# andrewendlinger/xmris

Hardware: AMD Instinct MI355X
Metric: spectra/sec (zero_fill->apodize->FFT->autophase), n_time=4096; HBM-roofline % (higher is better)
Workload: dtype f32

## Files before the change

include/xmris_hip.h:

```cpp
#ifndef XMRIS_HIP_H
#define XMRIS_HIP_H

#include <stdint.h>

#ifdef __cplusplus
extern "C" {
#endif

typedef enum { XM_C64 = 0, XM_C128 = 1 } xm_dtype;

typedef enum {
  XM_OK = 0,
  XM_ERR_INVALID_ARG = -1,
  XM_ERR_UNSUPPORTED_N = -2,
  XM_ERR_HIP = -3,
  XM_ERR_NO_DEVICE = -4
} xm_status;

#define XM_FFT_INVERSE 1u
#define XM_FFT_ORTHO 2u
#define XM_FFT_SHIFT_IN 4u
#define XM_FFT_SHIFT_OUT 8u
#define XM_AMAX_VALUE_ONLY 16u

#define XM_AMAX_GLOBAL_KEY 32u
#define XM_KEY_BYTES 131072
typedef struct {
  float max2;
  float pad_;
  int64_t flat;
} xm_argmax_result;

int xm_version(void);
const char* xm_last_error_string(void);
int xm_clear_cache(void);
const char* xm_last_kernel_string(void);
int xm_fft_supported(int n, int dtype);
int xm_plan_prepare(int n, int dtype);

int xm_zero_fill(const void* in, void* out, int64_t n_batch, int n_in, int n_out, int pad_left,
                 int dtype, void* stream);

int xm_apodize(const void* in, void* out, const void* window, int64_t n_batch, int n, int dtype,
               void* stream);

int xm_zf_apod(const void* in, int64_t in_row_stride, void* out, const void* window, int64_t n_batch, int n_in, int n_out,
               int pad_left, int in_dtype, int out_dtype, void* stream);

int xm_pipeline_key_native(const void* in, int64_t in_row_stride, int n_in, int n_out, int pad_left, unsigned flags,
                           int dtype);

int xm_fft1d_batched(const void* in, void* out, int64_t n_batch, int n, unsigned flags, int dtype,
                     void* stream);

int xm_roll(const void* in, void* out, int64_t n_batch, int n, int shift, int dtype, void* stream);

int xm_phase_apply(const void* in, void* out, const void* phase_table, int64_t n_batch, int n,
                   int dtype, void* stream);

int xm_absmax_rows(const void* in, int64_t n_batch, int n, void* absmax2, int32_t* argidx, int dtype,
                   void* stream);

int xm_row_l1(const void* in, int64_t in_row_stride, const void* window, int64_t n_batch, int n_in, int pad_left,
              int sub_step, void* norm, uint64_t* key, int dtype, void* stream);

int xm_argmax_key_take(uint64_t* key, int n_per_row, void* out_max2, int64_t* out_flat, const void* in,
                       int64_t in_row_stride, int n_in, void* out_row, int dtype, void* stream);

int xm_guess_supported(const void* in, int64_t in_row_stride, int n_in, int n_out, int pad_left, unsigned flags, int dtype);
int xm_guess_rows(const void* in, int64_t in_row_stride, const void* window, int64_t n_batch, int n_in, int n_out,
                  int n_guess, unsigned flags, float* est, uint64_t* key, int dtype, void* stream);
int xm_guess_refine(const void* in, int64_t in_row_stride, const void* window, int64_t n_batch, int n_in, int n_out,
                    unsigned flags, const float* est, uint64_t* guess_key, float band, uint64_t* work_key,
                    float* out_max2, int64_t* out_flat, void* out_row, int dtype, void* stream);

int xm_argmax_reduce(const void* absmax2, const int32_t* argidx, int64_t n_batch, int n, void* out_max2,
                     int64_t* out_flat, int dtype, void* stream);

int xm_gather_row_c128(const void* in, int64_t in_row_stride, int n_in, const int64_t* flat_index, int n_per_row,
                       void* out, int dtype, void* stream);

int xm_pipeline_fused(const void* in, int64_t in_row_stride, void* out, const void* window,
                      const void* phase_table, int64_t n_batch, int n_in, int n_out, int pad_left,
                      unsigned flags, void* absmax2, int32_t* argidx, int dtype, void* stream);

int xm_pipeline_fused_ramp(const void* in, int64_t in_row_stride, void* out, const void* window, double phase0,
                           double dphase, int64_t n_batch, int n_in, int n_out, int pad_left, unsigned flags,
                           void* absmax2, int32_t* argidx, int dtype, void* stream);
int xm_pipeline_ramp_native(const void* in, int64_t in_row_stride, int n_in, int n_out, int pad_left, unsigned flags,
                            int dtype);

int64_t xm_baseline_als_workspace_bytes(int64_t n_batch, int n);
int xm_baseline_als(const void* in, int is_complex, int64_t n_batch, int n, double lam, double p, int n_iter, void* out,
                    void* workspace, int64_t workspace_bytes, int dtype, void* stream);

int xm_amares_model(const double* params, int64_t n_batch, int n_peaks, int n, double dt, double t0, void* out,
                    void* stream);
int64_t xm_amares_workspace_bytes(int64_t n_batch, int n, int n_peaks);
int xm_amares_fit(const void* in, int64_t in_row_stride, int64_t n_batch, int n, double dt, double t0, int n_peaks,
                  const double* init, const double* lower, const double* upper, const int32_t* fixed, int max_iter,
                  double ftol, double xtol, double* params, double* amp_sd, double* rss, int32_t* status,
                  int32_t* iters, void* fit_data, void* workspace, int64_t workspace_bytes, int dtype, void* stream);
int xm_amares_fit_linked(const void* in, int64_t in_row_stride, int64_t n_batch, int n, double dt, double t0,
                         int n_peaks, const double* init, const double* lower, const double* upper,
                         const int32_t* fixed, const int32_t* link_to, const double* link_scale,
                         const double* link_offset, int max_iter, double ftol, double xtol, double* params,
                         double* amp_sd, double* rss, int32_t* status, int32_t* iters, void* fit_data, void* workspace,
                         int64_t workspace_bytes, int dtype, void* stream);

int xm_basis_model(const double* params, int64_t n_batch, const void* basis, int n_metab, const int32_t* group,
                   int n_groups, int n, double dt, void* out, void* stream);
int64_t xm_basis_workspace_bytes(int64_t n_batch, int n, int n_metab);
int xm_basis_fit(const void* in, int64_t in_row_stride, int64_t n_batch, int n, double dt, int skip, const void* basis,
                 int n_metab, const int32_t* group, int n_groups, const double* init, const double* lower,
                 const double* upper, const int32_t* fixed, int max_iter, double ftol, double xtol, double* params,
                 double* amp_sd, double* rss, int32_t* status, int32_t* iters, void* fit_data, void* workspace,
                 int64_t workspace_bytes, int dtype, void* stream);

#define XM_COIL_SVD 0
#define XM_COIL_FIRST_POINT 1
#define XM_COIL_SVD_FMA 2
#define XM_COIL_WORKSPACE_BYTES 256
int xm_coil_combine(const void* x, const void* ref_or_null, void* y, void* w, double* quality, int32_t* status,
                    int64_t n_outer, int C, int64_t n_inner, int N, int N_R, const void* linv_or_null, int method,
                    int n_points, int is_complex128, void* workspace, void* stream);

#define XM_ALIGN_WORKSPACE_BYTES 256
#define XM_ALIGN_SKIP_COARSE 0x100
#define XM_ALIGN_SKIP_REFINE 0x200
#define XM_ALIGN_SKIP_APPLY 0x400
int64_t xm_align_workspace_bytes(int64_t n_outer, int A, int64_t n_inner, int N);
int xm_align_rows(const void* x, const void* r, int64_t r_voxel_stride, void* y, void* mean_or_null, double* shift,
                  double* phase, double* quality, int32_t* status, int32_t* n_averaged_or_null, int64_t n_outer, int A,
                  int64_t n_inner, int N, int N_r, int L, double dt, double t0, double max_shift, double min_quality,
                  int dtype, void* workspace, void* stream);

#define XM_HSVD_WORKSPACE_BYTES 256
#define XM_HSVD_GRAM_FMA 0x100
#define XM_HSVD_STOP_GRAM 0x200
#define XM_HSVD_STOP_EIG 0x400
#define XM_HSVD_STOP_POLES 0x600
#define XM_HSVD_STOP_AMPL 0x800
int xm_hsvd_rows(const void* x, int64_t row_stride, void* y_or_null, double* freq, double* damp, double* amp,
                 double* phase, int32_t* removed, int32_t* n_removed, int32_t* status, int64_t n_batch, int N, int M,
                 int K, double dt, double f_lo, double f_hi, int dtype, void* workspace, void* stream);

#define XM_DENOISE_WORKSPACE_BYTES 256
#define XM_DENOISE_GRAM_FMA 0x100
#define XM_DENOISE_STOP_GRAM 0x200
#define XM_DENOISE_STOP_EIG 0x400
int xm_denoise_patches(const void* x, void* y, int32_t* rank_out, double* sigma, int32_t* status, int64_t n_outer, int s1,
                       int s2, int s3, int p1, int p2, int p3, int N, int rank, int dtype, void* workspace, void* stream);

int xm_axis_dft(const void* x, void* y, const void* table, int64_t n_outer, int n, int m, int64_t n_inner, int dtype,
                void* stream);

#define XM_SENSE_WORKSPACE_BYTES 256
int xm_sense_unfold(const void* a, void* y, const void* sens, const void* linv_or_null, double* g_or_null,
                    int32_t* status_or_null, int64_t n_outer, int C, const int32_t n[3], const int32_t accel[3], int N_t,
                    const int64_t a_strides[5], const int64_t y_strides[4], double regularization, int dtype,
                    void* workspace, void* stream);

int xm_grappa_fill(const void* a, void* y, const void* weights, int64_t n_outer, int C, const int32_t n[3],
                   const int32_t accel[3], const int32_t kernel[3], int N_t, const int64_t a_strides[5],
                   const int64_t y_strides[5], int dtype, void* stream);

int xm_axis_sparse(const void* x, void* y, const int32_t* rowptr, const int32_t* col, const double* val, int64_t n_outer,
                   int64_t n, int64_t n_rows, int64_t n_inner, int dtype, void* stream);

#define XM_CGS_VOXELS 16
int xm_cgs_expand(const void* r, void* p, const void* s, void* u, const double* rho_new, const double* rho_old,
                  const int32_t* status, int64_t n_coils, int64_t n_vox, int64_t n_cols, int first, int dtype,
                  void* stream);
int xm_cgs_reduce(const void* u, const void* s, const void* p, void* q, double* part, int64_t n_coils, int64_t n_vox,
                  int64_t n_cols, double lambda, int initial, int dtype, void* stream);
int xm_cgs_step(void* x, void* r, const void* p, const void* q, const double* rho, const double* rho0,
                const double* delta, double* rho_out, const int32_t* status_in, int32_t* status_out, int32_t* n_iter,
                double* residual, int64_t n_vox, int64_t n_cols, double tol, int iteration, int final_test, void* stream);

int xm_l1_start(const void* b, double* bpart, double* bmax, int32_t* status, double* change, void* x, int64_t n_vox,
                int64_t n_cols, int finish, void* stream);
int xm_l1_prox(void* x, void* v, const void* q, const void* b, const uint8_t* mask, const double* bmax,
               const double* d2_in, const double* n2_in, double* d2_out, double* n2_out, const int32_t* status_in,
               int32_t* status_out, int32_t* n_iter, double* change, int n_dims, int64_t m0, int64_t m1, int64_t m2, int l0,
               int l1, int l2, int s0, int s1, int s2, int64_t n_cols, double tau, double theta_scale, double beta, double tol,
               int iteration, int mode, void* stream);

int xm_espirit_eig(const void* h, void* maps, double* values, int32_t* status, int64_t n_vox, int n_coils, int n_maps,
                   int phase_ref, double crop, void* stream);

int xm_shift_time_fused(int L, int dtype);
int xm_shift_time(const void* in, int64_t in_row_stride, void* out, int64_t n_rows, int n, int L, const double* frac,
                  int64_t n_delay, int64_t delay_div, int dtype, void* stream);

int xm_kinetics_fit(const double* substrate, const double* products, const double* weights, int64_t n_batch,
                    int n_products, int n_times, const double* times, const double* flip_s, const double* flip_p,
                    const double* init, const double* lower, const double* upper, const int32_t* fixed, int max_iter,
                    double ftol, double xtol, double* params, double* param_sd, double* rss, int32_t* status,
                    int32_t* iters, double* fit, double* auc_ratio, void* stream);

#define XM_SPECIES_SKIP_GRAM 0x100
#define XM_SPECIES_SKIP_COARSE 0x200
#define XM_SPECIES_SKIP_REFINE 0x400
#define XM_SPECIES_SKIP_APPLY 0x800
int xm_species_separate(const void* x, void* y, const int64_t* dims, const int64_t* x_strides, const int64_t* y_strides,
                        int n_echoes, int n_species, const double* tables, const double* tau, int64_t tau_s0,
                        int64_t tau_s1, const double* psi, int64_t psi_s0, int64_t psi_s1, double* field,
                        double* residual, int32_t* status, int fit, double max_field, double span, int dtype,
                        void* stream);

#define XM_LIPID_FMA 0x100
#define XM_LIPID_SKIP_COEF 0x200
#define XM_LIPID_SKIP_APPLY 0x400
int xm_lipid_project(const void* x, void* y, int64_t n_rows, int64_t x_row_stride, int64_t y_row_stride, int T, int rank,
                     const double* tables, const uint8_t* apply, int32_t* status, int dtype, void* stream);

#define XM_SUB_MAX_RANK 32
int xm_sub_project(const void* y, void* b, const void* basis, const uint8_t* sampling, int64_t n_coils, int64_t n_samples,
                   int64_t n_frames, int64_t n_time, int rank, int64_t coil_stride, int64_t sample_stride,
                   int64_t frame_stride, int dtype, void* stream);
int xm_sub_mix(const void* a, void* z, const void* kernel, int64_t n_coils, int64_t n_samples, int64_t n_frames, int rank,
               int dtype, void* stream);
int xm_sub_expand(const void* u, const void* basis, void* x, int64_t n_vox, int64_t n_frames, int64_t n_time, int rank,
                  void* stream);

void* xm_solver_create(const double* slice_re_im, const double* coords, int n, double pivot, int method,
                       int target_idx, int index_width);
void xm_solver_destroy(void* solver);
double xm_solver_score(void* solver, const double* x, int nx);
void xm_solver_score_batch(void* solver, const double* xs, int nx, int count, double* out);
long xm_solver_nfev(void* solver);
int xm_solver_set_threads(void* solver, int threads);
int xm_solver_fg(void* solver, const double* x, int n, const double* lb, const double* ub, double* f_out, double* g_out);
long xm_solver_pool_backups(void);
int xm_solver_de(void* solver, int p0_only, unsigned seed, double tol, int maxiter, double* x_out ,
                 double* fun_out, int* nfev_out, int* nit_out);

int xm_phase_table(const double* coords, int n, double p0_deg, double p1_deg, double pivot, void* out, int as_float);

int xm_phase_apply_rows(const void* in, void* out, const double* coords, int64_t n_rows, int n, const double* p0,
                        const double* p1, const double* pivot, const int32_t* skip, int dtype, void* stream);

typedef struct {
  double x[2];
  double fun;
  double pg_norm;
  int32_t nfev, nit;
  int32_t status;
  int32_t needs_polish;
  int32_t target_idx;
  int32_t pad_;
  uint64_t seq;
  double t_us[8];
} xm_search_result;
int xm_search_supported(int n, int method, double x_range);
int xm_search_launch(const void* slice, int n, double c0, double cstep, double x_range, int method, int p0_only,
                     unsigned seed, double tol, int maxiter, uint64_t seq, xm_search_result* out, void* stream);
int xm_search_eval(const void* slice, int n, double c0, double cstep, double x_range, int target_idx, int p0_only,
                   const double* xs, int count, double* fs, void* stream);

enum { XM_SEARCH_CONVERGED = 0, XM_SEARCH_MAXITER = 1, XM_SEARCH_ALL_ZERO = 2, XM_SEARCH_NOT_FINITE = 3 };
typedef struct {
  double x[2];
  double fun;
  double pg_norm;
  int32_t nfev, nit;
  int32_t target_idx;
  int32_t status;
  int32_t needs_polish;
  int32_t pad_;
} xm_search_row;
int xm_search_rows_supported(int n, int method, double x_range, int dtype);
int xm_search_rows(const void* in, int64_t n_rows, int n, int dtype, double c0, double cstep, double x_range, int p0_only,
                   unsigned seed, double tol, int maxiter, double pivot, int target_idx, xm_search_row* records,
                   void* stream);

int xm_hostsearch_submit(const void* slice, int n, const double* coords, int method, int target_idx, int index_width,
                         int p0_only, unsigned seed, double tol, int maxiter, int threads, uint64_t seq,
                         xm_search_result* out);

int xm_hostsearch_set_workers(int n);

int xm_stream_create(void** stream, int reserved_cus, int partition);
int xm_stream_destroy(void* stream);
int xm_stream_cus(void* stream);

int64_t xm_atomic_load_acquire_i64(const int64_t* p);
void xm_atomic_store_release_i64(int64_t* p, int64_t value);
int xm_atomic_wait_all_ge_i64(const int64_t* p, int stride_words, int count, int64_t value, int spin_us);

#ifdef __cplusplus
}
#endif
#endif
```

xmris_amd/_lib.py:

```python
from __future__ import annotations

import ctypes
import os
import threading

XM_C64 = 0
XM_C128 = 1

XM_FFT_INVERSE = 1
XM_FFT_ORTHO = 2
XM_FFT_SHIFT_IN = 4
XM_FFT_SHIFT_OUT = 8
XM_AMAX_VALUE_ONLY = 16
XM_AMAX_GLOBAL_KEY = 32

XM_COIL_SVD = 0
XM_COIL_FIRST_POINT = 1
XM_COIL_SVD_FMA = 2
XM_COIL_WORKSPACE_BYTES = 256

XM_ALIGN_WORKSPACE_BYTES = 256
XM_ALIGN_SKIP_COARSE = 0x100
XM_ALIGN_SKIP_REFINE = 0x200
XM_ALIGN_SKIP_APPLY = 0x400

XM_HSVD_WORKSPACE_BYTES = 256
XM_HSVD_GRAM_FMA = 0x100
XM_HSVD_STOP_GRAM = 0x200
XM_HSVD_STOP_EIG = 0x400
XM_HSVD_STOP_POLES = 0x600
XM_HSVD_STOP_AMPL = 0x800

XM_DENOISE_WORKSPACE_BYTES = 256
XM_DENOISE_GRAM_FMA = 0x100
XM_DENOISE_STOP_GRAM = 0x200
XM_DENOISE_STOP_EIG = 0x400

XM_SPECIES_SKIP_GRAM = 0x100
XM_SPECIES_SKIP_COARSE = 0x200
XM_SPECIES_SKIP_REFINE = 0x400
XM_SPECIES_SKIP_APPLY = 0x800

XM_LIPID_FMA = 0x100
XM_LIPID_SKIP_COEF = 0x200
XM_LIPID_SKIP_APPLY = 0x400

XM_SENSE_WORKSPACE_BYTES = 256
XM_CGS_VOXELS = 16
XM_L1_MAX_BLOCK = 16
XM_SUB_MAX_RANK = 32

XM_ERR_INVALID_ARG = -1
XM_ERR_UNSUPPORTED_N = -2
XM_ERR_HIP = -3
XM_ERR_NO_DEVICE = -4

LIB_NAME = "libxmris_hip.so"
LIB_PATH = os.environ.get("XMRIS_AMD_LIB") or os.path.join(os.path.dirname(os.path.abspath(__file__)), LIB_NAME)

_p = ctypes.c_void_p
_i = ctypes.c_int
_u = ctypes.c_uint
_l = ctypes.c_int64

SIGNATURES = {
    "xm_version": (_i, []),
    "xm_last_error_string": (ctypes.c_char_p, []),
    "xm_clear_cache": (_i, []),
    "xm_last_kernel_string": (ctypes.c_char_p, []),
    "xm_fft_supported": (_i, [_i, _i]),
    "xm_plan_prepare": (_i, [_i, _i]),
    "xm_zero_fill": (_i, [_p, _p, _l, _i, _i, _i, _i, _p]),
    "xm_apodize": (_i, [_p, _p, _p, _l, _i, _i, _p]),
    "xm_fft1d_batched": (_i, [_p, _p, _l, _i, _u, _i, _p]),
    "xm_zf_apod": (_i, [_p, _l, _p, _p, _l, _i, _i, _i, _i, _i, _p]),
    "xm_roll": (_i, [_p, _p, _l, _i, _i, _i, _p]),
    "xm_phase_apply": (_i, [_p, _p, _p, _l, _i, _i, _p]),
    "xm_absmax_rows": (_i, [_p, _l, _i, _p, _p, _i, _p]),
    "xm_argmax_reduce": (_i, [_p, _p, _l, _i, _p, _p, _i, _p]),
    "xm_baseline_als_workspace_bytes": (_l, [_l, _i]),
    "xm_baseline_als": (_i, [_p, _i, _l, _i, ctypes.c_double, ctypes.c_double, _i, _p, _p, _l, _i, _p]),
    "xm_amares_model": (_i, [_p, _l, _i, _i, ctypes.c_double, ctypes.c_double, _p, _p]),
    "xm_amares_workspace_bytes": (_l, [_l, _i, _i]),
    "xm_amares_fit": (_i, [_p, _l, _l, _i, ctypes.c_double, ctypes.c_double, _i, _p, _p, _p, _p, _i, ctypes.c_double,
                           ctypes.c_double, _p, _p, _p, _p, _p, _p, _p, _l, _i, _p]),
    "xm_amares_fit_linked": (_i, [_p, _l, _l, _i, ctypes.c_double, ctypes.c_double, _i, _p, _p, _p, _p, _p, _p, _p, _i,
                                  ctypes.c_double, ctypes.c_double, _p, _p, _p, _p, _p, _p, _p, _l, _i, _p]),
    "xm_basis_model": (_i, [_p, _l, _p, _i, _p, _i, _i, ctypes.c_double, _p, _p]),
    "xm_basis_workspace_bytes": (_l, [_l, _i, _i]),
    "xm_basis_fit": (_i, [_p, _l, _l, _i, ctypes.c_double, _i, _p, _i, _p, _i, _p, _p, _p, _p, _i, ctypes.c_double,
                          ctypes.c_double, _p, _p, _p, _p, _p, _p, _p, _l, _i, _p]),
    "xm_coil_combine": (_i, [_p, _p, _p, _p, _p, _p, _l, _i, _l, _i, _i, _p, _i, _i, _i, _p, _p]),
    "xm_align_workspace_bytes": (_l, [_l, _i, _l, _i]),
    "xm_align_rows": (_i, [_p, _p, _l, _p, _p, _p, _p, _p, _p, _p, _l, _i, _l, _i, _i, _i, ctypes.c_double, ctypes.c_double,
                           ctypes.c_double, ctypes.c_double, _i, _p, _p]),
    "xm_hsvd_rows": (_i, [_p, _l, _p, _p, _p, _p, _p, _p, _p, _p, _l, _i, _i, _i, ctypes.c_double, ctypes.c_double,
                          ctypes.c_double, _i, _p, _p]),
    "xm_denoise_patches": (_i, [_p, _p, _p, _p, _p, _l, _i, _i, _i, _i, _i, _i, _i, _i, _i, _p, _p]),
    "xm_axis_dft": (_i, [_p, _p, _p, _l, _i, _i, _l, _i, _p]),
    "xm_sense_unfold": (_i, [_p, _p, _p, _p, _p, _p, _l, _i, _p, _p, _i, _p, _p, ctypes.c_double, _i, _p, _p]),
    "xm_grappa_fill": (_i, [_p, _p, _p, _l, _i, _p, _p, _p, _i, _p, _p, _i, _p]),
    "xm_axis_sparse": (_i, [_p, _p, _p, _p, _p, _l, _l, _l, _l, _i, _p]),
    "xm_cgs_expand": (_i, [_p, _p, _p, _p, _p, _p, _p, _l, _l, _l, _i, _i, _p]),
    "xm_cgs_reduce": (_i, [_p, _p, _p, _p, _p, _l, _l, _l, ctypes.c_double, _i, _i, _p]),
    "xm_cgs_step": (_i, [_p, _p, _p, _p, _p, _p, _p, _p, _p, _p, _p, _p, _l, _l, ctypes.c_double, _i, _i, _p]),
    "xm_l1_start": (_i, [_p, _p, _p, _p, _p, _p, _l, _l, _i, _p]),
    "xm_l1_prox": (_i, [_p] * 14 + [_i, _l, _l, _l, _i, _i, _i, _i, _i, _i, _l, ctypes.c_double, ctypes.c_double,
                                    ctypes.c_double, ctypes.c_double, _i, _i, _p]),
    "xm_espirit_eig": (_i, [_p, _p, _p, _p, _l, _i, _i, _i, ctypes.c_double, _p]),
    "xm_shift_time_fused": (_i, [_i, _i]),
    "xm_shift_time": (_i, [_p, _l, _p, _l, _i, _i, _p, _l, _l, _i, _p]),
    "xm_kinetics_fit": (_i, [_p, _p, _p, _l, _i, _i, _p, _p, _p, _p, _p, _p, _p, _i, ctypes.c_double, ctypes.c_double, _p, _p,
                             _p, _p, _p, _p, _p, _p]),
    "xm_species_separate": (_i, [_p, _p, _p, _p, _p, _i, _i, _p, _p, _l, _l, _p, _l, _l, _p, _p, _p, _i, ctypes.c_double,
                                 ctypes.c_double, _i, _p]),
    "xm_lipid_project": (_i, [_p, _p, _l, _l, _l, _i, _i, _p, _p, _p, _i, _p]),
    "xm_sub_project": (_i, [_p, _p, _p, _p, _l, _l, _l, _l, _i, _l, _l, _l, _i, _p]),
    "xm_sub_mix": (_i, [_p, _p, _p, _l, _l, _l, _i, _i, _p]),
    "xm_sub_expand": (_i, [_p, _p, _p, _l, _l, _l, _i, _p]),
    "xm_gather_row_c128":(_i, [_p, _l, _i, _p, _i, _p, _i, _p]),
    "xm_pipeline_fused": (_i, [_p, _l, _p, _p, _p, _l, _i, _i, _i, _u, _p, _p, _i, _p]),
    "xm_pipeline_fused_ramp": (_i, [_p, _l, _p, _p, ctypes.c_double, ctypes.c_double, _l, _i, _i, _i, _u, _p, _p, _i, _p]),
    "xm_pipeline_ramp_native": (_i, [_p, _l, _i, _i, _i, _u, _i]),
    "xm_pipeline_key_native": (_i, [_p, _l, _i, _i, _i, _u, _i]),
    "xm_row_l1": (_i, [_p, _l, _p, _l, _i, _i, _i, _p, _p, _i, _p]),
    "xm_argmax_key_take": (_i, [_p, _i, _p, _p, _p, _l, _i, _p, _i, _p]),
    "xm_guess_supported": (_i, [_p, _l, _i, _i, _i, _u, _i]),
    "xm_guess_rows": (_i, [_p, _l, _p, _l, _i, _i, _i, _u, _p, _p, _i, _p]),
    "xm_guess_refine": (_i, [_p, _l, _p, _l, _i, _i, _u, _p, _p, ctypes.c_float, _p, _p, _p, _p, _i, _p]),
    "xm_phase_table": (_i, [_p, _i, ctypes.c_double, ctypes.c_double, ctypes.c_double, _p, _i]),
    "xm_solver_create": (_p, [_p, _p, _i, ctypes.c_double, _i, _i, _i]),
    "xm_solver_destroy": (None, [_p]),
    "xm_solver_score": (ctypes.c_double, [_p, _p, _i]),
    "xm_solver_score_batch": (None, [_p, _p, _i, _i, _p]),
    "xm_solver_fg": (_i, [_p, _p, _i, _p, _p, _p, _p]),
    "xm_solver_pool_backups": (ctypes.c_long, []),
    "xm_solver_nfev": (ctypes.c_long, [_p]),
    "xm_solver_set_threads": (_i, [_p, _i]),
    "xm_solver_de": (_i, [_p, _i, _u, ctypes.c_double, _i, _p, _p, _p, _p]),
    "xm_search_supported": (_i, [_i, _i, ctypes.c_double]),
    "xm_search_launch": (_i, [_p, _i, ctypes.c_double, ctypes.c_double, ctypes.c_double, _i, _i, _u, ctypes.c_double, _i,
                              ctypes.c_uint64, _p, _p]),
    "xm_search_eval": (_i, [_p, _i, ctypes.c_double, ctypes.c_double, ctypes.c_double, _i, _i, _p, _i, _p, _p]),
    "xm_search_rows_supported": (_i, [_i, _i, ctypes.c_double, _i]),
    "xm_search_rows": (_i, [_p, _l, _i, _i, ctypes.c_double, ctypes.c_double, ctypes.c_double, _i, _u, ctypes.c_double, _i,
                            ctypes.c_double, _i, _p, _p]),
    "xm_phase_apply_rows": (_i, [_p, _p, _p, _l, _i, _p, _p, _p, _p, _i, _p]),
    "xm_hostsearch_submit": (_i, [_p, _i, _p, _i, _i, _i, _i, _u, ctypes.c_double, _i, _i, ctypes.c_uint64, _p]),
    "xm_hostsearch_set_workers": (_i, [_i]),
    "xm_stream_create": (_i, [_p, _i, _i]),
    "xm_stream_destroy": (_i, [_p]),
    "xm_stream_cus": (_i, [_p]),
    "xm_atomic_load_acquire_i64": (_l, [_p]),
    "xm_atomic_store_release_i64": (None, [_p, _l]),
    "xm_atomic_wait_all_ge_i64": (_i, [_p, _i, _i, _l, _i]),
}


class XmrisHipError(RuntimeError):

    def __init__(self, func: str, code: int, detail: str):
        self.func, self.code, self.detail = func, code, detail
        super().__init__(f"{func} failed with status {code}: {detail}")


class UnsupportedLengthError(XmrisHipError, ValueError):
    """The transform length has no in-LDS plan on the device (status XM_ERR_UNSUPPORTED_N)."""


_lock = threading.Lock()
_lib = None


def load() -> ctypes.CDLL:
    global _lib
    if _lib is not None:
        return _lib
    with _lock:
        if _lib is not None:
            return _lib
        if not os.path.exists(LIB_PATH):
            raise RuntimeError(
                f"{LIB_PATH} is missing. The xmris_amd hot path has no CPU fallback: build the HIP "
                f"library first (`python -c \"import __graft_entry__ as g; g.build()\"` or "
                f"`make -C xmris_amd/csrc`)."
            )
        lib = ctypes.CDLL(LIB_PATH)
        for name, (res, args) in SIGNATURES.items():
            fn = getattr(lib, name)
            fn.restype = res
            fn.argtypes = args
        _lib = lib
    return _lib


def check(func: str, status: int) -> None:
    if status == 0:
        return
    detail = load().xm_last_error_string()
    detail = detail.decode("utf-8", "replace") if detail else ""
    if status == XM_ERR_UNSUPPORTED_N:
        raise UnsupportedLengthError(func, status, detail)
    raise XmrisHipError(func, status, detail)


def call(func: str, *args) -> None:
    check(func, getattr(load(), func)(*args))
```

xmris_amd/csrc/xm_api.hip:

```cpp
#include "xm_host.h"
#include "xm_als.h"
#include "xm_kernels.h"
#include "xm_plans.h"
#include "xm_zfapod.h"

#include <cmath>
#include <cstdio>
#include <cstdlib>
#include <cstring>
#include <map>
#include <mutex>
#include <tuple>

#define XM_VERSION_NUM 500

static thread_local std::string g_err;
static thread_local std::string g_last_kernel;

#include <cxxabi.h>
void xm_note_kernel(const char* base, const std::type_info* plan, const char* scalar, int mode, int opt) {
  std::string name = base;
  name += "<";
  if (scalar) name += std::string(scalar) + ", ";
  if (plan) {
// ... 260 lines not shown
  HIP_TRY(hipGetDevice(&dev));
  HIP_TRY(hipDeviceGetAttribute(&total, hipDeviceAttributeMultiprocessorCount, dev));
  if (reserved_cus >= total || (partition == 1 && reserved_cus == 0)) return fail(XM_ERR_INVALID_ARG, "xm_stream_create: bad partition");
  const int words = (total + 31) / 32;
  std::vector<uint32_t> mask((size_t)words, 0u);
  for (int i = 0; i < total; ++i) {
    const bool reserved = i < reserved_cus;
    if (reserved == (partition == 1)) mask[i / 32] |= 1u << (i % 32);
  }
  hipStream_t st = nullptr;
  HIP_TRY(hipExtStreamCreateWithCUMask(&st, (uint32_t)words, mask.data()));
  {
    std::lock_guard<std::mutex> lk(g_stream_mu);
    g_stream_cus[st] = partition == 1 ? reserved_cus : total - reserved_cus;
  }
  *stream = (void*)st;
  return XM_OK;
}

extern "C" int xm_stream_destroy(void* stream) {
  if (!stream) return XM_OK;
  {
    std::lock_guard<std::mutex> lk(g_stream_mu);
    g_stream_cus.erase((hipStream_t)stream);
  }
  HIP_TRY(hipStreamDestroy((hipStream_t)stream));
  return XM_OK;
}

extern "C" int xm_stream_cus(void* stream) {
  int cus = 0;
  const int rc = xm_stream_cu_count((hipStream_t)stream, &cus);
  return rc ? rc : cus;
}

const char* xm_last_kernel_string(void) { return g_last_kernel.c_str(); }

int xm_clear_cache(void) {
  {
    std::lock_guard<std::mutex> lk(g_stream_mu);
    g_stream_cus.clear();
  }
  std::lock_guard<std::mutex> lk(g_mu);
  for (auto& kv : g_tables) (void)hipFree(kv.second);
  g_tables.clear();
  for (int d = 0; d < 16; ++d) {
    if (g_queue_base[d]) (void)hipFree(g_queue_base[d]);
    g_queue_base[d] = nullptr;
  }
  return XM_OK;
}

int xm_fft_supported(int n, int dtype) { return xm_supported(n, dtype) ? 1 : 0; }

int xm_plan_prepare(int n, int dtype) {
  if (!xm_supported(n, dtype)) return fail(XM_ERR_UNSUPPORTED_N, "unsupported length " + std::to_string(n));
  int rc = XM_OK;
  const int n_ins[2] = {n, n / 2};
  for (int i = 0; i < (n % 2 == 0 && n >= 4 ? 2 : 1) && rc == XM_OK; ++i) {
    const unsigned fl = XM_FFT_ORTHO | XM_FFT_SHIFT_OUT;
    rc = dtype == XM_C64
             ? xm_pipeline_f32(nullptr, n_ins[i], nullptr, nullptr, nullptr, nullptr, 0, n_ins[i], n, 0, fl, nullptr, nullptr, nullptr)
             : xm_pipeline_f64(nullptr, n_ins[i], nullptr, nullptr, nullptr, nullptr, 0, n_ins[i], n, 0, fl, nullptr, nullptr, nullptr);
  }
  return rc;
}

int xm_zero_fill(const void* in, void* out, int64_t n_batch, int n_in, int n_out, int pad_left, int dtype,
                 void* stream) {
  int rc = check_common(in, n_batch, n_in, dtype);
  if (rc) return rc;
  if (!out || n_out < n_in || pad_left < 0 || pad_left + n_in > n_out)
    return fail(XM_ERR_INVALID_ARG, "zero_fill: bad output pointer or geometry");
  if (n_batch == 0) return XM_OK;
  const long long total = (long long)n_batch * n_out;
  hipStream_t st = (hipStream_t)stream;
  DeviceGuard guard(in);
  if (dtype == XM_C64)
    hipLaunchKernelGGL(k_zero_fill<float>, dim3(grid_for(total, 256)), dim3(256), 0, st, (const Cx<float>*)in,
                       (Cx<float>*)out, (long long)n_batch, n_in, n_out, pad_left);
  else
    hipLaunchKernelGGL(k_zero_fill<double>, dim3(grid_for(total, 256)), dim3(256), 0, st, (const Cx<double>*)in,
                       (Cx<double>*)out, (long long)n_batch, n_in, n_out, pad_left);
  HIP_TRY(hipGetLastError());
  return XM_OK;
}

int xm_apodize(const void* in, void* out, const void* window, int64_t n_batch, int n, int dtype, void* stream) {
  int rc = check_common(in, n_batch, n, dtype);
  if (rc) return rc;
  if (!out || !window) return fail(XM_ERR_INVALID_ARG, "apodize: null output or window");
  if (n_batch == 0) return XM_OK;
  const long long total = (long long)n_batch * n;
  hipStream_t st = (hipStream_t)stream;
  DeviceGuard guard(in);
  if (dtype == XM_C64)
    hipLaunchKernelGGL(k_apodize<float>, dim3(grid_for(total, 256)), dim3(256), 0, st, (const Cx<float>*)in,
                       (Cx<float>*)out, (const float*)window, (long long)n_batch, n);
  else
    hipLaunchKernelGGL(k_apodize<double>, dim3(grid_for(total, 256)), dim3(256), 0, st, (const Cx<double>*)in,
                       (Cx<double>*)out, (const double*)window, (long long)n_batch, n);
  HIP_TRY(hipGetLastError());
  return XM_OK;
}

int xm_zf_apod(const void* in, int64_t in_row_stride, void* out, const void* window, int64_t n_batch, int n_in, int n_out,
               int pad_left, int in_dtype, int out_dtype, void* stream) {
  int rc = check_common(in, n_batch, n_in, in_dtype);
  if (rc) return rc;
  if (!out || !window || n_out < n_in || pad_left < 0 || pad_left + n_in > n_out || in_row_stride < n_in || in == out)
    return fail(XM_ERR_INVALID_ARG, "zf_apod: bad pointer or geometry");
  if ((out_dtype != XM_C64 && out_dtype != XM_C128) || (in_dtype == XM_C128 && out_dtype == XM_C64))
    return fail(XM_ERR_INVALID_ARG, "zf_apod: the output precision is the input's or complex128");
  if ((size_t)n_out * (out_dtype == XM_C64 ? 4 : 8) > 96 * 1024)
    return fail(XM_ERR_UNSUPPORTED_N, "zf_apod: the window does not fit the LDS (use xm_zero_fill + xm_apodize)");
  if (n_batch == 0) return XM_OK;
  hipStream_t st = (hipStream_t)stream;
  DeviceGuard guard(in);
  if (in_dtype == XM_C64 && out_dtype == XM_C64)
    return launch_zf_apod<float, float>(in, in_row_stride, out, window, n_batch, n_in, n_out, pad_left, st);
  if (in_dtype == XM_C64)
    return launch_zf_apod<float, double>(in, in_row_stride, out, window, n_batch, n_in, n_out, pad_left, st);
  return launch_zf_apod<double, double>(in, in_row_stride, out, window, n_batch, n_in, n_out, pad_left, st);
}

int xm_phase_apply(const void* in, void* out, const void* phase_table, int64_t n_batch, int n, int dtype,
                   void* stream) {
  int rc = check_common(in, n_batch, n, dtype);
  if (rc) return rc;
  if (!out || !phase_table) return fail(XM_ERR_INVALID_ARG, "phase_apply: null output or table");
  if (n_batch == 0) return XM_OK;
  const long long total = (long long)n_batch * n;
  hipStream_t st = (hipStream_t)stream;
  DeviceGuard guard(in);
  if (dtype == XM_C64)
    hipLaunchKernelGGL(k_phase<float>, dim3(grid_for(total, 256)), dim3(256), 0, st, (const Cx<float>*)in,
                       (Cx<float>*)out, (const Cx<float>*)phase_table, (long long)n_batch, n);
  else
    hipLaunchKernelGGL(k_phase<double>, dim3(grid_for(total, 256)), dim3(256), 0, st, (const Cx<double>*)in,
                       (Cx<double>*)out, (const Cx<double>*)phase_table, (long long)n_batch, n);
  HIP_TRY(hipGetLastError());
  return XM_OK;
}

int xm_phase_apply_rows(const void* in, void* out, const double* coords, int64_t n_rows, int n, const double* p0,
                        const double* p1, const double* pivot, const int32_t* skip, int dtype, void* stream) {
  int rc = check_common(in, n_rows, n, dtype);
  if (rc) return rc;
  if (n_rows == 0) return XM_OK;
  if (!out || !coords || !p0 || !p1 || !pivot) return fail(XM_ERR_INVALID_ARG, "phase_apply_rows: null pointer");
  const long long tiles = ((long long)n + kPhaseRowsBins * kPhaseRowsThreads - 1) / (kPhaseRowsBins * kPhaseRowsThreads);
  long long grid = (long long)n_rows * tiles;
  if (grid > 256LL * 8) grid = 256LL * 8;
  hipStream_t st = (hipStream_t)stream;
  DeviceGuard guard(in);
  if (dtype == XM_C64)
    hipLaunchKernelGGL(k_phase_rows<float>, dim3((unsigned)grid), dim3(kPhaseRowsThreads), 0, st, (const Cx<float>*)in,
                       (Cx<float>*)out, coords, (long long)n_rows, n, p0, p1, pivot, (const int*)skip);
  else
    hipLaunchKernelGGL(k_phase_rows<double>, dim3((unsigned)grid), dim3(kPhaseRowsThreads), 0, st, (const Cx<double>*)in,
                       (Cx<double>*)out, coords, (long long)n_rows, n, p0, p1, pivot, (const int*)skip);
  HIP_TRY(hipGetLastError());
  return XM_OK;
}

int xm_roll(const void* in, void* out, int64_t n_batch, int n, int shift, int dtype, void* stream) {
  int rc = check_common(in, n_batch, n, dtype);
  if (rc) return rc;
  if (!out || in == out) return fail(XM_ERR_INVALID_ARG, "roll: output must be a distinct buffer");
  if (n_batch == 0) return XM_OK;
  shift %= n;
  if (shift < 0) shift += n;
  const long long total = (long long)n_batch * n;
  hipStream_t st = (hipStream_t)stream;
  DeviceGuard guard(in);
  if (dtype == XM_C64)
    hipLaunchKernelGGL(k_roll<float>, dim3(grid_for(total, 256)), dim3(256), 0, st, (const Cx<float>*)in,
                       (Cx<float>*)out, (long long)n_batch, n, shift);
  else
    hipLaunchKernelGGL(k_roll<double>, dim3(grid_for(total, 256)), dim3(256), 0, st, (const Cx<double>*)in,
                       (Cx<double>*)out, (long long)n_batch, n, shift);
  HIP_TRY(hipGetLastError());
  return XM_OK;
}

int xm_absmax_rows(const void* in, int64_t n_batch, int n, void* absmax2, int32_t* argidx, int dtype,
                   void* stream) {
  int rc = check_common(in, n_batch, n, dtype);
  if (rc) return rc;
  if (!absmax2 || !argidx) return fail(XM_ERR_INVALID_ARG, "absmax_rows: null outputs");
  if (n_batch == 0) return XM_OK;
  hipStream_t st = (hipStream_t)stream;
  DeviceGuard guard(in);
  const int grid = (int)(n_batch < 65536 * 4 ? n_batch : 65536 * 4);
  if (dtype == XM_C64)
    hipLaunchKernelGGL(k_absmax_rows<float>, dim3(grid), dim3(256), 0, st, (const Cx<float>*)in,
                       (long long)n_batch, n, (float*)absmax2, argidx);
  else
    hipLaunchKernelGGL(k_absmax_rows<double>, dim3(grid), dim3(256), 0, st, (const Cx<double>*)in,
                       (long long)n_batch, n, (double*)absmax2, argidx);
  HIP_TRY(hipGetLastError());
  return XM_OK;
}

int xm_row_l1(const void* in, int64_t in_row_stride, const void* window, int64_t n_batch, int n_in, int pad_left,
              int sub_step, void* norm, uint64_t* key, int dtype, void* stream) {
  int rc = check_common(in, n_batch, n_in, dtype);
  if (rc) return rc;
  if ((!norm && !key) || pad_left < 0 || in_row_stride < n_in || sub_step < 1)
    return fail(XM_ERR_INVALID_ARG, "row_l1: bad arguments");
  if (key && (dtype != XM_C64 || n_batch > 0xffffffffLL))
    return fail(XM_ERR_INVALID_ARG, "row_l1: the arg-max key needs complex64 and fewer than 2^32 rows");
  if (n_batch == 0) return XM_OK;
  hipStream_t st = (hipStream_t)stream;
  DeviceGuard guard(in);
  const int64_t want = (n_batch + 3) / 4;
  const int grid = (int)(want < 256 * 8 ? want : 256 * 8);
  if (dtype == XM_C64)
    hipLaunchKernelGGL(k_row_l1<float>, dim3(grid), dim3(256), 0, st, (const Cx<float>*)in, (long long)in_row_stride,
                       (const float*)window, (long long)n_batch, n_in, pad_left, sub_step, (float*)norm,
                       (unsigned long long*)key);
  else
    hipLaunchKernelGGL(k_row_l1<double>, dim3(grid), dim3(256), 0, st, (const Cx<double>*)in,
                       (long long)in_row_stride, (const double*)window, (long long)n_batch, n_in, pad_left, sub_step,
                       (double*)norm, (unsigned long long*)nullptr);
  HIP_TRY(hipGetLastError());
  return XM_OK;
}

int xm_argmax_reduce(const void* absmax2, const int32_t* argidx, int64_t n_batch, int n, void* out_max2,
                     int64_t* out_flat, int dtype, void* stream) {
  if (!absmax2 || !argidx || !out_max2 || !out_flat || n_batch < 1 || n < 1)
    return fail(XM_ERR_INVALID_ARG, "argmax_reduce: null pointer or empty batch");
  if (dtype != XM_C64 && dtype != XM_C128) return fail(XM_ERR_INVALID_ARG, "bad dtype");
  hipStream_t st = (hipStream_t)stream;
  DeviceGuard guard(absmax2);
  if (dtype == XM_C64)
    hipLaunchKernelGGL(k_argmax_final<float>, dim3(1), dim3(1024), 0, st, (const float*)absmax2, argidx,
                       (long long)n_batch, n, (float*)out_max2, (long long*)out_flat);
  else
    hipLaunchKernelGGL(k_argmax_final<double>, dim3(1), dim3(1024), 0, st, (const double*)absmax2, argidx,
                       (long long)n_batch, n, (double*)out_max2, (long long*)out_flat);
  HIP_TRY(hipGetLastError());
  return XM_OK;
}

int xm_argmax_key_take(uint64_t* key, int n_per_row, void* out_max2, int64_t* out_flat, const void* in,
                       int64_t in_row_stride, int n_in, void* out_row, int dtype, void* stream) {
  if (!key || !out_max2 || !out_flat || n_per_row < 1) return fail(XM_ERR_INVALID_ARG, "argmax_key_take: null pointer");
  if (in && (!out_row || n_in < 1 || in_row_stride < n_in)) return fail(XM_ERR_INVALID_ARG, "argmax_key_take: bad row geometry");
  if (dtype != XM_C64 && dtype != XM_C128) return fail(XM_ERR_INVALID_ARG, "bad dtype");
  hipStream_t st = (hipStream_t)stream;
  DeviceGuard guard(key);
  if (dtype == XM_C64)
    hipLaunchKernelGGL(k_key_take<float>, dim3(1), dim3(1024), 0, st, (unsigned long long*)key, n_per_row, (float*)out_max2,
                       (long long*)out_flat, (const Cx<float>*)in, (long long)in_row_stride, n_in, (Cx<double>*)out_row);
  else
    hipLaunchKernelGGL(k_key_take<double>, dim3(1), dim3(1024), 0, st, (unsigned long long*)key, n_per_row, (float*)out_max2,
                       (long long*)out_flat, (const Cx<double>*)in, (long long)in_row_stride, n_in, (Cx<double>*)out_row);
  HIP_TRY(hipGetLastError());
  return XM_OK;
}

int xm_guess_supported(const void* in, int64_t in_row_stride, int n_in, int n_out, int pad_left, unsigned flags, int dtype) {
  if (!in || (dtype != XM_C64 && dtype != XM_C128) || in_row_stride < n_in) return 0;
  return xm_zf2p_guess_supported(in, in_row_stride, n_in, n_out, pad_left, flags, dtype);
}

static float guess_scale(int n_out, unsigned flags) {
  return (flags & XM_FFT_ORTHO) ? (float)(1.0 / std::sqrt((double)n_out)) : 1.0f;
}

int xm_guess_rows(const void* in, int64_t in_row_stride, const void* window, int64_t n_batch, int n_in, int n_out,
                  int n_guess, unsigned flags, float* est, uint64_t* key, int dtype, void* stream) {
  int rc = check_common(in, n_batch, n_out, dtype);
  if (rc) return rc;
  if (!est || !key || n_guess < 0 || n_batch > 0xffffffffLL)
    return fail(XM_ERR_INVALID_ARG, "guess_rows: null output or bad sizes");
  if (!xm_guess_supported(in, in_row_stride, n_in, n_out, 0, flags, dtype))
    return fail(XM_ERR_INVALID_ARG, "guess_rows: geometry outside xm_guess_supported");
  if (n_batch == 0) return XM_OK;
  DeviceGuard guard(in);
  return xm_zf2p_guess_rows(in, in_row_stride, (const float*)window, n_batch, n_in, n_out, n_guess,
                            guess_scale(n_out, flags), est, (unsigned long long*)key, dtype, (hipStream_t)stream);
}

int xm_guess_refine(const void* in, int64_t in_row_stride, const void* window, int64_t n_batch, int n_in, int n_out,
                    unsigned flags, const float* est, uint64_t* guess_key, float band, uint64_t* work_key,
                    float* out_max2, int64_t* out_flat, void* out_row, int dtype, void* stream) {
  int rc = check_common(in, n_batch, n_out, dtype);
  if (rc) return rc;
  if (!est || !guess_key || !work_key || work_key == guess_key || !out_flat || n_batch < 1 || n_batch > 0xffffffffLL ||
      !(band > 0.0f && band <= 1.0f))
    return fail(XM_ERR_INVALID_ARG, "guess_refine: null pointer, empty batch or band outside (0, 1]");
  if (!xm_guess_supported(in, in_row_stride, n_in, n_out, 0, flags, dtype))
    return fail(XM_ERR_INVALID_ARG, "guess_refine: geometry outside xm_guess_supported");
  DeviceGuard guard(in);
  return xm_zf2p_guess_refine(in, in_row_stride, (const float*)window, n_batch, n_in, n_out, flags,
                              guess_scale(n_out, flags), est, (unsigned long long*)guess_key, band,
                              (unsigned long long*)work_key, out_max2, (long long*)out_flat, out_row, dtype,
                              (hipStream_t)stream);
}

int64_t xm_baseline_als_workspace_bytes(int64_t n_batch, int n) {
  if (n_batch < 0 || n < 0) return 0;
  return 5 * n_batch * (int64_t)n * (int64_t)sizeof(double);
}

int xm_baseline_als(const void* in, int is_complex, int64_t n_batch, int n, double lam, double p, int n_iter, void* out,
                    void* workspace, int64_t workspace_bytes, int dtype, void* stream) {
  if ((!in || !out || !workspace) && n_batch > 0) return fail(XM_ERR_INVALID_ARG, "baseline_als: null pointer");
  if (n_batch < 0 || n < 4 || n_iter < 1) return fail(XM_ERR_INVALID_ARG, "baseline_als: needs n >= 4, n_iter >= 1");
  if (dtype != XM_C64 && dtype != XM_C128) return fail(XM_ERR_INVALID_ARG, "bad dtype");
  if (workspace_bytes < xm_baseline_als_workspace_bytes(n_batch, n))
    return fail(XM_ERR_INVALID_ARG, "baseline_als: workspace too small (see xm_baseline_als_workspace_bytes)");
  if (n_batch == 0) return XM_OK;
  hipStream_t st = (hipStream_t)stream;
  DeviceGuard guard(in);
  const long long plane = (long long)n_batch * n;
  double* yt = (double*)workspace;
  double *zt = yt + plane, *l1t = yt + 2 * plane, *l2t = yt + 3 * plane, *vt = yt + 4 * plane;
  const long long by = (n_batch + 31) / 32;
  if (by > 65535) return fail(XM_ERR_INVALID_ARG, "baseline_als: n_batch too large for one launch (> 2M spectra)");
  dim3 tgrid((n + 31) / 32, (unsigned)by), tblock(32, 8);
  if (dtype == XM_C64) {
    if (is_complex)
      hipLaunchKernelGGL((k_als_transpose_in<float, true>), tgrid, tblock, 0, st, (const float*)in, (long long)n_batch, n, yt);
    else
      hipLaunchKernelGGL((k_als_transpose_in<float, false>), tgrid, tblock, 0, st, (const float*)in, (long long)n_batch, n, yt);
  } else {
    if (is_complex)
      hipLaunchKernelGGL((k_als_transpose_in<double, true>), tgrid, tblock, 0, st, (const double*)in, (long long)n_batch, n, yt);
    else
      hipLaunchKernelGGL((k_als_transpose_in<double, false>), tgrid, tblock, 0, st, (const double*)in, (long long)n_batch, n, yt);
  }
  hipLaunchKernelGGL(k_als_solve, dim3((unsigned)((n_batch + 63) / 64)), dim3(64), 0, st, yt, zt, l1t, l2t, vt,
                     (long long)n_batch, n, lam, p, n_iter);
  hipLaunchKernelGGL(k_als_transpose_out, tgrid, tblock, 0, st, yt, zt, (long long)n_batch, n, (double*)out);
  HIP_TRY(hipGetLastError());
  return XM_OK;
}

int xm_gather_row_c128(const void* in, int64_t in_row_stride, int n_in, const int64_t* flat_index, int n_per_row,
                       void* out, int dtype, void* stream) {
  if (!in || !flat_index || !out || n_in < 1 || n_per_row < 1 || in_row_stride < n_in)
    return fail(XM_ERR_INVALID_ARG, "gather_row: null pointer or bad geometry");
  if (dtype != XM_C64 && dtype != XM_C128) return fail(XM_ERR_INVALID_ARG, "bad dtype");
  hipStream_t st = (hipStream_t)stream;
  DeviceGuard guard(in);
  const int grid = (n_in + 255) / 256;
  if (dtype == XM_C64)
    hipLaunchKernelGGL(k_gather_row<float>, dim3(grid), dim3(256), 0, st, (const Cx<float>*)in,
                       (long long)in_row_stride, n_in, (const long long*)flat_index, n_per_row, (Cx<double>*)out);
  else
    hipLaunchKernelGGL(k_gather_row<double>, dim3(grid), dim3(256), 0, st, (const Cx<double>*)in,
                       (long long)in_row_stride, n_in, (const long long*)flat_index, n_per_row, (Cx<double>*)out);
  HIP_TRY(hipGetLastError());
  return XM_OK;
}

static int pipeline_common(const void* in, int64_t in_row_stride, void* out, const void* window,
                           const void* phase_table, const double* ramp, int64_t n_batch, int n_in, int n_out,
                           int pad_left, unsigned flags, void* absmax2, int32_t* argidx, int dtype, void* stream) {
  int rc = check_common(in, n_batch, n_out, dtype);
  if (rc) return rc;
  if (n_in < 1 || pad_left < 0 || pad_left + n_in > n_out || in_row_stride < n_in)
    return fail(XM_ERR_INVALID_ARG, "pipeline: bad zero-fill geometry or row stride");
  if (flags & XM_AMAX_GLOBAL_KEY) {
    if (!absmax2 || n_batch > 0xffffffffLL ||
        !xm_pipeline_key_native(in, in_row_stride, n_in, n_out, pad_left, flags & ~(XM_AMAX_GLOBAL_KEY | XM_AMAX_VALUE_ONLY), dtype))
      return fail(XM_ERR_INVALID_ARG, "pipeline: XM_AMAX_GLOBAL_KEY needs a key and a geometry of xm_pipeline_key_native");
    if (dtype == XM_C128 && !argidx)
      return fail(XM_ERR_INVALID_ARG, "pipeline: complex128 arg-max keys are decoded by the launch itself (result record needed)");
  } else if ((absmax2 == nullptr) != (argidx == nullptr))
    return fail(XM_ERR_INVALID_ARG, "pipeline: absmax2 and argidx must be given together");
  if (!out && !absmax2) return fail(XM_ERR_INVALID_ARG, "pipeline: nothing to produce");
  if (out == in) return fail(XM_ERR_INVALID_ARG, "pipeline: in-place operation is not supported");
  if (ramp && !out) return fail(XM_ERR_INVALID_ARG, "pipeline: a phase ramp needs an output");
  if (flags & ~(XM_FFT_INVERSE | XM_FFT_ORTHO | XM_FFT_SHIFT_IN | XM_FFT_SHIFT_OUT | XM_AMAX_VALUE_ONLY | XM_AMAX_GLOBAL_KEY))
    return fail(XM_ERR_INVALID_ARG, "pipeline: unknown flag bits");
  if (!xm_supported(n_out, dtype))
    return fail(XM_ERR_UNSUPPORTED_N, "no plan for length " + std::to_string(n_out));
  hipStream_t st = (hipStream_t)stream;
  DeviceGuard guard(in);
  if (dtype == XM_C64)
    return xm_pipeline_f32(in, in_row_stride, out, window, phase_table, ramp, n_batch, n_in, n_out, pad_left, flags,
                           absmax2, argidx, st);
  return xm_pipeline_f64(in, in_row_stride, out, window, phase_table, ramp, n_batch, n_in, n_out, pad_left, flags,
                         absmax2, argidx, st);
}

int xm_pipeline_fused(const void* in, int64_t in_row_stride, void* out, const void* window,
                      const void* phase_table, int64_t n_batch, int n_in, int n_out, int pad_left, unsigned flags,
                      void* absmax2, int32_t* argidx, int dtype, void* stream) {
  return pipeline_common(in, in_row_stride, out, window, phase_table, nullptr, n_batch, n_in, n_out, pad_left, flags,
                         absmax2, argidx, dtype, stream);
}

int xm_pipeline_fused_ramp(const void* in, int64_t in_row_stride, void* out, const void* window, double phase0,
                           double dphase, int64_t n_batch, int n_in, int n_out, int pad_left, unsigned flags,
                           void* absmax2, int32_t* argidx, int dtype, void* stream) {
  const double ramp[2] = {phase0, dphase};
  return pipeline_common(in, in_row_stride, out, window, nullptr, ramp, n_batch, n_in, n_out, pad_left, flags, absmax2,
                         argidx, dtype, stream);
}

int xm_pipeline_ramp_native(const void* in, int64_t in_row_stride, int n_in, int n_out, int pad_left, unsigned flags,
                            int dtype) {
  if ((dtype != XM_C64 && dtype != XM_C128) || n_in < 1 || pad_left < 0 || pad_left + n_in > n_out) return 0;
  return dtype == XM_C64 ? xm_ramp_native_f32(in, in_row_stride, n_in, n_out, pad_left, flags)
                         : xm_ramp_native_f64(in, in_row_stride, n_in, n_out, pad_left, flags);
}

int xm_pipeline_key_native(const void* in, int64_t in_row_stride, int n_in, int n_out, int pad_left, unsigned flags,
                           int dtype) {
  if ((dtype != XM_C64 && dtype != XM_C128) || n_in < 1 || pad_left < 0 || pad_left + n_in > n_out) return 0;
  return dtype == XM_C64 ? xm_key_native_f32(in, in_row_stride, n_in, n_out, pad_left, flags)
                         : xm_key_native_f64(in, in_row_stride, n_in, n_out, pad_left, flags);
}

int xm_fft1d_batched(const void* in, void* out, int64_t n_batch, int n, unsigned flags, int dtype, void* stream) {
  if (!out) return fail(XM_ERR_INVALID_ARG, "fft: null output");
  return xm_pipeline_fused(in, n, out, nullptr, nullptr, n_batch, n, n, 0, flags, nullptr, nullptr, dtype, stream);
}

}
```

xmris_amd/csrc/xm_coarse.h:

```cpp
#pragma once
#include "xm_kernels.h"

typedef _Float16 xm_h8 __attribute__((ext_vector_type(8)));
typedef _Float16 xm_h2 __attribute__((ext_vector_type(2)));
typedef float xm_f16v __attribute__((ext_vector_type(16)));

struct CoarseArgs {
  const void* in;
  const float* window;
  const Cx<float>* w1024;
  float* est;
  unsigned long long* gkey;
  long long in_stride;
  long long n_batch;
  float scale2;
};

constexpr int kCoarseWaves = 4;

XM_DEV Cx<float> coarse_w1024(const Cx<float>* __restrict__ t, unsigned k) {
  k &= 1023u;
  const Cx<float> w = t[k & 511u];
  return (k & 512u) ? mk<float>(-w.re, -w.im) : w;
}

XM_DEV xm_h8 coarse_pack(const float* v) {
  union {
    xm_h8 v8;
    xm_h2 v2[4];
  } u;
#pragma unroll
  for (int j = 0; j < 4; ++j) {
    const xm_f2 p = {v[2 * j], v[2 * j + 1]};
    u.v2[j] = __builtin_convertvector(p, xm_h2);
  }
  return u.v8;
}

template <bool IN64>
__global__ __launch_bounds__(64 * kCoarseWaves, 2) void k_coarse_mfma(CoarseArgs A) {
  const unsigned lane = threadIdx.x & 63u, r = lane & 31u, h = lane >> 5;
  const long long wave = (long long)blockIdx.x * kCoarseWaves + (threadIdx.x >> 6);
  const long long n_waves = (long long)gridDim.x * kCoarseWaves;

  xm_h8 b1r, b1i, b1n, a2r[2], a2i[2], a2n[2];
  {
    float cr[8], ci[8], cn[8];
#pragma unroll
    for (int j = 0; j < 8; ++j) {
      const Cx<float> w = coarse_w1024(A.w1024, 32u * ((8u * h + (unsigned)j) * r));
      cr[j] = w.re;
      ci[j] = w.im;
      cn[j] = -w.im;
    }
    b1r = coarse_pack(cr);
    b1i = coarse_pack(ci);
    b1n = coarse_pack(cn);
#pragma unroll
    for (int s = 0; s < 2; ++s) {
#pragma unroll
      for (int j = 0; j < 8; ++j) {
        const unsigned n2 = 16u * s + 8u * ((unsigned)j >> 2) + 4u * h + ((unsigned)j & 3u);
        const Cx<float> w = coarse_w1024(A.w1024, 32u * (n2 * r));
        cr[j] = w.re;
        ci[j] = w.im;
        cn[j] = -w.im;
      }
      a2r[s] = coarse_pack(cr);
      a2i[s] = coarse_pack(ci);
      a2n[s] = coarse_pack(cn);
    }
  }
  float twr[16], twi[16];
#pragma unroll
  for (int q = 0; q < 16; ++q) {
    const unsigned n2 = ((unsigned)q & 3u) + 8u * ((unsigned)q >> 2) + 4u * h;
    const Cx<float> w = coarse_w1024(A.w1024, n2 * r);
    twr[q] = w.re;
    twi[q] = w.im;
  }
  float wnd[8];
#pragma unroll
  for (int j = 0; j < 8; ++j) wnd[j] = A.window[32u * (8u * h + (unsigned)j) + r];

  auto fetch = [&](long long s, Cx<float>* x) {
    if constexpr (IN64) {
      const xm_d2* __restrict__ row = reinterpret_cast<const xm_d2*>(A.in) + s * A.in_stride;
#pragma unroll
      for (int j = 0; j < 8; ++j) {
        const xm_d2 v = __builtin_nontemporal_load(row + 32u * (8u * h + (unsigned)j) + r);
        x[j] = mk<float>((float)v.x, (float)v.y);
      }
      return;
    }
    const xm_f2* __restrict__ row = reinterpret_cast<const xm_f2*>(A.in) + s * A.in_stride;
#pragma unroll
    for (int j = 0; j < 8; ++j) {
      const xm_f2 v = __builtin_nontemporal_load(row + 32u * (8u * h + (unsigned)j) + r);
      x[j] = mk<float>(v.x, v.y);
    }
  };

  unsigned best_key = 0u, best_row = 0u;
  bool have = false;
  constexpr int DEPTH = 1;
  Cx<float> nx[DEPTH][8];
  long long s = wave;
#pragma unroll
  for (int d = 0; d < DEPTH; ++d)
    if (s + d * n_waves < A.n_batch) fetch(s + d * n_waves, nx[d]);
  auto one_row = [&](Cx<float>* cur, long long s) {
    float re[8], im[8];
    float m = 0.f;
#pragma unroll
    for (int j = 0; j < 8; ++j) {
      re[j] = cur[j].re * wnd[j];
      im[j] = cur[j].im * wnd[j];
      m = fmaxf(m, fmaxf(fabsf(re[j]), fabsf(im[j])));
    }
    if (s + DEPTH * n_waves < A.n_batch) fetch(s + DEPTH * n_waves, cur);
    unsigned e = (wave_reduce_u32<true>(__float_as_uint(m)) >> 23) & 0xffu;
    e = e > 253u ? 253u : (e < 1u ? 1u : e);
    const float up = __uint_as_float((254u - e) << 23);
    const float down = __uint_as_float(e << 23);
#pragma unroll
    for (int j = 0; j < 8; ++j) {
      re[j] *= up;
      im[j] *= up;
    }
    const xm_h8 ar = coarse_pack(re), ai = coarse_pack(im);
    xm_f16v d1r = {0.f}, d1i = {0.f};
    d1r = __builtin_amdgcn_mfma_f32_32x32x16_f16(ar, b1r, d1r, 0, 0, 0);
    d1r = __builtin_amdgcn_mfma_f32_32x32x16_f16(ai, b1n, d1r, 0, 0, 0);
    d1i = __builtin_amdgcn_mfma_f32_32x32x16_f16(ar, b1i, d1i, 0, 0, 0);
    d1i = __builtin_amdgcn_mfma_f32_32x32x16_f16(ai, b1r, d1i, 0, 0, 0);
    float zr[16], zi[16];
#pragma unroll
    for (int q = 0; q < 16; ++q) {
      zr[q] = d1r[q] * twr[q] - d1i[q] * twi[q];
      zi[q] = d1r[q] * twi[q] + d1i[q] * twr[q];
    }
    xm_f16v d2r = {0.f}, d2i = {0.f};
#pragma unroll
    for (int k = 0; k < 2; ++k) {
      const xm_h8 br = coarse_pack(zr + 8 * k), bi = coarse_pack(zi + 8 * k);
      d2r = __builtin_amdgcn_mfma_f32_32x32x16_f16(a2r[k], br, d2r, 0, 0, 0);
      d2r = __builtin_amdgcn_mfma_f32_32x32x16_f16(a2n[k], bi, d2r, 0, 0, 0);
      d2i = __builtin_amdgcn_mfma_f32_32x32x16_f16(a2r[k], bi, d2i, 0, 0, 0);
      d2i = __builtin_amdgcn_mfma_f32_32x32x16_f16(a2i[k], br, d2i, 0, 0, 0);
    }
    float bv = -1.f;
#pragma unroll
    for (int q = 0; q < 16; ++q) bv = fmaxf(bv, d2r[q] * d2r[q] + d2i[q] * d2i[q]);
    bv = amax_nan_if_unset(bv);
    bv = bv * (down * down) * A.scale2;
    const unsigned key = wave_reduce_u32<true>(bv != bv ? 0x7fc00000u : __float_as_uint(bv));
    const unsigned row = (unsigned)s;
    const bool take = !have || key > best_key;
    best_key = take ? key : best_key;
    best_row = take ? row : best_row;
    have = true;
    if (lane == 0u) A.est[s] = __uint_as_float(key);
  };
  for (; s < A.n_batch; s += DEPTH * n_waves) {
#pragma unroll
    for (int d = 0; d < DEPTH; ++d)
      if (s + d * n_waves < A.n_batch) one_row(nx[d], s + d * n_waves);
  }
  if (A.gkey && have && lane == 0u)
    atomicMax(A.gkey + (blockIdx.x % XM_KEY_SLOTS) * XM_KEY_STRIDE,
              ((unsigned long long)best_key << 32) | (unsigned long long)(0xffffffffu - best_row));
}
```

xmris_amd/csrc/xm_host.h:

```cpp
#pragma once
#include <cstdlib>
#include "../../include/xmris_hip.h"
#include "xm_common.h"

#include <cmath>
#include <map>
#include <mutex>
#include <string>
#include <type_traits>
#include <utility>
#include <typeinfo>
#include <vector>

int xm_fail(int code, const std::string& msg);
#define HIP_TRY(expr)                                                                \
  do {                                                                               \
    hipError_t e_ = (expr);                                                          \
    if (e_ != hipSuccess) {                                                          \
      (void)hipGetLastError();  \
      return xm_fail(XM_ERR_HIP, std::string(#expr) + ": " + hipGetErrorString(e_)); \
    }                                                                                \
  } while (0)

struct DeviceGuard {
  int prev = -1;
  explicit DeviceGuard(const void* dev_ptr) {
    if (!dev_ptr) return;
    hipPointerAttribute_t at;
    if (hipPointerGetAttributes(&at, dev_ptr) != hipSuccess) {
      (void)hipGetLastError();
      return;
    }
    if (at.type != hipMemoryTypeDevice) return;
    int cur = 0;
    if (hipGetDevice(&cur) != hipSuccess) return;
    if (cur != at.device && hipSetDevice(at.device) == hipSuccess) prev = cur;
  }
  ~DeviceGuard() {
    if (prev >= 0) (void)hipSetDevice(prev);
  }
};

enum XmTableKind { TK_TWIDDLE = 0, TK_HALF = 1, TK_CHIRP = 2, TK_CHIRP_FFT = 3, TK_BIG_WN = 4 };

typedef void (*xm_table_gen)(int n, int m, const void* ctx, std::vector<double>& re, std::vector<double>& im);
int xm_table_get(int kind, int n, int m, int dtype, xm_table_gen gen, const void* ctx, const void** out);

void xm_unit(long long num, long long den, double sign, double& c, double& s);

bool xm_has_direct_plan(int n, int dtype);
bool xm_has_pow2_plan(int n, int dtype);
int xm_bluestein_m(int n);
bool xm_supported(int n, int dtype);

int xm_pipeline_f32(const void* in, int64_t in_stride, void* out, const void* window, const void* phase,
                    const double* ramp, int64_t n_batch, int n_in, int n_out, int pad_left, unsigned flags,
                    void* absmax2, int32_t* argidx, hipStream_t st);
int xm_pipeline_f64(const void* in, int64_t in_stride, void* out, const void* window, const void* phase,
                    const double* ramp, int64_t n_batch, int n_in, int n_out, int pad_left, unsigned flags,
                    void* absmax2, int32_t* argidx, hipStream_t st);
int xm_big_supported_f32(int n);
int xm_big_supported_f64(int n);
bool xm_supported_in_lds(int n, int dtype);
int xm_ramp_native_f32(const void* in, int64_t in_stride, int n_in, int n_out, int pad_left, unsigned flags);
int xm_ramp_native_f64(const void* in, int64_t in_stride, int n_in, int n_out, int pad_left, unsigned flags);
int xm_key_native_f32(const void* in, int64_t in_stride, int n_in, int n_out, int pad_left, unsigned flags);
int xm_key_native_f64(const void* in, int64_t in_stride, int n_in, int n_out, int pad_left, unsigned flags);

template <class T>
struct PipeArgs;
int xm_zf2p_launch(int h, int mode, const PipeArgs<float>& A, const double* ramp, hipStream_t st);
int xm_zf2d_launch(int h, int mode, const PipeArgs<double>& A, const double* ramp, hipStream_t st);
int xm_zf2p_guess_supported(const void* in, int64_t in_stride, int n_in, int n_out, int pad_left, unsigned flags, int dtype);
int xm_zf2p_guess_rows(const void* in, int64_t in_stride, const float* window, int64_t n_batch, int n_in, int n_out,
                       int n_guess, float scale, float* est, unsigned long long* key, int dtype, hipStream_t st);
int xm_zf2p_guess_refine(const void* in, int64_t in_stride, const float* window, int64_t n_batch, int n_in, int n_out,
                         unsigned flags, float scale, const float* est, unsigned long long* guess_key, float band,
                         unsigned long long* work_key, float* out_max2, long long* out_flat, void* out_row, int dtype,
                         hipStream_t st);

int xm_queue_slot(unsigned** out);

int xm_ramp_table_async(void* table, int n, double phase0, double dphase, int dtype, hipStream_t st);

extern "C" int xm_stream_cu_count(hipStream_t st, int* cus);

struct XmResidency {
  std::mutex mu;
  std::map<std::pair<int, size_t>, int> blocks;
  size_t opt_in[16] = {0};
};
template <class K>
int xm_resident_blocks(XmResidency& r, K kern, int nt, size_t lds, int* out, hipStream_t st = nullptr, int max_per_cu = 0) {
  int dev = 0;
  HIP_TRY(hipGetDevice(&dev));
  if (dev < 0 || dev >= 16) return xm_fail(XM_ERR_INVALID_ARG, "device ordinal out of range");
  int per_cu = 0;
  {
    std::lock_guard<std::mutex> lk(r.mu);
    if (lds > 48 * 1024 && lds > r.opt_in[dev]) {
      HIP_TRY(hipFuncSetAttribute((const void*)kern, hipFuncAttributeMaxDynamicSharedMemorySize, (int)lds));
      r.opt_in[dev] = lds;
    }
    auto it = r.blocks.find({dev, lds});
    if (it == r.blocks.end()) {
      int q = 0;
      HIP_TRY(hipOccupancyMaxActiveBlocksPerMultiprocessor(&q, kern, nt, lds));
      it = r.blocks.emplace(std::make_pair(dev, lds), q < 1 ? 1 : q).first;
    }
    per_cu = it->second;
  }
  if (max_per_cu > 0 && per_cu > max_per_cu) per_cu = max_per_cu;
  int cus = 0;
  const int rc = xm_stream_cu_count(st, &cus);
  if (rc) return rc;
  *out = per_cu * cus;
  return XM_OK;
}

template <int... Ms, class F>
int xm_with_mode(int mode, F&& f) {
  int rc = XM_OK;
  const bool hit = ((mode == Ms ? (rc = f(std::integral_constant<int, Ms>{}), true) : false) || ...);
  return hit ? rc : xm_fail(XM_ERR_INVALID_ARG, "no kernel built for mode " + std::to_string(mode));
}

template <class PL, bool PAIRED, class Args>
void xm_set_ramp(Args& A, const double* ramp) {
  using R = typename std::remove_reference<decltype(A.ramp_c[0])>::type;
  constexpr long long M = PAIRED ? 2 : 1;
  for (int q = 0; q < PL::P; ++q) {
    const long long base = (M * PL::NT * q + A.out_shift) % (M * PL::N);
    const double a = ramp[0] + ramp[1] * (double)base;
    A.ramp_c[2 * q] = (R)std::cos(a);
    A.ramp_c[2 * q + 1] = (R)std::sin(a);
  }
  if (PAIRED) {
    A.ramp_e[0] = (R)std::cos(ramp[1]);
    A.ramp_e[1] = (R)std::sin(ramp[1]);
  }
  A.ramp_db = ramp[1];
  A.phase = nullptr;
}

inline bool xm_pair_loads_ok(const void* in, int64_t in_stride, int n_in, int pad_left) {
  return (pad_left % 2 == 0) && (n_in % 2 == 0) && (in_stride % 2 == 0) && ((reinterpret_cast<size_t>(in) & 15u) == 0);
}

void xm_note_kernel(const char* base, const std::type_info* plan, const char* scalar, int mode, int opt);

template <class K, class Args>
int xm_launch_items(XmResidency& res, K kern, int nt, size_t lds, long long n_items, const Args& A, hipStream_t st,
                    const char* name, const char* form, int mode, int opt) {
  HIP_TRY(hipMemsetAsync(A.counter, 0, 2 * sizeof(unsigned), st));
  int resident = 0;
  if (const int rc = xm_resident_blocks(res, kern, nt, lds, &resident, st)) return rc;
  const long long blocks = n_items < resident ? n_items : resident;
  xm_note_kernel(name, nullptr, form, mode, opt);
  hipLaunchKernelGGL(kern, dim3((unsigned)blocks), dim3(nt), lds, st, A);
  HIP_TRY(hipGetLastError());
  return XM_OK;
}
```

xmris_amd/csrc/xm_zf2p.h:

```cpp
#pragma once
#include "xm_kernels.h"

enum { ZF2P_LOAD16 = 1, ZF2P_NT = 2, ZF2P_QUEUE = 8, ZF2P_EST = 16, ZF2P_CAND = 32, ZF2P_IN64 = 64 };
constexpr int ZF2P_CAND_CAP = 16;
constexpr int ZF2P_CAND_KMAX = 16384;
constexpr int ZF2P_CAND_ROWS = 1, ZF2P_CAND_EST = 1 + ZF2P_CAND_CAP, ZF2P_CAND_COUNT = 1 + 2 * ZF2P_CAND_CAP,
              ZF2P_CAND_TOP = ZF2P_CAND_COUNT + 1, ZF2P_CAND_BITMAP = ZF2P_CAND_TOP + 1;
constexpr size_t zf2p_cand_lds_bytes() { return (ZF2P_CAND_BITMAP + ZF2P_CAND_KMAX / 32) * sizeof(unsigned); }

constexpr int xm_ilog2(int v) {
  int s = 0;
  while ((1 << s) < v) ++s;
  return s;
}

template <class PL, bool L16>
constexpr int zf2p_pad_shift() {
  if (!L16) return -1;
  return PL::radix(0) == 8 ? 4 : xm_ilog2(2 * PL::radix(0));
}

template <class PL, int MODE, int OPT>
__global__ __launch_bounds__(PL::NT, (zf2_waves<float, PL>())) void k_zf2p(PipeArgs<float> A) {
  using T = float;
  using V = xm_f2;
  constexpr unsigned N = 2 * PL::N, NT = PL::NT;
  constexpr int P = PL::P;
  constexpr bool WRITE = (MODE & ZF2_WRITE) != 0, PHASE = (MODE & ZF2_PHASE) != 0, AMAX = (MODE & ZF2_AMAX) != 0;
  constexpr bool RAMP = (MODE & ZF2_RAMP) != 0;
  constexpr bool L16 = (OPT & ZF2P_LOAD16) != 0;
  constexpr int AUX = (OPT & ZF2P_NT) ? 2 : 0;
  constexpr bool EST = (OPT & ZF2P_EST) != 0, CAND = (OPT & ZF2P_CAND) != 0, IN64 = (OPT & ZF2P_IN64) != 0;
  static_assert(!EST || (NT == XM_WAVE && AMAX && !WRITE), "the per-row estimate is stored by the row's one wave");
  static_assert(!CAND || (AMAX && !WRITE && (OPT & ZF2P_QUEUE) == 0), "candidates: maxima only, static order");
  static_assert(!(IN64 && L16), "pair loads are complex64 loads");
  static_assert(!(PHASE && RAMP), "phase table and ramp are exclusive");
  static_assert(!RAMP || WRITE, "a ramp needs an output");
  static_assert(P % 2 == 0 && NT >= XM_WAVE, "pair loads need an even number of points per thread, whole waves");
  using FFT = BlockFFT<V, PL, zf2p_pad_shift<PL, L16>()>;
  using HT = HotTw<T, PL, RAMP>;
  extern __shared__ __attribute__((aligned(16))) char xm_smem[];
  Cx<V>* lds = reinterpret_cast<Cx<V>*>(xm_smem);
  Cx<T>* mid = reinterpret_cast<Cx<T>*>(lds + FFT::lds_elems());
  T* red_v = reinterpret_cast<T*>(mid + HT::mid_lds_size());
  int* red_i = reinterpret_cast<int*>(red_v + NT / XM_WAVE + 1);
  unsigned* lds_next = reinterpret_cast<unsigned*>(red_i + NT / XM_WAVE + 1);
  constexpr bool QUEUE = (OPT & ZF2P_QUEUE) != 0;
  const unsigned t = threadIdx.x;
  const unsigned lane = t & (XM_WAVE - 1), half = lane >> 5;
  const unsigned col = L16 ? (t & ~(XM_WAVE - 1u)) + 2u * (lane & 31u) + half : t;

  long long n_rows = A.n_batch;
  unsigned* cand = lds_next + ZF2P_CAND_ROWS;
  const unsigned n_in = (unsigned)A.n_in;
  if constexpr (CAND) {
    float* cand_e = reinterpret_cast<float*>(lds_next + ZF2P_CAND_EST);
    unsigned* cand_n = lds_next + ZF2P_CAND_COUNT;
    unsigned* top_bits = lds_next + ZF2P_CAND_TOP;
    unsigned* bitmap = lds_next + ZF2P_CAND_BITMAP;
    const unsigned G = gridDim.x, b = blockIdx.x;
    const unsigned kmax = (unsigned)((A.n_batch + G - 1) / G);
    for (unsigned i = t; i < (kmax + 31u) / 32u; i += NT) bitmap[i] = 0u;
    if (t < XM_WAVE) {
      const unsigned long long k = __hip_atomic_load(A.gkey_in + t * XM_KEY_STRIDE, __ATOMIC_RELAXED, __HIP_MEMORY_SCOPE_AGENT);
      const unsigned hi = wave_reduce_u32<true>((unsigned)(k >> 32));
      if (t == 0) *top_bits = hi;
    }
    __syncthreads();
    const float thr = A.band2 * __uint_as_float(*top_bits);
    for (unsigned k = t; k < kmax; k += NT) {
      const long long r = (long long)k * G + (b + 37u * k) % G;
      if (r < A.n_batch) {
        const float e = A.est[r];
        if (e >= thr || e != e) atomicOr(&bitmap[k >> 5], 1u << (k & 31u));
      }
    }
    __syncthreads();
    if (t == 0) {
      unsigned n = 0;
      for (unsigned w = 0; w < (kmax + 31u) / 32u; ++w) {
        unsigned bits = bitmap[w];
        while (bits) {
          const unsigned k = w * 32u + (unsigned)__builtin_ctz(bits);
          bits &= bits - 1u;
          const unsigned r = (unsigned)((long long)k * G + (b + 37u * k) % G);
          float e = A.est[r];
          e = e != e ? __builtin_inff() : e;
          unsigned pos = n;
          while (pos > 0 && cand_e[pos - 1] < e) --pos;
          if (pos >= (unsigned)ZF2P_CAND_CAP) continue;
          const unsigned top = n < (unsigned)ZF2P_CAND_CAP ? n : (unsigned)ZF2P_CAND_CAP - 1u;
          for (unsigned i = top; i > pos; --i) {
            cand[i] = cand[i - 1];
            cand_e[i] = cand_e[i - 1];
          }
          cand[pos] = r;
          cand_e[pos] = e;
          n = n < (unsigned)ZF2P_CAND_CAP ? n + 1u : n;
        }
      }
      *cand_n = n;
    }
    __syncthreads();
    n_rows = (long long)(unsigned)__builtin_amdgcn_readfirstlane((int)*cand_n);
  }
  const bool live = !CAND || n_rows > 0;

  HT tw;
  tw.mid = HT::mid_in_lds() ? mid : A.tw;
  if (live) {
    tw.load(A.tw, (int)t);
    for (unsigned i = t; i < (unsigned)HT::mid_lds_size(); i += NT) mid[i] = A.tw[i];
  }
  if constexpr (RAMP) {
    double sn, cs;
    sincos(A.ramp_db * (double)(2u * t), &sn, &cs);
    tw.fold(mk<T>((T)cs, (T)sn));
  }
  Cx<T> rot = live ? A.aux[col] : mk<T>(T(0), T(0));
  if constexpr (RAMP) rot = rot * mk<T>(A.ramp_e[0], A.ramp_e[1]);
  const unsigned coff = col - (unsigned)A.pad_left;
  T w[P];
#pragma unroll
  for (int q = 0; q < P; ++q) {
    const bool ok = live && (coff + NT * q) < n_in;
    w[q] = ok ? (A.window ? A.window[col + NT * q] * A.scale : A.scale) : T(0);
  }
  __syncthreads();

  constexpr int NRAW = L16 ? P / 2 : P;
  typedef unsigned raw_t __attribute__((ext_vector_type((L16 || IN64) ? 4 : 2)));
  raw_t raw[NRAW];
  const unsigned e0 = (t & ~(XM_WAVE - 1u)) + 2u * (lane & 31u) + NT * half - (unsigned)A.pad_left;
  auto fetch = [&](long long s2, unsigned ee0, unsigned cc, unsigned nin) {
    constexpr size_t EB = IN64 ? 16u : 8u;
    const char* __restrict__ row = reinterpret_cast<const char*>(A.in) + (size_t)(s2 * A.in_stride) * EB;
    if constexpr (L16) {
#pragma unroll
      for (int j = 0; j < P / 2; ++j) {
        const unsigned e = min(ee0 + 2u * NT * j, nin - 2u);
        raw[j] = __builtin_nontemporal_load(reinterpret_cast<const raw_t*>(row + (size_t)e * 8u));
      }
    } else {
#pragma unroll
      for (int q = 0; q < P; ++q) {
        const unsigned e = min(cc + NT * q, nin - 1u);
        raw[q] = *reinterpret_cast<const raw_t*>(row + (size_t)e * EB);
      }
    }
  };
  unsigned best_key = 0, best_row = 0;
  bool have = false;
  auto rowid = [&](long long v) -> long long {
    if constexpr (CAND) return (long long)(unsigned)__builtin_amdgcn_readfirstlane((int)cand[v]);
    else return v;
  };
  unsigned gb_seen = 0;
  auto next_live = [&](long long v) -> long long {
    if constexpr (CAND) {
      const float* cand_e = reinterpret_cast<const float*>(lds_next + ZF2P_CAND_EST);
      const unsigned gb = wave_reduce_u32<true>(__hip_atomic_load(A.gbest + lane * (2u * XM_KEY_STRIDE), __ATOMIC_RELAXED,
                                                                  __HIP_MEMORY_SCOPE_AGENT));
      gb_seen = gb;
      const float lim = A.band2 * __uint_as_float(gb);
      while (v < n_rows && __uint_as_float((unsigned)__builtin_amdgcn_readfirstlane((int)__float_as_uint(cand_e[v]))) < lim) ++v;
    }
    return v;
  };
  const long long ch = (!CAND && A.queue_chunk > 0) ? A.queue_chunk : 1;
  const long long c_first = CAND ? 0 : blockIdx.x, c_step = CAND ? 1 : gridDim.x;
  long long c_cur = c_first, c_nxt = c_cur + c_step, c_nn = c_nxt + c_step;
  long long s = c_cur * ch;
  unsigned off = 0;
  if constexpr (CAND) {
    if (n_rows > 0) {
      const float* cand_e = reinterpret_cast<const float*>(lds_next + ZF2P_CAND_EST);
      const float top = __uint_as_float((unsigned)__builtin_amdgcn_readfirstlane((int)__float_as_uint(cand_e[0])));
      const float emax2 = __uint_as_float((unsigned)__builtin_amdgcn_readfirstlane((int)lds_next[ZF2P_CAND_TOP]));
      if (top < 0.81f * emax2) {
#pragma unroll 1
        for (int i = 0; i < 3; ++i) __builtin_amdgcn_s_sleep(127);
        if (t < XM_WAVE) {
          const long long nx = next_live(0);
          if (t == 0u) *lds_next = (unsigned)nx;
        }
        __syncthreads();
        s = (long long)(unsigned)__builtin_amdgcn_readfirstlane((int)*lds_next);
        __syncthreads();
      }
    }
  }
  if (s < n_rows) fetch(rowid(s), e0, coff, n_in);
  if constexpr (QUEUE) {
    if (t == 0) *lds_next = atomicAdd(A.queue, 1u) + gridDim.x;
    __syncthreads();
    c_nxt = (long long)(unsigned)__builtin_amdgcn_readfirstlane((int)*lds_next);
    __syncthreads();
  }

  while (s < n_rows) {
    const bool chunk_end = (off + 1 == (unsigned)ch) || (s + 1 >= n_rows);
    long long s_nxt = chunk_end ? c_nxt * ch : s + 1;
    unsigned tt = t, cc = col, sh = (unsigned)A.out_shift, nin = n_in, pl = (unsigned)A.pad_left, ee0 = e0;
    asm volatile("" : "+v"(tt));
    asm volatile("" : "+v"(cc));
    asm volatile("" : "+v"(ee0));
    asm volatile("" : "+s"(sh));
    asm volatile("" : "+s"(nin));
    asm volatile("" : "+s"(pl));

    Cx<T> xr[P];
    if constexpr (L16) {
#pragma unroll
      for (int j = 0; j < P / 2; ++j) {
        const auto re = __builtin_amdgcn_permlane32_swap(raw[j].x, raw[j].z, false, false);
        const auto im = __builtin_amdgcn_permlane32_swap(raw[j].y, raw[j].w, false, false);
        xr[2 * j] = mk<T>(__uint_as_float(re[0]), __uint_as_float(im[0]));
        xr[2 * j + 1] = mk<T>(__uint_as_float(re[1]), __uint_as_float(im[1]));
      }
    } else if constexpr (IN64) {
#pragma unroll
      for (int q = 0; q < P; ++q) {
        Cx<double> d;
        __builtin_memcpy(&d, &raw[q], 16);
        xr[q] = mk<T>((T)d.re, (T)d.im);
      }
    } else {
#pragma unroll
      for (int q = 0; q < P; ++q) xr[q] = mk<T>(__uint_as_float(raw[q].x), __uint_as_float(raw[q].y));
    }
    Cx<V> v[P];
    static_for<0, P>([&](auto qc) {
      constexpr int q = decltype(qc)::value;
      const Cx<T> e = xr[q] * w[q];
      const Cx<T> o = mul_w<q, 2 * P, T>(e * rot);
      v[q].re = V{e.re, o.re};
      v[q].im = V{e.im, o.im};
    });
    if constexpr (!CAND) {
      if (s_nxt < n_rows) fetch(rowid(s_nxt), ee0, cc - pl, nin);
    }
    if constexpr (CAND) {
      FFT::run_cols(v, lds, tw, (int)tt, (int)cc, [&]() {
        if (tt < XM_WAVE) {
          const long long nx = next_live(s + 1);
          if (tt == 0u) *lds_next = (unsigned)nx;
        }
      });
      s_nxt = (long long)(unsigned)__builtin_amdgcn_readfirstlane((int)*lds_next);
      if (s_nxt < n_rows) fetch(rowid(s_nxt), ee0, cc - pl, nin);
    } else if constexpr (QUEUE) {
      const bool claim = off == 0u;
      unsigned ticket = 0;
      if (claim && tt == 0u) ticket = atomicAdd(A.queue, 1u) + gridDim.x;
      FFT::run_cols(v, lds, tw, (int)tt, (int)cc, [&]() {
        if (claim && tt == 0u) *lds_next = ticket;
      });
      if (claim) c_nn = (long long)(unsigned)__builtin_amdgcn_readfirstlane((int)*lds_next);
    } else {
      FFT::run_cols(v, lds, tw, (int)tt, (int)cc);
    }

    const unsigned t2 = 2u * tt;
    if constexpr (AMAX) {
      T bv = T(-1);
#pragma unroll
      for (int q = 0; q < P; ++q) {
        const V m2 = v[q].re * v[q].re + v[q].im * v[q].im;
        bv = fmax(bv, fmax(m2.x, m2.y));
      }
      bv = amax_nan_if_unset(bv);
      if (A.amax_value_only) {
        const unsigned key = wave_reduce_u32<true>(__float_as_uint(bv));
        if (A.gkey) {
          const unsigned r = (unsigned)rowid(s);
          const bool take = !have || key > best_key || (CAND && key == best_key && r < best_row);
          if constexpr (CAND) {
            if (lane == 0u && key > gb_seen) atomicMax(A.gbest + (blockIdx.x % XM_KEY_SLOTS) * (2u * XM_KEY_STRIDE), key);
          }
          best_key = take ? key : best_key;
          best_row = take ? r : best_row;
          have = true;
          if constexpr (EST) {
            if (lane == 0u) A.est[r] = __uint_as_float(key);
          }
        } else {
          if ((tt & (XM_WAVE - 1)) == 0u) atomicMax(reinterpret_cast<unsigned*>(A.absmax2 + s), key);
          if (tt == 0u) A.argidx[s] = 0;
        }
      } else {
        int bi = 0;
        if (!A.amax_value_only) {
          bi = 0x7fffffff;
          const bool all_nan = bv != bv;
#pragma unroll
          for (int q = 0; q < P; ++q) {
            const int k0 = (int)(((2u * NT * q + sh) & (N - 1u)) + t2);
            const V m2 = v[q].re * v[q].re + v[q].im * v[q].im;
            bi = min(bi, ((m2.x == bv) | all_nan) ? k0 : 0x7fffffff);
            bi = min(bi, ((m2.y == bv) | all_nan) ? k0 + 1 : 0x7fffffff);
          }
        }
        amax_reduce_store<T, (int)NT>(bv, bi, (int)tt, true, s, A.absmax2, A.argidx, red_v, red_i);
      }
    }
    if constexpr (WRITE) {
      Cx<T>* __restrict__ orow = A.out + s * (long long)N;
      const __amdgpu_buffer_rsrc_t rph = xm_rsrc(A.phase, PHASE ? N * 8u : 0u);
      typedef const T __attribute__((address_space(4))) * kptr_t;
      kptr_t rc = (kptr_t)((const char __attribute__((address_space(4)))*)__builtin_amdgcn_kernarg_segment_ptr() +
                           __builtin_offsetof(PipeArgs<T>, ramp_c));
      asm volatile("" : "+s"(rc));
      static_for<0, P>([&](auto qc) {
        constexpr int q = decltype(qc)::value;
        const unsigned base = (2u * NT * q + sh) & (N - 1u);
        const __amdgpu_buffer_rsrc_t rout = xm_rsrc(orow + base, 2u * NT * 8u);
        Cx<V> y = v[q];
        if constexpr (RAMP) {
          const V cr = V{rc[2 * q], rc[2 * q]}, ci = V{rc[2 * q + 1], rc[2 * q + 1]};
          y.re = __builtin_elementwise_fma(v[q].re, cr, -(v[q].im * ci));
          y.im = __builtin_elementwise_fma(v[q].re, ci, v[q].im * cr);
        } else if constexpr (PHASE) {
          const CxPair<T> ph = buf_load(rph, t2 * 8u, base * 8u, (CxPair<T>*)nullptr);
          const V cr = V{ph.a.re, ph.b.re}, ci = V{ph.a.im, ph.b.im};
          y.re = __builtin_elementwise_fma(v[q].re, cr, -(v[q].im * ci));
          y.im = __builtin_elementwise_fma(v[q].re, ci, v[q].im * cr);
        }
        xm_u4 u;
        u.x = __float_as_uint(y.re.x);
        u.y = __float_as_uint(y.im.x);
        u.z = __float_as_uint(y.re.y);
        u.w = __float_as_uint(y.im.y);
        __builtin_amdgcn_raw_buffer_store_b128(u, rout, t2 * 8u, 0, AUX);
      });
    }
    if (chunk_end) {
      c_cur = c_nxt;
      c_nxt = c_nn;
      if constexpr (!QUEUE) c_nn = c_nxt + c_step;
      off = 0;
    } else {
      ++off;
    }
    s = s_nxt;
  }
  if constexpr (AMAX) {
    if (A.gkey && have && lane == 0u)
      atomicMax(A.gkey + (blockIdx.x % XM_KEY_SLOTS) * XM_KEY_STRIDE,
                ((unsigned long long)best_key << 32) | (unsigned long long)(0xffffffffu - best_row));
  }
  if constexpr (QUEUE || CAND || (AMAX && WRITE)) {
    bool decode = false;
    if constexpr (AMAX) decode = A.gkey && (A.key_result || (CAND && A.take_flat));
    if (decode) {
      asm volatile("s_waitcnt vmcnt(0)" ::: "memory");
      __syncthreads();
    }
    unsigned last = 0;
    if (t == 0) {
      const unsigned d = atomicAdd(A.queue + 1, 1u);
      last = d == gridDim.x - 1u;
      if (last) {
        __hip_atomic_store(A.queue, 0u, __ATOMIC_RELAXED, __HIP_MEMORY_SCOPE_AGENT);
        __hip_atomic_store(A.queue + 1, 0u, __ATOMIC_RELAXED, __HIP_MEMORY_SCOPE_AGENT);
      }
      if constexpr (CAND) *lds_next = last;
    }
    if constexpr (AMAX) {
      if (decode && t < XM_WAVE) {
        last = (unsigned)__builtin_amdgcn_readfirstlane((int)last);
        if (last) {
          unsigned long long k = __hip_atomic_load(A.gkey + t * XM_KEY_STRIDE, __ATOMIC_RELAXED, __HIP_MEMORY_SCOPE_AGENT);
          __hip_atomic_store(A.gkey + t * XM_KEY_STRIDE, 0ull, __ATOMIC_RELAXED, __HIP_MEMORY_SCOPE_AGENT);
          if constexpr (CAND) {
            __hip_atomic_store(A.gkey_in + t * XM_KEY_STRIDE, 0ull, __ATOMIC_RELAXED, __HIP_MEMORY_SCOPE_AGENT);
            __hip_atomic_store(A.gbest + t * (2u * XM_KEY_STRIDE), 0u, __ATOMIC_RELAXED, __HIP_MEMORY_SCOPE_AGENT);
          }
#pragma unroll
          for (int m = XM_WAVE / 2; m >= 1; m >>= 1) {
            const unsigned hi = (unsigned)__shfl_xor((int)(k >> 32), m, XM_WAVE), lo = (unsigned)__shfl_xor((int)(unsigned)k, m, XM_WAVE);
            const unsigned long long o = ((unsigned long long)hi << 32) | lo;
            k = o > k ? o : k;
          }
          if (t == 0) {
            const unsigned row = k ? 0xffffffffu - (unsigned)(k & 0xffffffffu) : 0u;
            if (A.key_result) {
              A.key_result->max2 = __uint_as_float((unsigned)(k >> 32));
              A.key_result->flat = (long long)row * (long long)N;
            }
            if constexpr (CAND) {
              if (A.take_max2) A.take_max2[0] = __uint_as_float((unsigned)(k >> 32));
              A.take_flat[0] = (long long)row * (long long)N;
              cand[0] = row;
            }
          }
        }
      }
      if constexpr (CAND) {
        if (decode) {
          __syncthreads();
          if (*lds_next != 0u && A.take_row) {
            const size_t r = (size_t)cand[0] * (size_t)A.in_stride;
            for (unsigned j = t; j < n_in; j += NT) {
              if constexpr (IN64) {
                A.take_row[j] = reinterpret_cast<const Cx<double>*>(A.in)[r + j];
              } else {
                const Cx<T> x = A.in[r + j];
                A.take_row[j] = mk<double>((double)x.re, (double)x.im);
              }
            }
          }
        }
      }
    }
  }
}
```

xmris_amd/device.py:

```python
from __future__ import annotations

import ctypes
import math

import numpy as np

from . import _lib


def _torch():
    import torch

    return torch


def _dtype_code(x) -> int:
    torch = _torch()
    if x.dtype == torch.complex64:
        return _lib.XM_C64
    if x.dtype == torch.complex128:
        return _lib.XM_C128
    raise TypeError(f"xmris_amd kernels need complex64/complex128 data, got {x.dtype}")


# ... 1498 lines not shown

    def row_level(t_):
        if t_.shape[-1] > 1 and t_.stride(-1) != 1:
            return None
        lv = _collapse(lead, [[t_.stride(a)] for a in range(len(lead))])
        if len(lv) > 1 or (lv and lv[0][1][0] < T):
            return None
        return lv[0][1][0] if lv else T

    in_place = out is x
    if out is not None and (tuple(out.shape) != tuple(x.shape) or out.dtype != x.dtype or out.device != x.device):
        raise ValueError("out must have x's shape, dtype and device")
    xs, copied = x, False
    sx = row_level(xs)
    if sx is None:
        xs, copied, in_place = x.contiguous(), True, False
        sx = T
    if in_place:
        ys = xs
    elif out is not None and not copied and row_level(out) is not None:
        ys = out
    else:
        ys = torch.empty(xs.shape, dtype=x.dtype, device=x.device)
    sy = row_level(ys)
    status = torch.empty(lead, dtype=torch.int32, device=x.device)
    ap = None
    if apply is not None:
        ap = apply if isinstance(apply, torch.Tensor) else torch.from_numpy(np.ascontiguousarray(apply))
        if tuple(ap.shape) != lead:
            raise ValueError(f"apply must have the data's leading shape {lead}, got {tuple(ap.shape)}")
        ap = (ap != 0).to(device=x.device, dtype=torch.uint8).contiguous()
    if form == "fma":
        code |= LIPID_FLAGS["fma"]
    for s in _skip:
        code |= LIPID_FLAGS[s]
    _lib.call("xm_lipid_project", xs.data_ptr(), ys.data_ptr(), n_rows, int(sx), int(sy), T, r, tables.data_ptr(),
              ap.data_ptr() if ap is not None else None, status.data_ptr(), code, _stream(x))
    if out is not None and ys is not out:
        out.copy_(ys)
        ys = out
    return LipidResult(out=ys, status=status, copied=copied)


SUB_MAX_RANK = _lib.XM_SUB_MAX_RANK


def _sub_basis(basis, what: str = "basis"):
    torch = _torch()
    _require_device(basis)
    if basis.dtype != torch.complex128 or basis.dim() != 2 or not basis.is_contiguous():
        raise ValueError(f"{what} must be a contiguous complex128 tensor [R, T], got {tuple(basis.shape)} of {basis.dtype}")
    r, t = (int(n) for n in basis.shape)
    if not 1 <= r <= SUB_MAX_RANK or r > t:
        raise ValueError(f"{what}: rank {r} must be in 1 ... {SUB_MAX_RANK} and at most T = {t}")
    return r, t


def sub_project(y, basis, sampling=None):
    torch = _torch()
    _require_device(y)
    code = _dtype_code(y)
    if y.dim() != 4:
        raise ValueError(f"y must be [C, S, F, T], got {tuple(y.shape)}")
    c, s, f, t = (int(n) for n in y.shape)
    r, tb = _sub_basis(basis)
    if tb != t:
        raise ValueError(f"sub_project: the data has {t} points along time, the basis {tb}")
    if t > 1 and y.stride(3) != 1:
        y = y.contiguous()
    m = None
    if sampling is not None:
        _require_device(sampling)
        if sampling.dtype not in (torch.uint8, torch.bool) or tuple(sampling.shape) != (s, t) or not sampling.is_contiguous():
            raise ValueError(f"sampling must be a contiguous uint8 / bool tensor of shape {(s, t)}")
        m = sampling
    b = torch.empty((c, s, r, f), dtype=y.dtype, device=y.device)
    if b.numel():
        _lib.call("xm_sub_project", y.data_ptr(), b.data_ptr(), basis.data_ptr(), None if m is None else m.data_ptr(), c, s, f, t,
                  r, int(y.stride(0)), int(y.stride(1)), int(y.stride(2)), code, _stream(y))
    return b


def sub_mix(a, kernel, out=None):
    torch = _torch()
    _require_device(a)
    code = _dtype_code(a)
    if a.dim() != 4 or not a.is_contiguous():
        raise ValueError(f"a must be a contiguous tensor [C, S, R, F], got {tuple(a.shape)}")
    c, s, r, f = (int(n) for n in a.shape)
    _cgs_c128(kernel, (s, r, r), "kernel")
    z = torch.empty_like(a) if out is None else out
    if z is not a and (tuple(z.shape) != tuple(a.shape) or z.dtype != a.dtype or not z.is_contiguous() or z.device != a.device):
        raise ValueError("out must be contiguous with a's shape, dtype and device")
    if a.numel():
        _lib.call("xm_sub_mix", a.data_ptr(), z.data_ptr(), kernel.data_ptr(), c, s, f, r, code, _stream(a))
    return z


def sub_expand(u, basis):
    torch = _torch()
    r, t = _sub_basis(basis)
    if u.dim() != 3 or int(u.shape[1]) != r:
        raise ValueError(f"u must be [V, {r}, F], got {tuple(u.shape)}")
    v, _, f = (int(n) for n in u.shape)
    _cgs_c128(u, (v, r, f), "u")
    x = torch.empty((v, f, t), dtype=torch.complex128, device=u.device)
    if x.numel():
        _lib.call("xm_sub_expand", u.data_ptr(), basis.data_ptr(), x.data_ptr(), v, f, t, r, _stream(u))
    return x


class SubspaceSetup:

    __slots__ = ("basis", "sampling", "kernel", "kappa", "fraction")

    def __init__(self, **kw):
        for k, v in kw.items():
            setattr(self, k, v)


def subspace_setup(basis, sampling, weights, n_samples: int, device) -> SubspaceSetup:
    torch = _torch()
    V = basis if hasattr(basis, "detach") else torch.from_numpy(np.ascontiguousarray(basis, dtype=np.complex128))
    V = V.to(device=device, dtype=torch.complex128).contiguous()
    r, t = (int(n) for n in V.shape)
    if not 1 <= r <= SUB_MAX_RANK or r > t:
        raise ValueError(f"basis: rank {r} must be in 1 ... {SUB_MAX_RANK} and at most T = {t}")
    pairs = (V.conj()[:, None, :] * V[None, :, :]).reshape(r * r, t)
    if sampling is None:
        m, fraction = None, 1.0
        K = pairs.sum(dim=1).reshape(1, r, r).expand(int(n_samples), r, r).contiguous()
    else:
        m = torch.from_numpy(np.ascontiguousarray(sampling, dtype=np.uint8)).to(device)
        K = (m.to(torch.complex128) @ pairs.transpose(0, 1)).reshape(int(n_samples), r, r).contiguous()
        fraction = float(m.to(torch.float64).mean().item())
    w = torch.from_numpy(np.ascontiguousarray(weights, dtype=np.float64)).to(device)
    trace = torch.diagonal(K, dim1=1, dim2=2).real.sum(dim=1)
    kappa = float(((w * trace).sum() / (r * w.sum())).item())
    return SubspaceSetup(basis=V, sampling=m, kernel=K, kappa=kappa, fraction=fraction)


class SubspaceSense:

    __slots__ = ("x", "coefficients", "residual", "iterations", "status")

    def __init__(self, **kw):
        for k, v in kw.items():
            setattr(self, k, v)


def subspace_sense(y, s, adjoint, forward, setup: SubspaceSetup, lam: float, iterations: int, tol: float) -> SubspaceSense:
    c, n_s, f, _ = (int(n) for n in y.shape)
    v = int(s.shape[1])
    V, K = setup.basis, setup.kernel
    r = int(V.shape[0])
    b = sub_project(y, V, setup.sampling)
    s_rep = s.repeat_interleave(r, dim=1) if hasattr(s, "repeat_interleave") else np.repeat(s, r, axis=1)

    def adj(a):
        n = int(a.shape[2])
        return adjoint(a.reshape(c, n_s, r * n)).reshape(c, v * r, n)

    def fwd(u):
        n = int(u.shape[2])
        z = forward(u.reshape(c, v, r * n)).reshape(c, n_s, r, n)
        z = z.contiguous() if hasattr(z, "contiguous") else np.ascontiguousarray(z)
        return sub_mix(z, K, out=z).reshape(c, n_s * r, n)

    res = cg_sense(b.reshape(c, n_s * r, f), s_rep, adj, fwd, lam, iterations, tol)
    coef = res.x.reshape(v, r, f)
    return SubspaceSense(x=sub_expand(coef, V), coefficients=coef, residual=res.residual, iterations=res.iterations,
                         status=res.status)


def absmax_argmax(x):
    _require_device(x)
    torch = _torch()
    xc = x if x.is_contiguous() else x.contiguous()
    n = xc.shape[-1] if xc.dim() else 1
    x2 = xc.reshape(-1, n)
    nb = x2.shape[0]
    rd = _real_dtype(x)
    amax = torch.empty(nb, dtype=rd, device=x.device)
    aidx = torch.empty(nb, dtype=torch.int32, device=x.device)
    gmax = torch.empty(1, dtype=rd, device=x.device)
    gflat = torch.empty(1, dtype=torch.int64, device=x.device)
    code, st = _dtype_code(x), _stream(x)
    _lib.call("xm_absmax_rows", x2.data_ptr(), nb, n, amax.data_ptr(), aidx.data_ptr(), code, st)
    _lib.call("xm_argmax_reduce", amax.data_ptr(), aidx.data_ptr(), nb, n, gmax.data_ptr(), gflat.data_ptr(),
              code, st)
    return float(gmax.item()) ** 0.5, int(gflat.item())


class FusedResult:

    __slots__ = ("out", "absmax2", "argidx")

    def __init__(self, out, absmax2, argidx):
        self.out, self.absmax2, self.argidx = out, absmax2, argidx


def ramp_native(x2, n_out: int, pad_left: int = 0, shift_out: bool = True, ortho: bool = True) -> bool:
    _require_device(x2)
    flags = (_lib.XM_FFT_ORTHO if ortho else 0) | (_lib.XM_FFT_SHIFT_OUT if shift_out else 0)
    return bool(_lib.load().xm_pipeline_ramp_native(x2.data_ptr(), x2.shape[1], x2.shape[1], int(n_out), int(pad_left),
                                                    flags, _dtype_code(x2)))


def key_native(x2, n_out: int, pad_left: int = 0, shift_out: bool = True, ortho: bool = True) -> bool:
    _require_device(x2)
    flags = (_lib.XM_FFT_ORTHO if ortho else 0) | (_lib.XM_FFT_SHIFT_OUT if shift_out else 0)
    return x2.shape[0] >= 2 and bool(_lib.load().xm_pipeline_key_native(x2.data_ptr(), x2.shape[1], x2.shape[1], int(n_out),
                                                                       int(pad_left), flags, _dtype_code(x2)))


def pipeline_fused(x2, n_out: int, pad_left: int = 0, window=None, phase_table=None, shift_out: bool = True,
                   ortho: bool = True, want_out: bool = True, want_argmax: bool = False, out=None,
                   absmax2=None, argidx=None, argmax_value_only: bool = False, phase_ramp=None, global_key=None,
                   key_result=None):
    _require_device(x2)
    torch = _torch()
    if x2.dim() != 2 or not x2.is_contiguous():
        raise ValueError("pipeline_fused expects a contiguous [n_batch, n_in] tensor")
    nb, n_in = x2.shape
    rd = _real_dtype(x2)
    if want_out and out is None:
        out = torch.empty((nb, n_out), dtype=x2.dtype, device=x2.device)
    if global_key is not None:
        want_argmax, absmax2 = True, global_key
        argidx = key_result
    if want_argmax:
        if absmax2 is None:
            absmax2 = torch.empty(nb, dtype=rd, device=x2.device)
        if argidx is None and global_key is None:
            argidx = torch.empty(nb, dtype=torch.int32, device=x2.device)
    flags = (_lib.XM_FFT_ORTHO if ortho else 0) | (_lib.XM_FFT_SHIFT_OUT if shift_out else 0)
    if global_key is not None:
        flags |= _lib.XM_AMAX_GLOBAL_KEY | _lib.XM_AMAX_VALUE_ONLY
    if argmax_value_only:
        flags |= _lib.XM_AMAX_VALUE_ONLY
    if phase_ramp is not None:
        if phase_table is not None or not want_out:
            raise ValueError("phase_ramp excludes phase_table and needs an output")
        _lib.call(
            "xm_pipeline_fused_ramp", x2.data_ptr(), n_in, out.data_ptr(),
            window.data_ptr() if window is not None else None, float(phase_ramp[0]), float(phase_ramp[1]), nb, n_in,
            n_out, pad_left, flags, absmax2.data_ptr() if want_argmax else None,
            argidx.data_ptr() if (want_argmax and argidx is not None) else None, _dtype_code(x2), _stream(x2))
        return FusedResult(out, absmax2 if want_argmax else None, argidx if want_argmax else None)
    _lib.call(
        "xm_pipeline_fused", x2.data_ptr(), n_in, out.data_ptr() if want_out else None,
        window.data_ptr() if window is not None else None,
        phase_table.data_ptr() if phase_table is not None else None, nb, n_in, n_out, pad_left, flags,
        absmax2.data_ptr() if want_argmax else None,
        argidx.data_ptr() if (want_argmax and argidx is not None) else None, _dtype_code(x2), _stream(x2))
    return FusedResult(out if want_out else None, absmax2 if want_argmax else None,
                       argidx if want_argmax else None)


def row_l1(x2, window=None, pad_left: int = 0, out=None, n_used: int | None = None, sub_step: int = 1, key=None):
    _require_device(x2)
    torch = _torch()
    if x2.dim() != 2 or not x2.is_contiguous():
        raise ValueError("row_l1 expects a contiguous [n_batch, n_in] tensor")
    nb, n_in = x2.shape
    if out is None and key is None:
        out = torch.empty(nb, dtype=_real_dtype(x2), device=x2.device)
    n_sum = n_in if n_used is None else max(1, min(int(n_used), n_in))
    _lib.call("xm_row_l1", x2.data_ptr(), n_in, window.data_ptr() if window is not None else None, nb, n_sum,
              int(pad_left), max(1, int(sub_step)), out.data_ptr() if out is not None else None,
              key.data_ptr() if key is not None else None, _dtype_code(x2), _stream(x2))
    return out


def guess_supported(x2, n_out: int, pad_left: int = 0, shift_out: bool = True, ortho: bool = True) -> bool:
    _require_device(x2)
    if x2.dim() != 2 or not x2.is_contiguous():
        return False
    flags = (_lib.XM_FFT_ORTHO if ortho else 0) | (_lib.XM_FFT_SHIFT_OUT if shift_out else 0)
    return bool(_lib.load().xm_guess_supported(x2.data_ptr(), x2.shape[1], x2.shape[1], int(n_out), int(pad_left), flags,
                                               _dtype_code(x2)))


def guess_rows(x2, n_out: int, window32, est, key, n_guess: int = 0, shift_out: bool = True, ortho: bool = True):
    _require_device(x2)
    flags = (_lib.XM_FFT_ORTHO if ortho else 0) | (_lib.XM_FFT_SHIFT_OUT if shift_out else 0)
    nb, n_in = x2.shape
    _lib.call("xm_guess_rows", x2.data_ptr(), n_in, window32.data_ptr() if window32 is not None else None, nb, n_in,
              int(n_out), int(n_guess), flags, est.data_ptr(), key.data_ptr(), _dtype_code(x2), _stream(x2))
    return est


def guess_refine(x2, n_out: int, window32, est, guess_key, work_key, gmax, gflat, out_row, band: float = 0.75,
                 shift_out: bool = True, ortho: bool = True):
    _require_device(x2)
    flags = (_lib.XM_FFT_ORTHO if ortho else 0) | (_lib.XM_FFT_SHIFT_OUT if shift_out else 0)
    nb, n_in = x2.shape
    _lib.call("xm_guess_refine", x2.data_ptr(), n_in, window32.data_ptr() if window32 is not None else None, nb, n_in,
              int(n_out), flags, est.data_ptr(), guess_key.data_ptr(), float(band), work_key.data_ptr(),
              gmax.data_ptr(), gflat.data_ptr(), out_row.data_ptr(), _dtype_code(x2), _stream(x2))
    return out_row


def new_argmax_key(device):
    return _torch().zeros(131072 // 8, dtype=_torch().int64, device=device)


def new_key_result():
    return _torch().zeros(2, dtype=_torch().int64, pin_memory=True)


def read_key_result(rec, complex128: bool = False):
    m2 = rec.view(_torch().float64)[0] if complex128 else rec.view(_torch().float32)[0]
    return float(m2.item()), int(rec[1].item())


def argmax_key_take(key, n_per_row: int, gmax, gflat, x2=None, out_row=None):
    torch = _torch()
    if x2 is not None:
        _require_device(x2)
        if out_row is None:
            out_row = torch.empty((1, x2.shape[1]), dtype=torch.complex128, device=x2.device)
    st = torch.cuda.current_stream(key.device).cuda_stream
    _lib.call("xm_argmax_key_take", key.data_ptr(), int(n_per_row), gmax.data_ptr(), gflat.data_ptr(),
              x2.data_ptr() if x2 is not None else None, x2.shape[1] if x2 is not None else 0,
              x2.shape[1] if x2 is not None else 0, out_row.data_ptr() if x2 is not None else None,
              _dtype_code(x2) if x2 is not None else _lib.XM_C64, st)
    return out_row


def argmax_reduce(absmax2, argidx, n: int):
    torch = _torch()
    nb = absmax2.numel()
    gmax = torch.empty(1, dtype=absmax2.dtype, device=absmax2.device)
    gflat = torch.empty(1, dtype=torch.int64, device=absmax2.device)
    code = _lib.XM_C64 if absmax2.dtype == torch.float32 else _lib.XM_C128
    _lib.call("xm_argmax_reduce", absmax2.data_ptr(), argidx.data_ptr(), nb, n, gmax.data_ptr(),
              gflat.data_ptr(), code, torch.cuda.current_stream(absmax2.device).cuda_stream)
    return float(gmax.item()) ** 0.5, int(gflat.item())


def argmax_reduce_async(absmax2, argidx, n: int, gmax=None, gflat=None):
    torch = _torch()
    nb = absmax2.numel()
    if gmax is None:
        gmax = torch.empty(1, dtype=absmax2.dtype, device=absmax2.device)
    if gflat is None:
        gflat = torch.empty(1, dtype=torch.int64, device=absmax2.device)
    code = _lib.XM_C64 if absmax2.dtype == torch.float32 else _lib.XM_C128
    _lib.call("xm_argmax_reduce", absmax2.data_ptr(), argidx.data_ptr(), nb, n, gmax.data_ptr(),
              gflat.data_ptr(), code, torch.cuda.current_stream(absmax2.device).cuda_stream)
    return gmax, gflat


def gather_row_c128(x2, gflat, n_per_row: int, out=None):
    _require_device(x2)
    torch = _torch()
    nb, n_in = x2.shape
    if out is None:
        out = torch.empty((1, n_in), dtype=torch.complex128, device=x2.device)
    _lib.call("xm_gather_row_c128", x2.data_ptr(), n_in, n_in, gflat.data_ptr(), int(n_per_row), out.data_ptr(),
              _dtype_code(x2), _stream(x2))
    return out


def last_kernel() -> str:
    v = _lib.load().xm_last_kernel_string()
    return v.decode("utf-8", "replace") if v else ""


def fft_supported(n: int, complex128: bool = False) -> bool:
    if n == 1:
        return True
    return bool(_lib.load().xm_fft_supported(int(n), _lib.XM_C128 if complex128 else _lib.XM_C64))


SEARCH_RECORD_WORDS = 16


def search_supported(n: int, method: str = "acme", x_range: float = 1.0) -> bool:
    from .autophase_solver import METHODS

    return method in METHODS and bool(_lib.load().xm_search_supported(int(n), METHODS.index(method), float(x_range)))


def new_search_record():
    return _torch().zeros(SEARCH_RECORD_WORDS, dtype=_torch().int64, pin_memory=True)


def uniform_axis(coords):
    c = np.asarray(coords, dtype=np.float64)
    if c.size < 2:
        return None
    step = (c[-1] - c[0]) / (c.size - 1)
    rng = float(c.max() - c.min())
    if step == 0 or rng <= 0 or not np.all(np.abs(c - (c[0] + step * np.arange(c.size))) <= 4e-15 * rng):
        return None
    return float(c[0]), float(step), rng


def search_launch(slice_c128, axis, record, seq: int, p0_only: bool = False, seed: int = 42, tol: float = 0.01,
                  maxiter: int = 1000, stream=None):
    torch = _torch()
    n = slice_c128.numel()
    st = (stream if stream is not None else torch.cuda.current_stream()).cuda_stream
    _lib.call("xm_search_launch", slice_c128.data_ptr(), int(n), float(axis[0]), float(axis[1]), float(axis[2]), 0,
              int(bool(p0_only)), int(seed), float(tol), int(maxiter), int(seq), record.data_ptr(), st)


def search_done(record, seq: int) -> bool:
    return int(_lib.load().xm_atomic_load_acquire_i64(record.data_ptr() + 56)) == int(seq)


def read_search_record(record) -> dict:
    f = record.view(_torch().float64)
    i = record.view(_torch().int32)
    return dict(x=(float(f[0]), float(f[1])), fun=float(f[2]), pg_norm=float(f[3]), nfev=int(i[8]), nit=int(i[9]),
                status=int(i[10]), needs_polish=bool(int(i[11])), target_idx=int(i[12]),
                t_us=[float(v) for v in f[8:14]])


def search_eval(slice_c128, axis, xs, target_idx: int = -1, p0_only: bool = False):
    torch = _torch()
    xs_t = torch.as_tensor(np.ascontiguousarray(xs, dtype=np.float64)).reshape(-1, 2).to(slice_c128.device if slice_c128.is_cuda else "cuda")
    fs = torch.empty(xs_t.shape[0], dtype=torch.float64, device=xs_t.device)
    _lib.call("xm_search_eval", slice_c128.data_ptr(), int(slice_c128.numel()), float(axis[0]), float(axis[1]),
              float(axis[2]), int(target_idx), int(bool(p0_only)), xs_t.data_ptr(), int(xs_t.shape[0]), fs.data_ptr(),
              torch.cuda.current_stream().cuda_stream)
    return fs.cpu().numpy()


SEARCH_ALL_ZERO, SEARCH_NOT_FINITE = 2, 3
SEARCH_ROW_DTYPE = np.dtype([("x", "<f8", (2,)), ("fun", "<f8"), ("pg_norm", "<f8"), ("nfev", "<i4"), ("nit", "<i4"),
                             ("target_idx", "<i4"), ("status", "<i4"), ("needs_polish", "<i4"), ("pad_", "<i4")])


def search_rows_supported(n: int, method: str = "acme", x_range: float = 1.0, complex128: bool = False) -> bool:
    from .autophase_solver import METHODS

    return method in METHODS and bool(_lib.load().xm_search_rows_supported(
        int(n), METHODS.index(method), float(x_range), _lib.XM_C128 if complex128 else _lib.XM_C64))


def search_rows(x2d, axis, p0_only: bool = False, seed: int = 42, tol: float = 0.01, maxiter: int = 1000, pivot=None,
                target_idx: int = -1):
    _require_device(x2d)
    torch = _torch()
    if x2d.dim() != 2 or not x2d.is_contiguous():
        raise ValueError("search_rows expects a contiguous [n_rows, n] tensor")
    nb, n = x2d.shape
    rec = torch.empty((nb, SEARCH_ROW_DTYPE.itemsize), dtype=torch.uint8, device=x2d.device)
    _lib.call("xm_search_rows", x2d.data_ptr(), nb, n, _dtype_code(x2d), float(axis[0]), float(axis[1]), float(axis[2]),
              int(bool(p0_only)), int(seed), float(tol), int(maxiter), float("nan") if pivot is None else float(pivot),
              -1 if pivot is None else int(target_idx), rec.data_ptr(), _stream(x2d))
    return rec.cpu().numpy().view(SEARCH_ROW_DTYPE).reshape(nb)


def phase_apply_rows(x, axis: int, coords, p0, p1, pivot, skip=None, out=None):
    _require_device(x)
    torch = _torch()
    x2, restore = _rows(x, axis)
    nb, n = x2.shape
    lead = tuple(x.shape[:axis % x.dim()]) + tuple(x.shape[axis % x.dim() + 1:])
    c = np.array(coords, dtype=np.float64)
    if c.size != n:
        raise ValueError(f"coordinate axis has {c.size} points, data axis has {n}")

    def per_row(v, dtype):
        v = np.array(np.broadcast_to(np.asarray(v, dtype=dtype), lead))
        return torch.from_numpy(v.reshape(nb)).to(x.device)

    cd = torch.from_numpy(c).to(x.device)
    p0d, p1d, pvd = (per_row(v, np.float64) for v in (p0, p1, pivot))
    skd = per_row(np.asarray(skip) != 0, np.int32) if skip is not None else None
    if out is not None:
        if out is not x or x2.data_ptr() != x.data_ptr():
            raise ValueError("phase_apply_rows: `out` must be `x` itself, contiguous with `axis` last")
        y2 = x2
    else:
        y2 = torch.empty_like(x2)
    _lib.call("xm_phase_apply_rows", x2.data_ptr(), y2.data_ptr(), cd.data_ptr(), nb, n, p0d.data_ptr(), p1d.data_ptr(),
              pvd.data_ptr(), skd.data_ptr() if skd is not None else None, _dtype_code(x), _stream(x))
    return x if out is not None else restore(y2)


class ChipPartition:

    def __init__(self, device, reserved: int, n_search: int):
        import ctypes

        torch = _torch()
        self.device, self.reserved = device, int(reserved)
        self._handles = []

        def make(partition):
            h = ctypes.c_void_p()
            with torch.cuda.device(device):
                _lib.call("xm_stream_create", ctypes.byref(h), int(reserved), partition)
            self._handles.append(h.value)
            return torch.cuda.ExternalStream(h.value, device=device)

        self.compute = make(0)
        self.search = [make(1) for _ in range(int(n_search))]

    def another_search_stream(self):
        import ctypes

        h = ctypes.c_void_p()
        with _torch().cuda.device(self.device):
            _lib.call("xm_stream_create", ctypes.byref(h), self.reserved, 1)
        self._handles.append(h.value)
        st = _torch().cuda.ExternalStream(h.value, device=self.device)
        self.search.append(st)
        return st


_PARTITIONS = {}


def chip_partition(device, reserved: int, n_search: int) -> ChipPartition:
    torch = _torch()
    device = torch.device(device)
    key = (device.index if device.index is not None else torch.cuda.current_device(), int(reserved))
    part = _PARTITIONS.get(key)
    if part is None:
        part = _PARTITIONS[key] = ChipPartition(device, reserved, n_search)
    while len(part.search) < n_search:
        part.another_search_stream()
    return part


def replacement_search_stream(device, partition_streams):
    torch = _torch()
    if partition_streams is None:
        return torch.cuda.Stream(device=device)
    for part in _PARTITIONS.values():
        if partition_streams and partition_streams[0] in part.search:
            return part.another_search_stream()
    return torch.cuda.Stream(device=device)
```

xmris_amd/pipeline.py:

```python
from __future__ import annotations

from dataclasses import dataclass, field

import numpy as np

from . import autophase_solver as aps
from . import device as dev
from .cpu_budget import search_team as _search_team, search_workers as _search_workers
from .dims import MSG_POSITION


@dataclass
class PipelinePlan:

    n_in: int
    n_out: int
    pad_left: int
    time: np.ndarray
    freq: np.ndarray
    window_host: np.ndarray
    window: object = None
    window64: object = None
    extra: dict = field(default_factory=dict)


def zero_fill_coords(t: np.ndarray, target_points: int, pad_left: int) -> np.ndarray:
    delta = t[1] - t[0]
    if pad_left == 0:
        return t[0] + np.arange(target_points) * delta
    return (t[0] - (pad_left * delta)) + np.arange(target_points) * delta


def make_plan(x2, t: np.ndarray, target_points: int, lb, position: str = "end", window_host=None) -> PipelinePlan:
    import torch

    n_in = x2.shape[-1]
    t = np.asarray(t, dtype=np.float64)
    if target_points <= n_in:
        n_out, pad_left, tt = n_in, 0, t
    else:
        n_out = int(target_points)
        if position == "end":
            pad_left = 0
        elif position == "symmetric":
            pad_left = (n_out - n_in) // 2
        else:
            raise ValueError(MSG_POSITION)
        tt = zero_fill_coords(t, n_out, pad_left) if len(t) > 1 else t
    win = np.exp(-np.pi * lb * tt) if lb is not None else np.ones(n_out)
    if window_host is not None:
        win = np.asarray(window_host, dtype=np.float64)
        if win.shape != (n_out,):
            raise ValueError("window_host must cover the zero-filled axis")
    delta = (tt[1] - tt[0]) if len(tt) > 1 else 1.0
    freq = np.roll(np.fft.fftfreq(n_out, d=delta), n_out // 2)
    rd = torch.float32 if x2.dtype == torch.complex64 else torch.float64
    wdev = torch.from_numpy(np.ascontiguousarray(win)).to(device=x2.device, dtype=rd)
    return PipelinePlan(n_in, n_out, pad_left, tt, freq, win, wdev)


@dataclass
class AutophaseResult:
    p0: float
    p1: float
    pivot: float
    flat_index: int
    target_idx: int
    max_abs: float
    nfev: int = 0
    fun: float = float("nan")
    timing: dict = field(default_factory=dict)
    owner: int = 0
    mine: bool = True
    speculation: str = ""
    hedged: bool = False


def slice_on_host() -> bool:
    import os

    return os.environ.get("XMRIS_AMD_SLICE", "host") != "device"


def winner_spectrum(plan: "PipelinePlan", row) -> np.ndarray:
    n_out, n_in, pl = plan.n_out, plan.n_in, plan.pad_left
    row = np.asarray(row).reshape(-1)[:n_in]
    buf = np.zeros(n_out, dtype=np.complex128)
    buf[pl:pl + n_in] = row
    if plan.window_host is not None:
        buf = buf * np.asarray(plan.window_host, dtype=np.float64)
    return np.roll(np.fft.fft(buf, norm="ortho"), n_out // 2)


class Selection:

    @staticmethod
    def new_slot(x2, plan: "PipelinePlan", real_dtype):
        import torch

        return (torch.empty(1, dtype=real_dtype, pin_memory=True), torch.empty(1, dtype=torch.int64, pin_memory=True),
                torch.empty((1, plan.n_out), dtype=torch.complex128, pin_memory=True),
                torch.empty((1, x2.shape[1]), dtype=torch.complex128, device=x2.device),
                torch.empty((1, x2.shape[1]), dtype=torch.complex128, pin_memory=True))

    def __init__(self, x2, plan: "PipelinePlan", absmax2, argidx, index_from_slice: bool = False, key=None, slot=None,
                 refine=None, blocking=None):
        import torch

        n = plan.n_out
        self.index_from_slice = index_from_slice
        if plan.window64 is None:
            plan.window64 = torch.from_numpy(np.ascontiguousarray(plan.window_host)).to(x2.device, torch.float64)
        self.n = n
        rdt = absmax2.dtype if (key is None and refine is None) else torch.float32
        if slot is None:
            pool = plan.extra.setdefault("pinned", [])
            turn = plan.extra["turn"] = (plan.extra.get("turn", -1) + 1) % 2
            if len(pool) <= turn:
                pool.append(Selection.new_slot(x2, plan, rdt))
            slot = pool[turn]
        self.h_max, self.h_flat, self.h_slice, x1 = slot[:4]
        self.plan = plan
        self.h_row = slot[4] if (len(slot) > 4 and slice_on_host()) else None
        if self.h_row is not None:
            x1 = self.h_row
        if refine is not None:
            window32, est, gkey, wkey, band = refine
            dev.guess_refine(x2, n, window32, est, gkey, wkey, self.h_max, self.h_flat, x1, band=band)
        elif key is not None:
            dev.argmax_key_take(key, n, self.h_max, self.h_flat, x2, out_row=x1)
        else:
            dev.argmax_reduce_async(absmax2, argidx, n, gmax=self.h_max, gflat=self.h_flat)
            dev.gather_row_c128(x2, self.h_flat, n, out=x1)
        if self.h_row is None:
            dev.pipeline_fused(x1, n, plan.pad_left, window=plan.window64, out=self.h_slice)
        self.event = torch.cuda.Event(blocking=aps.scarce_cpus() if blocking is None else blocking)
        self.event.record()
        self._done = False

    def wait(self):
        self.event.synchronize()
        if self.h_row is not None and not self._done:
            self.h_slice[0].numpy()[:] = winner_spectrum(self.plan, self.h_row[0].numpy())
            self._done = True
        sl = self.h_slice[0].numpy().copy()
        flat = int(self.h_flat.item())
        if self.index_from_slice:
            flat = (flat // self.n) * self.n + int(np.argmax(np.abs(sl)))
        return float(self.h_max.item()) ** 0.5, flat, sl


def select_and_solve(x2, plan: PipelinePlan, absmax2, argidx, method="acme", peak_width=100, target_coord=None,
                     p0_only=False, exchange=None, rank_offset_rows=0, disp=False, on_host_phase=None,
                     selection: "Selection | None" = None, threads=None, polish="exact"):
    n = plan.n_out
    sl_ready = None
    if selection is not None:
        amax, flat, sl_ready = selection.wait()
    else:
        amax, flat = dev.argmax_reduce(absmax2, argidx, n)
    gflat = rank_offset_rows * n + flat
    mine = True
    if exchange is not None:
        mine, gflat = exchange(amax, gflat)
    k = gflat % n
    if target_coord is not None:
        target_idx = int(np.argmin(np.abs(plan.freq - target_coord)))
        pivot = float(target_coord)
    else:
        target_idx = int(k)
        pivot = float(plan.freq[k])
    res = AutophaseResult(0.0, 0.0, pivot, int(gflat), target_idx, amax)
    if mine:
        import torch

        if sl_ready is not None:
            sl = sl_ready
        else:
            row = gflat // n - rank_offset_rows
            x1 = x2[row:row + 1].to(torch.complex128)
            if plan.window64 is None:
                plan.window64 = torch.from_numpy(np.ascontiguousarray(plan.window_host)).to(x2.device, torch.float64)
            w64 = plan.window64
            sl = dev.pipeline_fused(x1, n, plan.pad_left, window=w64).out[0].cpu().numpy()
        if on_host_phase is not None:
            on_host_phase()
        iw = aps.index_width_of(plan.freq, peak_width)
        p0, p1, opt = aps.solve(sl, plan.freq, pivot, target_idx, iw, method=method, p0_only=p0_only, disp=disp,
                                threads=threads, polish=polish)
        res.p0, res.p1, res.nfev, res.fun = p0, p1, int(opt.nfev), float(opt.fun)
        res.timing = {"generations_ms": 1e3 * opt.get("t_generations", 0.0), "polish_ms": 1e3 * opt.get("t_polish", 0.0)}
    elif on_host_phase is not None:
        on_host_phase()
    return res, mine


def run(x2, t, target_points: int, lb: float, method: str = "acme", peak_width=100, target_coord=None,
        p0_only: bool = False, out=None, plan: PipelinePlan | None = None, params=None, polish: str | None = None):
    import os

    import torch

    if polish is None:
        polish = aps.default_polish()

    if plan is None:
        plan = make_plan(x2, t, target_points, lb)
    n = plan.n_out
    if (params is None and target_coord is None and os.environ.get("XMRIS_AMD_RUN_CLASSIC") is None
            and x2.dim() == 2 and x2.is_contiguous() and plan.window is not None
            and dev.guess_supported(x2, n, plan.pad_left) and dev.key_native(x2, n, plan.pad_left)):
        if out is None:
            out = torch.empty((x2.shape[0], n), dtype=x2.dtype, device=x2.device)
        res = run_stream([x2], [out], plan, method=method, peak_width=peak_width, p0_only=p0_only, speculate=True,
                         polish=polish)[0]
        return out, res, plan
    pre = dev.pipeline_fused(x2, n, plan.pad_left, window=plan.window, want_out=False, want_argmax=True,
                             argmax_value_only=params is None)
    if params is None:
        sel = Selection(x2, plan, pre.absmax2, pre.argidx, index_from_slice=True)
        res, _ = select_and_solve(x2, plan, pre.absmax2, pre.argidx, method, peak_width, target_coord, p0_only,
                                  selection=sel, threads=aps.burst_threads(), polish=polish)
    else:
        res = _selection_only(pre, plan, target_coord)
    if params is not None:
        res.p0, res.p1 = float(params[0]), float(params[1])
    main = main_pass(plan, x2, out, res.p0, res.p1, res.pivot)
    return main.out, res, plan


def run_stream(inputs, outputs, plan: PipelinePlan, *, exchange=None, broadcast=None, rank_offset_rows: int = 0,
               overlap: bool = True, method: str = "acme", peak_width=100, target_coord=None, p0_only: bool = False,
               trace: list | None = None, speculate: bool = False, polish: str | None = None):
    import time

    import torch

    n_sets = len(inputs)
    if polish is None:
        polish = aps.default_polish()
    if n_sets != len(outputs):
        raise ValueError("inputs and outputs must have the same length")
    if n_sets == 0:
        return []
    import gc

    gc_was_enabled = gc.isenabled()
    gc.disable()
    try:
        return _run_stream(inputs, outputs, plan, exchange, broadcast, rank_offset_rows, overlap, method, peak_width,
                           target_coord, p0_only, trace, speculate, polish)
    finally:
        if gc_was_enabled:
            gc.enable()


def _run_stream(inputs, outputs, plan, exchange, broadcast, rank_offset_rows, overlap, method, peak_width,
                target_coord, p0_only, trace, speculate, polish="exact"):
    import time

    import torch

    n_sets = len(inputs)
    if speculate:
        if target_coord is not None:
            raise ValueError("speculate=True needs the arg-max pivot (target_coord=None)")
        from . import stream

        return stream.run_speculative(inputs, outputs, plan, exchange, broadcast, rank_offset_rows, overlap, method,
                                      peak_width, p0_only, trace, polish)
    n = plan.n_out
    x0 = inputs[0]
    rd = torch.float32 if x0.dtype == torch.complex64 else torch.float64
    bufs = plan.extra.get(("stream_bufs", x0.shape[0], str(rd)))
    if bufs is None:
        bufs = plan.extra[("stream_bufs", x0.shape[0], str(rd))] = (
            [torch.empty(x0.shape[0], dtype=rd, device=x0.device) for _ in range(2)],
            [torch.empty(x0.shape[0], dtype=torch.int32, device=x0.device) for _ in range(2)])
    absmax2, argidx = bufs
    sel = [None, None]
    events = [dict() for _ in range(n_sets)]

    def prepass(i):
        b = i & 1
        ev = events[i]
        if trace is not None:
            ev["pre0"], ev["pre1"] = torch.cuda.Event(enable_timing=True), torch.cuda.Event(enable_timing=True)
            ev["pre0"].record()
        dev.pipeline_fused(inputs[i], n, plan.pad_left, window=plan.window, want_out=False, want_argmax=True,
                           absmax2=absmax2[b], argidx=argidx[b], argmax_value_only=True)
        if trace is not None:
            ev["pre1"].record()
        sel[b] = Selection(inputs[i], plan, absmax2[b], argidx[b], index_from_slice=True)

    results = []
    prepass(0)
    for i in range(n_sets):
        b = i & 1
        ev = events[i]
        ev["t_start"] = time.perf_counter()
        owner_box = [0]

        def merged(amax, gflat):
            if exchange is None:
                ev["t_exchanged"] = time.perf_counter()
                return True, gflat
            mine, gwin, owner = exchange(amax, gflat)
            owner_box[0] = owner
            ev["t_exchanged"] = time.perf_counter()
            return mine, gwin

        def queue_next():
            if overlap and i + 1 < n_sets:
                prepass(i + 1)

        res, mine = select_and_solve(inputs[i], plan, absmax2[b], argidx[b], method, peak_width, target_coord,
                                     p0_only, exchange=merged, rank_offset_rows=rank_offset_rows,
                                     on_host_phase=queue_next, selection=sel[b], polish=polish)
        if broadcast is not None:
            res.p0, res.p1 = broadcast([res.p0, res.p1], owner_box[0])
        res.owner, res.mine = owner_box[0], mine
        ev["t_solved"] = ev["t_table"] = time.perf_counter()
        if trace is not None:
            ev["main0"], ev["main1"] = torch.cuda.Event(enable_timing=True), torch.cuda.Event(enable_timing=True)
            ev["main0"].record()
        main_pass(plan, inputs[i], outputs[i], res.p0, res.p1, res.pivot)
        if trace is not None:
            ev["main1"].record()
        if not overlap and i + 1 < n_sets:
            prepass(i + 1)
        results.append(res)
        if trace is not None:
            trace.append(ev)
    return results


def phase_ramp_of(plan: PipelinePlan, p0: float, p1: float, pivot: float):
    lin = plan.extra.get("freq_linear")
    if lin is None:
        f = np.asarray(plan.freq, dtype=np.float64)
        ok = f.size >= 2
        if ok:
            step = (f[-1] - f[0]) / (f.size - 1)
            ok = step != 0 and bool(np.all(np.abs(f - (f[0] + step * np.arange(f.size))) <= 1e-12 * np.abs(f).max()))
        lin = plan.extra["freq_linear"] = (float(f[0]), float(step), float(f.max() - f.min())) if ok else False
    if lin is False:
        return None
    c0, step, rng = lin
    if rng == 0:
        return float(np.deg2rad(p0)), 0.0
    return (float(np.deg2rad(p0) + np.deg2rad(p1) * (c0 - pivot) / rng), float(np.deg2rad(p1) * step / rng))


def main_pass(plan: PipelinePlan, x2, out, p0: float, p1: float, pivot: float, **kw):
    native = plan.extra.get(("ramp_native", x2.data_ptr() & 15, x2.shape[1], str(x2.dtype)))
    if native is None:
        native = plan.extra[("ramp_native", x2.data_ptr() & 15, x2.shape[1], str(x2.dtype))] = dev.ramp_native(
            x2, plan.n_out, plan.pad_left)
    ramp = phase_ramp_of(plan, p0, p1, pivot) if native else None
    if ramp is not None:
        return dev.pipeline_fused(x2, plan.n_out, plan.pad_left, window=plan.window, phase_ramp=ramp, out=out, **kw)
    ph = upload_phase_table(plan, x2, p0, p1, pivot)
    return dev.pipeline_fused(x2, plan.n_out, plan.pad_left, window=plan.window, phase_table=ph, out=out, **kw)


def upload_phase_table(plan: PipelinePlan, like, p0: float, p1: float, pivot: float):
    import torch

    n = plan.n_out
    key = ("phase_stage", str(like.dtype))
    stage = plan.extra.get(key)
    if stage is None:
        stage = plan.extra[key] = [torch.empty(n, dtype=like.dtype, pin_memory=True) for _ in range(2)] + [0]
    stage[2] ^= 1
    host = stage[stage[2]]
    from . import _lib

    freq = plan.extra.get("freq_c")
    if freq is None:
        freq = plan.extra["freq_c"] = np.ascontiguousarray(plan.freq, dtype=np.float64)
    rc = _lib.load().xm_phase_table(freq.ctypes.data, n, float(p0), float(p1), float(pivot), host.data_ptr(),
                                    1 if like.dtype == torch.complex64 else 0)
    if rc:
        raise ValueError("xm_phase_table rejected its arguments")
    dev_t = plan.extra.setdefault(("phase_dev", str(like.dtype)),
                                  [torch.empty(n, dtype=like.dtype, device=like.device) for _ in range(2)])
    out = dev_t[stage[2]]
    out.copy_(host, non_blocking=True)
    return out


def _selection_only(pre, plan, target_coord):
    amax, flat = dev.argmax_reduce(pre.absmax2, pre.argidx, plan.n_out)
    k = flat % plan.n_out
    if target_coord is not None:
        return AutophaseResult(0.0, 0.0, float(target_coord), flat,
                               int(np.argmin(np.abs(plan.freq - target_coord))), amax)
    return AutophaseResult(0.0, 0.0, float(plan.freq[k]), flat, int(k), amax)
```

xmris_amd/stream.py:

```python
from __future__ import annotations

import os
import threading
import time
from concurrent.futures import FIRST_COMPLETED, ThreadPoolExecutor
from concurrent.futures import TimeoutError as FutureTimeout
from concurrent.futures import wait as wait_first
from dataclasses import dataclass
from typing import NamedTuple

import numpy as np
import torch

from . import _lib
from . import autophase_solver as aps
from . import cpu_budget
from . import device as dev
from .pipeline import AutophaseResult, Selection, main_pass, slice_on_host, winner_spectrum

_SUB_STEP = 8


def _look_ahead(workers: int, n_sets: int, overlap: bool, polish: str) -> int:
    if not overlap:
        return 0
    if n_sets <= 2:
        return 1
    extra = 3 if polish == "exact" else 0
    return min(workers + extra, n_sets - 1)


_ABANDONED_RECORDS = []


def _abandon(rec):
    _ABANDONED_RECORDS.append(rec)
    del _ABANDONED_RECORDS[:-256]



@dataclass(frozen=True)
class Schedule:

    workers: int
    team: int
    fill_team: int
    n_workers: int
    s_ahead: int
    s_look: int
    g_ahead: int
    ring: int
    cpu_fill: int
    use_dev: bool
    dev_ahead: int
    est_ms: float
    fast_fill: bool
    ramped: bool
    use_service: bool
    use_keys: bool
    use_guess: bool
    l1_keys: bool
    band: float
    n_used: int
    sub_step: int
    blocking: bool


def _uniform_axis(plan):
    axis = plan.extra.get("uniform_axis")
    if axis is None:
        axis = plan.extra["uniform_axis"] = dev.uniform_axis(plan.freq) or False
    return axis


def _device_engine_wanted(plan, method, polish, overlap) -> bool:
    want = os.environ.get("XMRIS_AMD_SEARCH", "auto")
    if want == "auto":
        local_world = cpu_budget.local_world()
        own_gpu = torch.cuda.device_count() >= local_world
        want = "device" if (cpu_budget.cpu_share() < 2 * local_world and own_gpu) else "host"
    axis = _uniform_axis(plan)
    return (want == "device" and polish == "exact" and method == "acme" and overlap and axis is not False
            and dev.search_supported(plan.n_out, method, axis[2]))


def _geometry(plan, x):
    k = ("geometry", x.data_ptr() & 15, tuple(x.shape), str(x.dtype), x.is_contiguous())
    g = plan.extra.get(k)
    if g is None:
        g = plan.extra[k] = (dev.key_native(x, plan.n_out, plan.pad_left), dev.guess_supported(x, plan.n_out, plan.pad_left))
    return g


def _window_weights(plan):
    return np.abs(np.asarray(plan.window_host, dtype=np.float64)[plan.pad_left:plan.pad_left + plan.n_in])


def _guess_band(plan) -> float:
    band = plan.extra.get("guess_band")
    if band is None:
        wabs = _window_weights(plan)
        inside = float(wabs[:512].sum()) / max(float(wabs.sum()), 1e-300)
        band = plan.extra["guess_band"] = float(min(0.95, max(0.4, 0.9 * inside)))
    return band


def _guess_n_used(plan) -> int:
    n_used = plan.extra.get("guess_n_used")
    if n_used is None:
        wabs = _window_weights(plan)
        total = float(wabs.sum())
        n_used = plan.n_in
        if total > 0:
            n_used = int(np.searchsorted(np.cumsum(wabs), (1.0 - 1e-3) * total)) + 1
            n_used = min(plan.n_in, max(256, -(-n_used // 256) * 256))
        plan.extra["guess_n_used"] = n_used
    return n_used


def make_schedule(inputs, plan, exchange, broadcast, overlap, method, polish) -> Schedule:
    n_sets, n, x0 = len(inputs), plan.n_out, inputs[0]
    workers, _ = cpu_budget.search_workers(plan, x0.shape[0], x0.element_size())
    use_dev = _device_engine_wanted(plan, method, polish, overlap)
    est_ms = 600 * (2.3 + 0.4 * n / 1000.0) * 1e-3
    dev_ahead = 0
    if use_dev:
        device_ms = x0.shape[0] * (plan.n_in + plan.n_out) * x0.element_size() / 5.5e9 + 0.12
        dev_ahead = int(min(24, max(3, -(-est_ms // device_ms) + 2)))
    if exchange is not None:
        if broadcast is not None:
            got = broadcast([float(workers), float(dev_ahead)], 0)
            workers, dev_ahead = int(round(got[0])), int(round(got[1]))
        else:
            workers, dev_ahead = 2, 0
        use_dev = dev_ahead > 0
    s_ahead = _look_ahead(workers, n_sets, overlap, polish)
    cpu_fill = min(n_sets, min(workers, s_ahead) + 1) if use_dev else n_sets
    use_dev = use_dev and cpu_fill < n_sets
    g_ahead = s_ahead + 1 if overlap else 0
    if use_dev:
        g_ahead = max(g_ahead, min(dev_ahead, n_sets - 1))
    s_look = s_ahead if not use_dev else (g_ahead if exchange is None else max(s_ahead, g_ahead - 1))
    n_workers = min(workers, s_ahead) if s_ahead >= 2 else 0
    fast_fill = exchange is None and not use_dev and overlap and n_sets > 2 and s_ahead >= 2
    c128 = x0.dtype == torch.complex128
    distinct = list({id(x): x for x in inputs}.values())
    use_keys = all(_geometry(plan, x)[0] for x in distinct)
    use_guess = (os.environ.get("XM_GUESS_L1") is None and plan.window is not None
                 and all(_geometry(plan, x)[1] for x in distinct))
    return Schedule(
        workers=workers, team=cpu_budget.search_team(n_workers) if n_workers else cpu_budget.stream_threads(),
        fill_team=cpu_budget.burst_threads(), n_workers=n_workers, s_ahead=s_ahead, s_look=s_look, g_ahead=g_ahead,
        ring=g_ahead + 2, cpu_fill=cpu_fill, use_dev=use_dev, dev_ahead=dev_ahead, est_ms=est_ms, fast_fill=fast_fill,
        ramped=overlap and not use_dev and not fast_fill,
        use_service=polish == "exact", use_keys=use_keys, use_guess=use_guess,
        l1_keys=use_keys and not c128 and not use_guess,
        band=_guess_band(plan), n_used=_guess_n_used(plan), sub_step=_SUB_STEP, blocking=cpu_budget.scarce_cpus())



@dataclass
class Ring:

    norm: list
    est: list
    wkey: object
    zero_idx: object
    tmax: list
    tidx: list
    vmax: list
    vflat: list
    gkey: list
    vkey: list
    vres: list
    sel_slots: list

    @staticmethod
    def of(plan, x0, s: Schedule) -> "Ring":
        rd = torch.float32 if x0.dtype == torch.complex64 else torch.float64
        nb, d = x0.shape[0], x0.device
        key = ("spec_bufs", nb, str(rd), s.ring, s.use_guess, s.use_keys, s.l1_keys)
        ring = plan.extra.get(key)
        if ring is None:
            slots = range(s.ring)
            sel_rd = torch.float32 if s.use_guess else rd
            ring = plan.extra[key] = Ring(
                norm=[None if (s.l1_keys or s.use_guess) else torch.empty(nb, dtype=rd, device=d) for _ in slots],
                est=[torch.empty(nb, dtype=torch.float32, device=d) if s.use_guess else None for _ in slots],
                wkey=dev.new_argmax_key(d) if s.use_guess else None,
                zero_idx=torch.zeros(nb, dtype=torch.int32, device=d),
                tmax=[None if s.use_keys else torch.empty(nb, dtype=rd, device=d) for _ in slots],
                tidx=[None if s.use_keys else torch.empty(nb, dtype=torch.int32, device=d) for _ in slots],
                vmax=[torch.empty(1, dtype=rd, pin_memory=True) for _ in slots],
                vflat=[torch.empty(1, dtype=torch.int64, pin_memory=True) for _ in slots],
                gkey=[dev.new_argmax_key(d) if (s.use_keys or s.use_guess) else None for _ in slots],
                vkey=[dev.new_argmax_key(d) if s.use_keys else None for _ in slots],
                vres=[dev.new_key_result() if s.use_keys else None for _ in slots],
                sel_slots=[Selection.new_slot(x0, plan, sel_rd) for _ in slots])
        return ring


class Records:

    def __init__(self, recs):
        self.recs, self.seq = recs, 0

    @staticmethod
    def of(plan, name, ring, new):
        r = plan.extra.get((name, ring))
        if r is None:
            r = plan.extra[(name, ring)] = Records([new() for _ in range(ring)])
        return r

    def next_seq(self) -> int:
        self.seq += 1
        return self.seq



@dataclass
class SearchOutcome:
    p0: float
    p1: float
    nfev: int
    fun: float
    timing: dict
    hedged: bool
    k: int


class Ticket(NamedTuple):

    handle: object
    sl: object
    k: int
    pivot: float


class Pending(NamedTuple):

    res: AutophaseResult | None
    engine: object
    ticket: Ticket | None


class Hedger:

    def __init__(self, plan, s: Schedule):
        self.enabled = os.environ.get("XMRIS_AMD_HEDGE", "1") != "0"
        self.gap = max(1, int(os.environ.get("XM_HEDGE_SPACING", "8")))
        self.run_hist = plan.extra.setdefault("search_run_hist", [])
        self.fill_hist = plan.extra.setdefault("fill_run_hist", [])
        self.last = -100
        self.n_out, self.team, self.fill_team = plan.n_out, s.team, s.fill_team

    def allowed(self, i: int) -> bool:
        return self.enabled and i - self.last >= self.gap

    def deadline(self, i: int, t_exchanged: float, scale: float, offset: float = 0.0) -> float:
        recent = (self.fill_hist if i == 0 else self.run_hist)[-9:]
        if len(recent) < 3:
            recent = [scale * cpu_budget.search_ms(self.n_out, self.fill_team if i == 0 else self.team) + offset]
        typical = sorted(recent)[len(recent) // 2]
        return t_exchanged + 2.0 * typical + 0.5e-3

    def record(self, i: int, seconds: float):
        hist = self.fill_hist if i == 0 else self.run_hist
        hist.append(seconds)
        del hist[:-16]


class PolishHandoff:

    def __init__(self, x: "Executor"):
        self.x, self.futs = x, {}
        pool = x.plan.extra.get("polish_pool")
        if pool is None:
            if os.environ.get("XM_POLISH_THREADS"):
                pool = ThreadPoolExecutor(max_workers=max(1, int(os.environ["XM_POLISH_THREADS"])),
                                          thread_name_prefix="xm-polish")
            elif x.n_sets > 4:
                pool = aps.polish_workers()
            if pool is not None:
                x.plan.extra["polish_pool"] = pool
        self.pool = pool

    def _args(self, j, k, x0):
        x = self.x
        sl = x.sel[j % x.s.ring].h_slice[0].numpy().copy()
        return (sl, x.plan.freq, float(x.plan.freq[k]), k, x.iw, x.method, x.p0_only, x0)

    def advance(self, pending):
        for j, p in pending.items():
            if j in self.futs or p.engine is None:
                continue
            rec = p.engine.record(j)
            if rec is None or not dev.search_done(rec, p.ticket.handle):
                continue
            r = dev.read_search_record(rec)
            if not r["needs_polish"] or self.pool is None:
                self.futs[j] = None
                continue
            args = self._args(j, r["target_idx"], r["x"])
            self.futs[j] = (self.pool.submit(aps.polish_reference, *args) if isinstance(self.pool, ThreadPoolExecutor)
                            else self.pool.submit(*args))

    def settle(self, i, r, k, out: SearchOutcome) -> SearchOutcome:
        if r["needs_polish"]:
            t0 = time.perf_counter()
            fut = self.futs.pop(i, None)
            x, fun, nfev_p, _ = fut.result() if fut is not None else aps.polish_reference(*self._args(i, k, r["x"]))
            out.p0, out.p1, out.fun, out.nfev = float(x[0]), (float(x[1]) if not self.x.p0_only else 0.0), fun, r["nfev"] + nfev_p
            out.timing["polish_ms"] = 1e3 * (time.perf_counter() - t0)
            out.timing["polish_route"] = "numpy"
        else:
            self.futs.pop(i, None)
        if self.x.p0_only:
            out.p1 = 0.0
        return out


def _record_outcome(r, p0_only, k, timing) -> SearchOutcome:
    p0, p1 = r["x"]
    return SearchOutcome(p0, p1, r["nfev"] + (1 if p0_only else 2) + 1, r["fun"], timing, False, k)


def _opt_outcome(p0, p1, opt, hedged, k) -> SearchOutcome:
    timing = {"generations_ms": 1e3 * opt.get("t_generations", 0.0), "polish_ms": 1e3 * opt.get("t_polish", 0.0)}
    return SearchOutcome(p0, p1, int(opt.nfev), float(opt.fun), timing, hedged, k)


class ServiceEngine:

    def __init__(self, x: "Executor"):
        self.x = x
        self.records = Records.of(x.plan, "host_search", x.s.ring, lambda: torch.zeros(dev.SEARCH_RECORD_WORDS, dtype=torch.int64))
        if x.plan.extra.get("freq_c") is None:
            x.plan.extra["freq_c"] = np.ascontiguousarray(x.plan.freq, dtype=np.float64)
        self.workers = max(1, x.s.n_workers)
        _lib.load().xm_hostsearch_set_workers(self.workers)

    def record(self, j):
        return self.records.recs[j % self.x.s.ring]

    def done(self, j, t: Ticket) -> bool:
        return dev.search_done(self.record(j), t.handle)

    def _submit(self, j, k, threads, rec, delay=0.0) -> int:
        x = self.x
        seq = self.records.next_seq()
        rec[7] = 0
        args = ("xm_hostsearch_submit", x.sel[j % x.s.ring].h_slice.data_ptr(), x.plan.n_out,
                x.plan.extra["freq_c"].ctypes.data, aps.METHODS.index(x.method), int(k), int(x.iw), int(bool(x.p0_only)),
                42, 0.01, 1000, int(threads), seq, rec.data_ptr())
        if delay:
            _abandon(rec)
            tm = threading.Timer(delay, _lib.call, args)
            tm.daemon = True
            tm.start()
        else:
            _lib.call(*args)
        return seq

    def submit(self, j, sl, k, pivot, threads) -> Ticket:
        return Ticket(self._submit(j, k, threads, self.record(j), self.x.slow_delay(j)), sl, k, pivot)

    def collect(self, i, t: Ticket, ev) -> SearchOutcome:
        x, h, b = self.x, self.x.hedger, i % self.x.s.ring
        rec = self.records.recs[b]
        deadline = h.deadline(i, ev["t_exchanged"], 3e-3, 1e-3)
        can_hedge, second, hedged, nap = h.allowed(i), None, False, 0.0
        give_up = time.perf_counter() + 120.0
        while not dev.search_done(rec, t.handle):
            if second is not None and dev.search_done(*second):
                _abandon(rec)
                self.records.recs[b] = torch.zeros(dev.SEARCH_RECORD_WORDS, dtype=torch.int64)
                rec = second[0]
                break
            now = time.perf_counter()
            if can_hedge and second is None and now > deadline:
                h.last, hedged = i, True
                spare = torch.zeros(dev.SEARCH_RECORD_WORDS, dtype=torch.int64)
                _abandon(spare)
                _lib.load().xm_hostsearch_set_workers(self.workers + 1)
                second = (spare, self._submit(i, t.k, x.s.fill_team, spare))
                _lib.load().xm_hostsearch_set_workers(self.workers)
            if now > give_up:
                raise RuntimeError("the search service did not answer within two minutes")
            nap = x.nap(nap)
        r = dev.read_search_record(rec)
        h.record(i, 1e-6 * r["t_us"][5])
        timing = {"generations_ms": 1e-3 * r["t_us"][0], "polish_ms": 1e-3 * (r["t_us"][5] - r["t_us"][0])}
        out = _record_outcome(r, x.p0_only, t.k, timing)
        out.hedged = hedged
        return x.polish.settle(i, r, t.k, out)


class ThreadEngine:

    def __init__(self, x: "Executor"):
        self.x, self.pool = x, None
        n_workers = x.s.n_workers
        if n_workers:
            self.pool = x.plan.extra.get(("search_pool", n_workers))
            if self.pool is None:
                self.pool = x.plan.extra[("search_pool", n_workers)] = ThreadPoolExecutor(
                    max_workers=n_workers + 1, thread_name_prefix="xm-search")

    def record(self, j):
        return None

    def done(self, j, t: Ticket) -> bool:
        return not hasattr(t.handle, "done") or t.handle.done()

    def submit(self, j, sl, k, pivot, threads) -> Ticket:
        x = self.x
        if self.pool is None:
            return Ticket(x.search(sl, k, pivot, threads, x.events[j]), sl, k, pivot)
        return Ticket(self.pool.submit(x.search, sl, k, pivot, threads, x.events[j], x.slow_delay(j)), sl, k, pivot)

    def collect(self, i, t: Ticket, ev) -> SearchOutcome:
        if self.pool is None:
            return _opt_outcome(*t.handle, False, t.k)
        (p0, p1, opt), hedged = self._wait(i, t, ev)
        if "t_search_end" in ev and "t_search_begin" in ev:
            self.x.hedger.record(i, ev["t_search_end"] - ev["t_search_begin"])
        return _opt_outcome(p0, p1, opt, hedged, t.k)

    def _wait(self, i, t: Ticket, ev):
        x, h, fut = self.x, self.x.hedger, t.handle
        if not h.allowed(i):
            return fut.result(), False
        try:
            return fut.result(timeout=max(h.deadline(i, ev["t_exchanged"], 1.5e-3) - time.perf_counter(), 0.0)), False
        except FutureTimeout:
            h.last = i
            hedge_pool = x.plan.extra.get("hedge_pool")
            if hedge_pool is None:
                hedge_pool = x.plan.extra["hedge_pool"] = ThreadPoolExecutor(max_workers=1, thread_name_prefix="xm-hedge")
            again = hedge_pool.submit(x.search, t.sl, t.k, t.pivot, x.s.fill_team, {})
            done, _ = wait_first([fut, again], return_when=FIRST_COMPLETED)
            return (fut.result() if fut in done else again.result()), True


class DeviceEngine:

    def __init__(self, x: "Executor", partition_streams):
        self.x, self.partition_streams = x, partition_streams
        self.records = Records.of(x.plan, "dev_search", x.s.ring, dev.new_search_record)
        self.streams = list(partition_streams)

    def record(self, j):
        return self.records.recs[j % self.x.s.ring]

    def done(self, j, t: Ticket) -> bool:
        return dev.search_done(self.record(j), t.handle)

    def submit(self, j, sl, k, pivot, threads, after=None) -> Ticket:
        x = self.x
        st = self.streams[j % len(self.streams)]
        if after is not None:
            st.wait_event(after)
        seq = self.records.next_seq()
        dev.search_launch(x.sel[j % x.s.ring].h_slice[0], _uniform_axis(x.plan), self.record(j), seq, p0_only=x.p0_only,
                          stream=st)
        x.events[j]["t_search_begin"] = time.perf_counter()
        return Ticket(seq, sl, k, pivot)

    def collect(self, i, t: Ticket, ev) -> SearchOutcome:
        x = self.x
        rec = self.record(i)
        deadline = time.perf_counter() + max(4.0 * x.s.est_ms * 1e-3, 8e-3)
        nap = 0.0
        while not dev.search_done(rec, t.handle):
            if time.perf_counter() > deadline:
                return self._overtake(i, rec)
            nap = x.nap(nap)
        ev["t_search_end"] = time.perf_counter()
        r = dev.read_search_record(rec)
        out = _record_outcome(r, x.p0_only, r["target_idx"], {"generations_ms": 1e-3 * r["t_us"][5], "polish_ms": 0.0,
                                                                "device": True})
        return x.polish.settle(i, r, out.k, out)

    def _overtake(self, i, rec) -> SearchOutcome:
        x = self.x
        sl = x.sel[i % x.s.ring].h_slice[0].numpy().copy()
        k = int(np.argmax(np.abs(sl)))
        p0, p1, opt = x.search(sl, k, float(x.plan.freq[k]), x.s.fill_team, {})
        s = i % len(self.streams)
        _abandon((rec, self.streams[s]))
        self.records.recs[i % x.s.ring] = dev.new_search_record()
        self.streams[s] = dev.replacement_search_stream(x.inputs[0].device, self.partition_streams)
        return _opt_outcome(p0, p1, opt, True, k)



class Executor:

    def __init__(self, inputs, outputs, plan, s: Schedule, exchange, broadcast, rank_offset_rows, method, peak_width,
                 p0_only, trace, polish, search_streams=None):
        self.t_call = time.perf_counter()
        self.inputs, self.outputs, self.plan, self.s = inputs, outputs, plan, s
        self.exchange, self.broadcast, self.rank_offset_rows = exchange, broadcast, rank_offset_rows
        self.method, self.p0_only, self.trace, self.polish_mode = method, p0_only, trace, polish
        self.n_sets, self.n = len(inputs), plan.n_out
        self.c128 = inputs[0].dtype == torch.complex128
        self.bufs = Ring.of(plan, inputs[0], s)
        if s.use_guess and plan.extra.get("window32") is None:
            plan.extra["window32"] = plan.window.to(torch.float32).contiguous()
        self.sel = [None] * s.ring
        self.events = [dict() for _ in range(self.n_sets)]
        self.results = [None] * self.n_sets
        self.iw = aps.index_width_of(plan.freq, peak_width)
        self.pending, self.dev_tickets, self.unverified = {}, {}, []
        self.guessed = self.started = -1
        slow = os.environ.get("XM_TEST_SLOW_SEARCH")
        self.slow_j, self.slow_s = (int(slow.split(",")[0]), 1e-3 * float(slow.split(",")[1])) if slow else (-1, 0.0)
        self.host = ServiceEngine(self) if s.use_service else ThreadEngine(self)
        self.polish = PolishHandoff(self)
        self.device = DeviceEngine(self, search_streams) if s.use_dev else None
        self.hedger = Hedger(plan, s)

    def slow_delay(self, j) -> float:
        return self.slow_s if j == self.slow_j and j >= 0 else 0.0

    def nap(self, nap: float) -> float:
        if self.s.blocking:
            nap = min(1e-4, nap + 1e-5)
            time.sleep(nap)
        return nap

    def search(self, sl, k, pivot, threads, ev, delay=0.0):
        ev["t_search_begin"] = time.perf_counter()
        if delay:
            time.sleep(delay)
        out = aps.solve(sl, self.plan.freq, pivot, k, self.iw, method=self.method, p0_only=self.p0_only, threads=threads,
                        polish=self.polish_mode)
        ev["t_search_end"] = time.perf_counter()
        return out

    def guess_next(self):
        self.guessed += 1
        j, s, bufs, plan = self.guessed, self.s, self.bufs, self.plan
        b, ev, x2 = j % s.ring, self.events[j], self.inputs[j]
        if self.trace is not None:
            ev["pre0"], ev["pre1"] = torch.cuda.Event(enable_timing=True), torch.cuda.Event(enable_timing=True)
            ev["pre0"].record()
        if s.use_guess:
            dev.guess_rows(x2, self.n, plan.extra["window32"], bufs.est[b], bufs.gkey[b])
        else:
            dev.row_l1(x2, plan.window, plan.pad_left, out=bufs.norm[b], n_used=s.n_used, sub_step=s.sub_step,
                       key=bufs.gkey[b] if s.l1_keys else None)
        if self.trace is not None:
            ev["pre1"].record()
            ev["guess_kernel"] = dev.last_kernel()
        self.sel[b] = Selection(x2, plan, bufs.norm[b], bufs.zero_idx, index_from_slice=True,
                                key=bufs.gkey[b] if s.l1_keys else None, slot=bufs.sel_slots[b],
                                refine=(plan.extra["window32"], bufs.est[b], bufs.gkey[b], bufs.wkey, s.band)
                                if s.use_guess else None, blocking=s.blocking)
        if self.trace is not None:
            ev["sel1"] = torch.cuda.Event(enable_timing=True)
            ev["sel1"].record()
        if s.use_dev and self.exchange is None and j >= s.cpu_fill and not slice_on_host():
            self.dev_tickets[j] = self.device.submit(j, None, -1, 0.0, 0, after=self.sel[b].event)

    def start_search(self, j):
        s, ev, n = self.s, self.events[j], self.n
        ev["t_start"] = time.perf_counter()
        on_dev = s.use_dev and j >= s.cpu_fill
        if on_dev and self.exchange is None and not slice_on_host():
            ev["t_exchanged"] = ev["t_start"]
            self.pending[j] = Pending(None, self.device, self.dev_tickets.pop(j))
            return
        amax, flat, sl = self.sel[j % s.ring].wait()
        ev["t_selected"] = time.perf_counter()
        gflat, mine, owner = self.rank_offset_rows * n + flat, True, 0
        if self.exchange is not None:
            mine, gflat, owner = self.exchange(amax, gflat)
        ev["t_exchanged"] = time.perf_counter()
        k = gflat % n
        res = AutophaseResult(0.0, 0.0, float(self.plan.freq[k]), int(gflat), int(k), amax)
        res.owner, res.mine = owner, mine
        if not mine:
            self.pending[j] = Pending(res, None, None)
            return
        engine = self.device if on_dev else self.host
        ticket = engine.submit(j, sl, int(k), res.pivot, s.fill_team if j == 0 else s.team)
        self.pending[j] = Pending(res, engine, ticket)

    def fill_one_rank(self):
        s, last = self.s, self.n_sets - 1
        while self.guessed < min(last, 1):
            self.guess_next()
        self.started = 0
        self.start_search(0)
        first = self.pending[0]
        while first.engine is not None and not first.engine.done(0, first.ticket):
            more_guesses = self.guessed < min(last, s.g_ahead)
            if more_guesses:
                self.guess_next()
            nxt = self.started + 1
            if nxt > min(last, s.s_look, 1):
                if more_guesses:
                    continue
                break
            if nxt <= self.guessed and self.sel[nxt % s.ring].event.query():
                self.started = nxt
                self.start_search(nxt)
            elif s.blocking and not more_guesses:
                time.sleep(2e-5)

    def look_ahead(self, i):
        s, last = self.s, self.n_sets - 1
        if i == 0 and s.fast_fill:
            self.fill_one_rank()
        ramp = 2 + 3 * i if s.ramped else self.n_sets
        while self.started < min(last, i + s.s_look, ramp):
            while self.guessed < min(last, self.started + 1):
                self.guess_next()
            self.started += 1
            self.start_search(self.started)
        while self.guessed < min(last, i + s.g_ahead):
            self.guess_next()

    def collect(self, i) -> AutophaseResult:
        ev, s, n = self.events[i], self.s, self.n
        if s.use_service or s.use_dev:
            self.polish.advance(self.pending)
        p = self.pending.pop(i)
        ev["t_collect"] = time.perf_counter()
        res = p.res
        if p.engine is not None:
            out = p.engine.collect(i, p.ticket, ev)
            if res is None:
                slot = self.bufs.sel_slots[i % s.ring]
                gflat = (self.rank_offset_rows + int(slot[1].item()) // n) * n + out.k
                res = AutophaseResult(0.0, 0.0, float(self.plan.freq[out.k]), int(gflat), int(out.k),
                                      float(slot[0].item()) ** 0.5)
            res.p0, res.p1, res.nfev, res.fun, res.timing, res.hedged = (out.p0, out.p1, out.nfev, out.fun, out.timing,
                                                                         out.hedged)
        if self.broadcast is not None:
            res.p0, res.p1 = self.broadcast([res.p0, res.p1], res.owner)
        ev["t_solved"] = ev["t_table"] = time.perf_counter()
        return res

    def queue_main(self, i, res):
        s, bufs, ev, b = self.s, self.bufs, self.events[i], i % self.s.ring
        if self.trace is not None:
            ev["main0"], ev["main1"] = torch.cuda.Event(enable_timing=True), torch.cuda.Event(enable_timing=True)
            ev["main0"].record()
        if s.use_keys:
            main_pass(self.plan, self.inputs[i], self.outputs[i], res.p0, res.p1, res.pivot, global_key=bufs.vkey[b],
                      key_result=bufs.vres[b])
        else:
            main_pass(self.plan, self.inputs[i], self.outputs[i], res.p0, res.p1, res.pivot, want_argmax=True,
                      absmax2=bufs.tmax[b], argidx=bufs.tidx[b], argmax_value_only=True)
        if self.trace is not None:
            ev["main1"].record()
            ev["main_kernel"] = dev.last_kernel()
        if not s.use_keys:
            dev.argmax_reduce_async(bufs.tmax[b], bufs.tidx[b], self.n, gmax=bufs.vmax[b], gflat=bufs.vflat[b])
        ev["verify_event"] = torch.cuda.Event(blocking=s.blocking)
        ev["verify_event"].record()

    def verify(self, i):
        b, n, plan, off = i % self.s.ring, self.n, self.plan, self.rank_offset_rows
        res, ev = self.results[i], self.events[i]
        ev["verify_event"].synchronize()
        if self.s.use_keys:
            m2, fl = dev.read_key_result(self.bufs.vres[b], self.c128)
            tmax, trow = m2 ** 0.5, fl // n
        else:
            tmax, trow = float(self.bufs.vmax[b].item()) ** 0.5, int(self.bufs.vflat[b].item()) // n
        g_row, owner, mine = off + trow, 0, True
        if self.exchange is not None:
            mine, gflat, owner = self.exchange(tmax, (off + trow) * n)
            g_row = gflat // n
        if g_row == res.flat_index // n:
            res.speculation = "hit"
            if mine:
                res.max_abs = tmax
            return
        vals = [0.0, 0.0, 0.0, 0.0]
        if mine:
            x1 = self.inputs[i][g_row - off:g_row - off + 1].to(torch.complex128)
            if plan.window64 is None:
                plan.window64 = torch.from_numpy(np.ascontiguousarray(plan.window_host)).to(x1.device, torch.float64)
            if slice_on_host():
                sl = winner_spectrum(plan, x1[0].cpu().numpy())
            else:
                sl = dev.pipeline_fused(x1, n, plan.pad_left, window=plan.window64).out[0].cpu().numpy()
            k = int(np.argmax(np.abs(sl)))
            p0, p1, opt = aps.solve(sl, plan.freq, float(plan.freq[k]), k, self.iw, method=self.method,
                                    p0_only=self.p0_only, polish=self.polish_mode)
            vals = [p0, p1, float(k), float(opt.nfev)]
        if self.broadcast is not None:
            vals = self.broadcast(vals, owner)
        p0, p1, k = float(vals[0]), float(vals[1]), int(vals[2])
        pivot = float(plan.freq[k])
        main_pass(plan, self.inputs[i], self.outputs[i], p0, p1, pivot)
        res.p0, res.p1, res.pivot, res.target_idx = p0, p1, pivot, k
        res.flat_index, res.max_abs, res.owner, res.mine = g_row * n + k, tmax, owner, mine
        res.nfev = int(vals[3]) if mine else 0
        res.speculation = "repaired"

    def run(self):
        self.events[0]["t_call"] = self.t_call
        for i in range(self.n_sets):
            self.look_ahead(i)
            res = self.results[i] = self.collect(i)
            out_i = self.outputs[i].data_ptr()
            while self.unverified and (self.unverified[0] <= i - 2
                                       or any(self.outputs[j].data_ptr() == out_i for j in self.unverified)):
                self.verify(self.unverified.pop(0))
            self.queue_main(i, res)
            self.unverified.append(i)
            if self.trace is not None:
                self.trace.append(self.events[i])
        self.events[-1]["t_last_queued"] = time.perf_counter()
        while self.unverified:
            self.verify(self.unverified.pop(0))
        self.events[-1]["t_return"] = time.perf_counter()
        return self.results


def run_speculative(inputs, outputs, plan, exchange, broadcast, rank_offset_rows, overlap, method, peak_width, p0_only,
                    trace, polish="exact"):
    s = make_schedule(inputs, plan, exchange, broadcast, overlap, method, polish)
    args = (inputs, outputs, plan, s, exchange, broadcast, rank_offset_rows, method, peak_width, p0_only, trace, polish)
    if not s.use_dev:
        return Executor(*args).run()
    x0 = inputs[0]
    reserved = int(min(32, 8 * -(-max(s.dev_ahead, 1) // 8)))
    part = dev.chip_partition(x0.device, reserved, n_search=min(16, max(s.dev_ahead, 1) + 2))
    caller = torch.cuda.current_stream(x0.device)
    part.compute.wait_stream(caller)
    try:
        with torch.cuda.stream(part.compute):
            return Executor(*args, search_streams=part.search).run()
    finally:
        caller.wait_stream(part.compute)
```

Before: 58.19 million.

## Fuse coarse guess of next set with refine of previous set in one kernel

Adds a fused guess-stage kernel. In one launch it runs the MFMA coarse estimate for the current dataset and the candidate refine/argmax pass for the previous dataset, with blocks doing coarse rows after or between their refine rows. The stream scheduler is reworked to pipeline selection one set behind guessing, with a larger ring and look-ahead. The aim is to cut kernel launches and to overlap the two passes so the device stays busy. In exchange it adds scheduler complexity, delays each selection by one stage, and is limited by a per-launch row cap.

New measurement: 55.73 million. 0.958x the previous value.

```diff
diff --git a/include/xmris_hip.h b/include/xmris_hip.h
--- a/include/xmris_hip.h
+++ b/include/xmris_hip.h
@@ -73,6 +73,12 @@
 int xm_guess_refine(const void* in, int64_t in_row_stride, const void* window, int64_t n_batch, int n_in, int n_out,
                     unsigned flags, const float* est, uint64_t* guess_key, float band, uint64_t* work_key,
                     float* out_max2, int64_t* out_flat, void* out_row, int dtype, void* stream);
+int xm_guess_stage_supported(const void* in, int64_t in_row_stride, int n_in, int n_out, int pad_left, unsigned flags,
+                             int dtype);
+int xm_guess_stage(const void* in, int64_t in_row_stride, const void* window, int64_t n_batch, int n_in, int n_out,
+                   unsigned flags, float* est, uint64_t* key, const void* refine_in, int64_t refine_n_batch,
+                   const float* refine_est, uint64_t* refine_guess_key, float band, uint64_t* work_key, float* out_max2,
+                   int64_t* out_flat, void* out_row, int dtype, void* stream);
 
 int xm_argmax_reduce(const void* absmax2, const int32_t* argidx, int64_t n_batch, int n, void* out_max2,
                      int64_t* out_flat, int dtype, void* stream);
diff --git a/xmris_amd/_lib.py b/xmris_amd/_lib.py
--- a/xmris_amd/_lib.py
+++ b/xmris_amd/_lib.py
@@ -128,6 +128,8 @@
     "xm_guess_supported": (_i, [_p, _l, _i, _i, _i, _u, _i]),
     "xm_guess_rows": (_i, [_p, _l, _p, _l, _i, _i, _i, _u, _p, _p, _i, _p]),
     "xm_guess_refine": (_i, [_p, _l, _p, _l, _i, _i, _u, _p, _p, ctypes.c_float, _p, _p, _p, _p, _i, _p]),
+    "xm_guess_stage_supported": (_i, [_p, _l, _i, _i, _i, _u, _i]),
+    "xm_guess_stage": (_i, [_p, _l, _p, _l, _i, _i, _u, _p, _p, _p, _l, _p, _p, ctypes.c_float, _p, _p, _p, _p, _i, _p]),
     "xm_phase_table": (_i, [_p, _i, ctypes.c_double, ctypes.c_double, ctypes.c_double, _p, _i]),
     "xm_solver_create": (_p, [_p, _p, _i, ctypes.c_double, _i, _i, _i]),
     "xm_solver_destroy": (None, [_p]),
diff --git a/xmris_amd/csrc/xm_api.hip b/xmris_amd/csrc/xm_api.hip
--- a/xmris_amd/csrc/xm_api.hip
+++ b/xmris_amd/csrc/xm_api.hip
@@ -586,6 +586,37 @@
                               (hipStream_t)stream);
 }
 
+int xm_guess_stage_supported(const void* in, int64_t in_row_stride, int n_in, int n_out, int pad_left, unsigned flags,
+                             int dtype) {
+  if (!xm_guess_supported(in, in_row_stride, n_in, n_out, pad_left, flags, dtype)) return 0;
+  return xm_zf2p_guess_stage_supported(in, in_row_stride, n_in, n_out, pad_left, flags, dtype);
+}
+
+int xm_guess_stage(const void* in, int64_t in_row_stride, const void* window, int64_t n_batch, int n_in, int n_out,
+                   unsigned flags, float* est, uint64_t* key, const void* refine_in, int64_t refine_n_batch,
+                   const float* refine_est, uint64_t* refine_guess_key, float band, uint64_t* work_key, float* out_max2,
+                   int64_t* out_flat, void* out_row, int dtype, void* stream) {
+  int rc = check_common(in, n_batch, n_out, dtype);
+  if (rc) return rc;
+  if (!est || !key || !window || n_batch < 1 || n_batch > 0xffffffffLL)
+    return fail(XM_ERR_INVALID_ARG, "guess_stage: null output, no window or bad sizes");
+  if (!xm_guess_stage_supported(in, in_row_stride, n_in, n_out, 0, flags, dtype))
+    return fail(XM_ERR_INVALID_ARG, "guess_stage: geometry outside xm_guess_stage_supported");
+  if (refine_in) {
+    if (!refine_est || !refine_guess_key || !work_key || work_key == refine_guess_key || work_key == key ||
+        refine_guess_key == key || refine_est == est || !out_flat || refine_n_batch < 1 || refine_n_batch > 0xffffffffLL ||
+        !(band > 0.0f && band <= 1.0f))
+      return fail(XM_ERR_INVALID_ARG, "guess_stage: refine job with a null or shared buffer, an empty batch or band outside (0, 1]");
+    if (!xm_guess_stage_supported(refine_in, in_row_stride, n_in, n_out, 0, flags, dtype))
+      return fail(XM_ERR_INVALID_ARG, "guess_stage: refine dataset outside xm_guess_stage_supported");
+  }
+  DeviceGuard guard(in);
+  return xm_zf2p_guess_stage(in, in_row_stride, (const float*)window, n_batch, n_in, n_out, flags, guess_scale(n_out, flags),
+                             est, (unsigned long long*)key, refine_in, refine_n_batch, refine_est,
+                             (unsigned long long*)refine_guess_key, band, (unsigned long long*)work_key, out_max2,
+                             (long long*)out_flat, out_row, dtype, (hipStream_t)stream);
+}
+
 int64_t xm_baseline_als_workspace_bytes(int64_t n_batch, int n) {
   if (n_batch < 0 || n < 0) return 0;
   return 5 * n_batch * (int64_t)n * (int64_t)sizeof(double);
diff --git a/xmris_amd/csrc/xm_coarse.h b/xmris_amd/csrc/xm_coarse.h
--- a/xmris_amd/csrc/xm_coarse.h
+++ b/xmris_amd/csrc/xm_coarse.h
@@ -37,11 +37,15 @@
   return u.v8;
 }
 
-template <bool IN64>
-__global__ __launch_bounds__(64 * kCoarseWaves, 2) void k_coarse_mfma(CoarseArgs A) {
+struct CoarseStride {
+  long long wave, n_waves;
+  XM_DEV long long first() const { return wave; }
+  XM_DEV long long next(long long s) { return s + n_waves; }
+};
+
+template <bool IN64, class SCHED>
+XM_DEV void coarse_rows(const CoarseArgs& A, SCHED sched) {
   const unsigned lane = threadIdx.x & 63u, r = lane & 31u, h = lane >> 5;
-  const long long wave = (long long)blockIdx.x * kCoarseWaves + (threadIdx.x >> 6);
-  const long long n_waves = (long long)gridDim.x * kCoarseWaves;
 
   xm_h8 b1r, b1i, b1n, a2r[2], a2i[2], a2n[2];
   {
@@ -105,11 +109,9 @@
   bool have = false;
   constexpr int DEPTH = 1;
   Cx<float> nx[DEPTH][8];
-  long long s = wave;
-#pragma unroll
-  for (int d = 0; d < DEPTH; ++d)
-    if (s + d * n_waves < A.n_batch) fetch(s + d * n_waves, nx[d]);
-  auto one_row = [&](Cx<float>* cur, long long s) {
+  long long s = sched.first();
+  if (s < A.n_batch) fetch(s, nx[0]);
+  auto one_row = [&](Cx<float>* cur, long long s) -> long long {
     float re[8], im[8];
     float m = 0.f;
 #pragma unroll
@@ -118,7 +120,8 @@
       im[j] = cur[j].im * wnd[j];
       m = fmaxf(m, fmaxf(fabsf(re[j]), fabsf(im[j])));
     }
-    if (s + DEPTH * n_waves < A.n_batch) fetch(s + DEPTH * n_waves, cur);
+    const long long s_nxt = sched.next(s);
+    if (s_nxt < A.n_batch) fetch(s_nxt, cur);
     unsigned e = (wave_reduce_u32<true>(__float_as_uint(m)) >> 23) & 0xffu;
     e = e > 253u ? 253u : (e < 1u ? 1u : e);
     const float up = __uint_as_float((254u - e) << 23);
@@ -161,13 +164,16 @@
     best_row = take ? row : best_row;
     have = true;
     if (lane == 0u) A.est[s] = __uint_as_float(key);
+    return s_nxt;
   };
-  for (; s < A.n_batch; s += DEPTH * n_waves) {
-#pragma unroll
-    for (int d = 0; d < DEPTH; ++d)
-      if (s + d * n_waves < A.n_batch) one_row(nx[d], s + d * n_waves);
-  }
+  while (s < A.n_batch) s = one_row(nx[0], s);
   if (A.gkey && have && lane == 0u)
     atomicMax(A.gkey + (blockIdx.x % XM_KEY_SLOTS) * XM_KEY_STRIDE,
               ((unsigned long long)best_key << 32) | (unsigned long long)(0xffffffffu - best_row));
 }
+
+template <bool IN64>
+__global__ __launch_bounds__(64 * kCoarseWaves, 2) void k_coarse_mfma(CoarseArgs A) {
+  const long long n_waves = (long long)gridDim.x * kCoarseWaves;
+  coarse_rows<IN64>(A, CoarseStride{(long long)blockIdx.x * kCoarseWaves + (threadIdx.x >> 6), n_waves});
+}
diff --git a/xmris_amd/csrc/xm_guess_fused.h b/xmris_amd/csrc/xm_guess_fused.h
--- /dev/null
+++ b/xmris_amd/csrc/xm_guess_fused.h
@@ -0,0 +1,49 @@
+#pragma once
+#include "xm_coarse.h"
+#include "xm_zf2p.h"
+
+constexpr int kGuessFusedThreads = 64 * kCoarseWaves;
+
+template <class PL, bool IN64>
+constexpr size_t guess_fused_group_lds() {
+  using FFT = BlockFFT<xm_f2, PL, zf2p_pad_shift<PL, !IN64>()>;
+  const size_t b = (size_t)FFT::lds_elems() * sizeof(Cx<xm_f2>) + (size_t)HotTw<float, PL>::mid_lds_size() * sizeof(Cx<float>) +
+                   ((size_t)PL::NT / XM_WAVE + 2) * (sizeof(float) + sizeof(int)) + zf2p_cand_lds_bytes();
+  return (b + 15u) & ~(size_t)15u;
+}
+
+template <bool IN64>
+struct GuessFusedHooks {
+  static constexpr bool kLateTables = true;
+  const CoarseArgs& C;
+  bool done;
+  XM_DEV void coarse() {
+    const long long n_waves = (long long)gridDim.x * kCoarseWaves;
+    coarse_rows<IN64>(C, CoarseStride{(long long)blockIdx.x * kCoarseWaves + (threadIdx.x >> 6), n_waves});
+    done = true;
+  }
+  XM_DEV void deferred() { coarse(); }
+  XM_DEV void after_rows() {
+    if (!done) coarse();
+  }
+};
+
+template <class PL, int IN64>
+__global__ __launch_bounds__(kGuessFusedThreads, 2) void k_guess_fused(PipeArgs<float> R, CoarseArgs C) {
+  static_assert(kGuessFusedThreads % PL::NT == 0, "whole groups");
+  extern __shared__ __attribute__((aligned(16))) char xm_smem[];
+  GuessFusedHooks<IN64 != 0> hooks{C, false};
+  if (R.in == nullptr) {
+    hooks.coarse();
+    return;
+  }
+  constexpr size_t GB = guess_fused_group_lds<PL, IN64 != 0>();
+  const unsigned grp = threadIdx.x / PL::NT;
+  using FFT = BlockFFT<xm_f2, PL, zf2p_pad_shift<PL, !IN64>()>;
+  constexpr size_t kNextOff = (size_t)FFT::lds_elems() * sizeof(Cx<xm_f2>) +
+                              (size_t)HotTw<float, PL>::mid_lds_size() * sizeof(Cx<float>) +
+                              ((size_t)PL::NT / XM_WAVE + 1) * (sizeof(float) + sizeof(int));
+  unsigned* lead_next = reinterpret_cast<unsigned*>(xm_smem + kNextOff);
+  zf2p_body<PL, ZF2_AMAX, ZF2P_CAND | (IN64 ? ZF2P_IN64 : ZF2P_LOAD16)>(R, xm_smem + (size_t)grp * GB, threadIdx.x % PL::NT,
+                                                                        grp == 0u, lead_next, hooks);
+}
diff --git a/xmris_amd/csrc/xm_guess_fused.hip b/xmris_amd/csrc/xm_guess_fused.hip
--- /dev/null
+++ b/xmris_amd/csrc/xm_guess_fused.hip
@@ -0,0 +1,113 @@
+#include "xm_host.h"
+#include "xm_plans.h"
+#include "xm_tables.h"
+#include "xm_guess_fused.h"
+
+#include <cstring>
+#include <string>
+
+namespace {
+
+using T = float;
+constexpr int kGuessHalf = 512;
+
+int half_table(int n, const Cx<T>** out) {
+  const void* half = nullptr;
+  const int rc = xm_table_get(TK_HALF, n, 0, XM_C64, xm_gen_half, nullptr, &half);
+  *out = (const Cx<T>*)half;
+  return rc;
+}
+
+}
+
+namespace {
+
+template <class PL, int IN64>
+int launch_fused(PipeArgs<T> R, CoarseArgs C, hipStream_t st) {
+  if (R.in) {
+    const void* tw = nullptr;
+    const int rc = xm_table_get(TK_TWIDDLE, PL::N, PL::signature(), XM_C64, xm_gen_twiddles<PL>, nullptr, &tw);
+    if (rc) return rc;
+    R.tw = (const Cx<T>*)tw;
+  }
+  const size_t lds = guess_fused_group_lds<PL, IN64 != 0>() * (size_t)(kGuessFusedThreads / PL::NT);
+  static XmResidency res;
+  int resident = 0;
+  int rc = xm_resident_blocks(res, k_guess_fused<PL, IN64>, kGuessFusedThreads, lds, &resident, st);
+  if (rc) return rc;
+  long long want = (C.n_batch + kCoarseWaves - 1) / kCoarseWaves;
+  if (R.in && R.n_batch > want) want = R.n_batch;
+  const long long blocks = want < 1 ? 1 : (want < resident ? want : resident);
+  if (R.in && (R.n_batch + blocks - 1) / blocks > ZF2P_CAND_KMAX)
+    return xm_fail(XM_ERR_INVALID_ARG, "guess_stage: too many rows for one launch");
+  if (R.in) {
+    rc = xm_queue_slot(&R.queue);
+    if (rc) return rc;
+  }
+  xm_note_kernel("k_guess_fused", &typeid(PL), nullptr, IN64, -1);
+  hipLaunchKernelGGL((k_guess_fused<PL, IN64>), dim3((unsigned)blocks), dim3(kGuessFusedThreads), lds, st, R, C);
+  HIP_TRY(hipGetLastError());
+  return XM_OK;
+}
+
+template <int IN64>
+int fused_plan(int h, const PipeArgs<T>& R, const CoarseArgs& C, hipStream_t st) {
+  switch (h) {
+    case 512: return launch_fused<typename Zf2PlanOf<512>::type, IN64>(R, C, st);
+    case 1024: return launch_fused<typename Zf2PlanOf<1024>::type, IN64>(R, C, st);
+    case 2048: return launch_fused<typename Zf2PlanOf<2048>::type, IN64>(R, C, st);
+    case 4096: return launch_fused<typename PlanOf<4096>::type, IN64>(R, C, st);
+    default: break;
+  }
+  return xm_fail(XM_ERR_UNSUPPORTED_N, "guess_stage: no plan for half length " + std::to_string(h));
+}
+
+}
+
+int xm_zf2p_guess_stage_supported(const void* in, int64_t in_stride, int n_in, int n_out, int pad_left, unsigned flags,
+                                  int dtype) {
+  if (!xm_zf2p_guess_supported(in, in_stride, n_in, n_out, pad_left, flags, dtype)) return 0;
+  return n_in >= kGuessHalf && n_out / 2 <= 4096;
+}
+
+int xm_zf2p_guess_stage(const void* in, int64_t in_stride, const float* window, int64_t n_batch, int n_in, int n_out,
+                        unsigned flags, float scale, float* est, unsigned long long* key, const void* r_in,
+                        int64_t r_n_batch, const float* r_est, unsigned long long* r_guess_key, float band,
+                        unsigned long long* work_key, float* out_max2, long long* out_flat, void* out_row, int dtype,
+                        hipStream_t st) {
+  CoarseArgs C;
+  int rc = half_table(2 * kGuessHalf, &C.w1024);
+  if (rc) return rc;
+  C.in = in;
+  C.window = window;
+  C.est = est;
+  C.gkey = key;
+  C.in_stride = in_stride;
+  C.n_batch = n_batch;
+  C.scale2 = scale * scale;
+  PipeArgs<T> R;
+  std::memset(&R, 0, sizeof(R));
+  if (r_in) {
+    R.in = (const Cx<T>*)r_in;
+    R.window = window;
+    R.in_stride = in_stride;
+    R.n_batch = r_n_batch;
+    R.n = n_out;
+    R.n_in = n_in;
+    R.out_shift = (flags & XM_FFT_SHIFT_OUT) ? n_out / 2 : 0;
+    R.amax_value_only = 1;
+    R.scale = scale;
+    R.gkey = work_key;
+    R.gbest = reinterpret_cast<unsigned*>(work_key) + XM_KEY_GBEST_WORD;
+    R.gkey_in = r_guess_key;
+    R.est = const_cast<float*>(r_est);
+    R.absmax2 = const_cast<float*>(r_est);
+    R.band2 = band * band;
+    R.take_max2 = out_max2;
+    R.take_flat = out_flat;
+    R.take_row = (Cx<double>*)out_row;
+    rc = half_table(n_out, &R.aux);
+    if (rc) return rc;
+  }
+  return dtype == XM_C64 ? fused_plan<0>(n_out / 2, R, C, st) : fused_plan<1>(n_out / 2, R, C, st);
+}
diff --git a/xmris_amd/csrc/xm_host.h b/xmris_amd/csrc/xm_host.h
--- a/xmris_amd/csrc/xm_host.h
+++ b/xmris_amd/csrc/xm_host.h
@@ -78,6 +78,13 @@
                          unsigned flags, float scale, const float* est, unsigned long long* guess_key, float band,
                          unsigned long long* work_key, float* out_max2, long long* out_flat, void* out_row, int dtype,
                          hipStream_t st);
+int xm_zf2p_guess_stage_supported(const void* in, int64_t in_stride, int n_in, int n_out, int pad_left, unsigned flags,
+                                  int dtype);
+int xm_zf2p_guess_stage(const void* in, int64_t in_stride, const float* window, int64_t n_batch, int n_in, int n_out,
+                        unsigned flags, float scale, float* est, unsigned long long* key, const void* r_in,
+                        int64_t r_n_batch, const float* r_est, unsigned long long* r_guess_key, float band,
+                        unsigned long long* work_key, float* out_max2, long long* out_flat, void* out_row, int dtype,
+                        hipStream_t st);
 
 int xm_queue_slot(unsigned** out);
 
diff --git a/xmris_amd/csrc/xm_zf2p.h b/xmris_amd/csrc/xm_zf2p.h
--- a/xmris_amd/csrc/xm_zf2p.h
+++ b/xmris_amd/csrc/xm_zf2p.h
@@ -20,8 +20,72 @@
   return PL::radix(0) == 8 ? 4 : xm_ilog2(2 * PL::radix(0));
 }
 
-template <class PL, int MODE, int OPT>
-__global__ __launch_bounds__(PL::NT, (zf2_waves<float, PL>())) void k_zf2p(PipeArgs<float> A) {
+template <unsigned NT>
+XM_DEV unsigned zf2p_cand_scan(const PipeArgs<float>& A, unsigned* lds_next, const unsigned t) {
+  unsigned* cand = lds_next + ZF2P_CAND_ROWS;
+  float* cand_e = reinterpret_cast<float*>(lds_next + ZF2P_CAND_EST);
+  unsigned* cand_n = lds_next + ZF2P_CAND_COUNT;
+  unsigned* top_bits = lds_next + ZF2P_CAND_TOP;
+  unsigned* bitmap = lds_next + ZF2P_CAND_BITMAP;
+  const unsigned G = gridDim.x, b = blockIdx.x;
+  const unsigned kmax = (unsigned)((A.n_batch + G - 1) / G);
+  for (unsigned i = t; i < (kmax + 31u) / 32u; i += NT) bitmap[i] = 0u;
+  if (t < XM_WAVE) {
+    const unsigned long long k = __hip_atomic_load(A.gkey_in + t * XM_KEY_STRIDE, __ATOMIC_RELAXED, __HIP_MEMORY_SCOPE_AGENT);
+    const unsigned hi = wave_reduce_u32<true>((unsigned)(k >> 32));
+    if (t == 0) *top_bits = hi;
+  }
+  __syncthreads();
+  const float thr = A.band2 * __uint_as_float(*top_bits);
+  for (unsigned k = t; k < kmax; k += NT) {
+    const long long r = (long long)k * G + (b + 37u * k) % G;
+    if (r < A.n_batch) {
+      const float e = A.est[r];
+      if (e >= thr || e != e) atomicOr(&bitmap[k >> 5], 1u << (k & 31u));
+    }
+  }
+  __syncthreads();
+  if (t == 0) {
+    unsigned n = 0;
+    for (unsigned w = 0; w < (kmax + 31u) / 32u; ++w) {
+      unsigned bits = bitmap[w];
+      while (bits) {
+        const unsigned k = w * 32u + (unsigned)__builtin_ctz(bits);
+        bits &= bits - 1u;
+        const unsigned r = (unsigned)((long long)k * G + (b + 37u * k) % G);
+        float e = A.est[r];
+        e = e != e ? __builtin_inff() : e;
+        unsigned pos = n;
+        while (pos > 0 && cand_e[pos - 1] < e) --pos;
+        if (pos >= (unsigned)ZF2P_CAND_CAP) continue;
+        const unsigned top = n < (unsigned)ZF2P_CAND_CAP ? n : (unsigned)ZF2P_CAND_CAP - 1u;
+        for (unsigned i = top; i > pos; --i) {
+          cand[i] = cand[i - 1];
+          cand_e[i] = cand_e[i - 1];
+        }
+        cand[pos] = r;
+        cand_e[pos] = e;
+        n = n < (unsigned)ZF2P_CAND_CAP ? n + 1u : n;
+      }
+    }
+    *cand_n = n;
+  }
+  __syncthreads();
+  return (unsigned)__builtin_amdgcn_readfirstlane((int)*cand_n);
+}
+
+struct Zf2pNap {
+  static constexpr bool kLateTables = false;
+  XM_DEV void deferred() {
+#pragma unroll 1
+    for (int i = 0; i < 3; ++i) __builtin_amdgcn_s_sleep(127);
+  }
+  XM_DEV void after_rows() {}
+};
+
+template <class PL, int MODE, int OPT, class HOOKS>
+XM_DEV void zf2p_body(const PipeArgs<float>& A, char* xm_smem, const unsigned t, const bool lead, unsigned* lead_next,
+                      HOOKS&& hooks) {
   using T = float;
   using V = xm_f2;
   constexpr unsigned N = 2 * PL::N, NT = PL::NT;
@@ -39,122 +103,20 @@
   static_assert(P % 2 == 0 && NT >= XM_WAVE, "pair loads need an even number of points per thread, whole waves");
   using FFT = BlockFFT<V, PL, zf2p_pad_shift<PL, L16>()>;
   using HT = HotTw<T, PL, RAMP>;
-  extern __shared__ __attribute__((aligned(16))) char xm_smem[];
   Cx<V>* lds = reinterpret_cast<Cx<V>*>(xm_smem);
   Cx<T>* mid = reinterpret_cast<Cx<T>*>(lds + FFT::lds_elems());
   T* red_v = reinterpret_cast<T*>(mid + HT::mid_lds_size());
   int* red_i = reinterpret_cast<int*>(red_v + NT / XM_WAVE + 1);
   unsigned* lds_next = reinterpret_cast<unsigned*>(red_i + NT / XM_WAVE + 1);
   constexpr bool QUEUE = (OPT & ZF2P_QUEUE) != 0;
-  const unsigned t = threadIdx.x;
   const unsigned lane = t & (XM_WAVE - 1), half = lane >> 5;
   const unsigned col = L16 ? (t & ~(XM_WAVE - 1u)) + 2u * (lane & 31u) + half : t;
 
   long long n_rows = A.n_batch;
   unsigned* cand = lds_next + ZF2P_CAND_ROWS;
   const unsigned n_in = (unsigned)A.n_in;
-  if constexpr (CAND) {
-    float* cand_e = reinterpret_cast<float*>(lds_next + ZF2P_CAND_EST);
-    unsigned* cand_n = lds_next + ZF2P_CAND_COUNT;
-    unsigned* top_bits = lds_next + ZF2P_CAND_TOP;
-    unsigned* bitmap = lds_next + ZF2P_CAND_BITMAP;
-    const unsigned G = gridDim.x, b = blockIdx.x;
-    const unsigned kmax = (unsigned)((A.n_batch + G - 1) / G);
-    for (unsigned i = t; i < (kmax + 31u) / 32u; i += NT) bitmap[i] = 0u;
-    if (t < XM_WAVE) {
-      const unsigned long long k = __hip_atomic_load(A.gkey_in + t * XM_KEY_STRIDE, __ATOMIC_RELAXED, __HIP_MEMORY_SCOPE_AGENT);
-      const unsigned hi = wave_reduce_u32<true>((unsigned)(k >> 32));
-      if (t == 0) *top_bits = hi;
-    }
-    __syncthreads();
-    const float thr = A.band2 * __uint_as_float(*top_bits);
-    for (unsigned k = t; k < kmax; k += NT) {
-      const long long r = (long long)k * G + (b + 37u * k) % G;
-      if (r < A.n_batch) {
-        const float e = A.est[r];
-        if (e >= thr || e != e) atomicOr(&bitmap[k >> 5], 1u << (k & 31u));
-      }
-    }
-    __syncthreads();
-    if (t == 0) {
-      unsigned n = 0;
-      for (unsigned w = 0; w < (kmax + 31u) / 32u; ++w) {
-        unsigned bits = bitmap[w];
-        while (bits) {
-          const unsigned k = w * 32u + (unsigned)__builtin_ctz(bits);
-          bits &= bits - 1u;
-          const unsigned r = (unsigned)((long long)k * G + (b + 37u * k) % G);
-          float e = A.est[r];
-          e = e != e ? __builtin_inff() : e;
-          unsigned pos = n;
-          while (pos > 0 && cand_e[pos - 1] < e) --pos;
-          if (pos >= (unsigned)ZF2P_CAND_CAP) continue;
-          const unsigned top = n < (unsigned)ZF2P_CAND_CAP ? n : (unsigned)ZF2P_CAND_CAP - 1u;
-          for (unsigned i = top; i > pos; --i) {
-            cand[i] = cand[i - 1];
-            cand_e[i] = cand_e[i - 1];
-          }
-          cand[pos] = r;
-          cand_e[pos] = e;
-          n = n < (unsigned)ZF2P_CAND_CAP ? n + 1u : n;
-        }
-      }
-      *cand_n = n;
-    }
-    __syncthreads();
-    n_rows = (long long)(unsigned)__builtin_amdgcn_readfirstlane((int)*cand_n);
-  }
-  const bool live = !CAND || n_rows > 0;
-
-  HT tw;
-  tw.mid = HT::mid_in_lds() ? mid : A.tw;
-  if (live) {
-    tw.load(A.tw, (int)t);
-    for (unsigned i = t; i < (unsigned)HT::mid_lds_size(); i += NT) mid[i] = A.tw[i];
-  }
-  if constexpr (RAMP) {
-    double sn, cs;
-    sincos(A.ramp_db * (double)(2u * t), &sn, &cs);
-    tw.fold(mk<T>((T)cs, (T)sn));
-  }
-  Cx<T> rot = live ? A.aux[col] : mk<T>(T(0), T(0));
-  if constexpr (RAMP) rot = rot * mk<T>(A.ramp_e[0], A.ramp_e[1]);
-  const unsigned coff = col - (unsigned)A.pad_left;
-  T w[P];
-#pragma unroll
-  for (int q = 0; q < P; ++q) {
-    const bool ok = live && (coff + NT * q) < n_in;
-    w[q] = ok ? (A.window ? A.window[col + NT * q] * A.scale : A.scale) : T(0);
-  }
-  __syncthreads();
-
-  constexpr int NRAW = L16 ? P / 2 : P;
-  typedef unsigned raw_t __attribute__((ext_vector_type((L16 || IN64) ? 4 : 2)));
-  raw_t raw[NRAW];
-  const unsigned e0 = (t & ~(XM_WAVE - 1u)) + 2u * (lane & 31u) + NT * half - (unsigned)A.pad_left;
-  auto fetch = [&](long long s2, unsigned ee0, unsigned cc, unsigned nin) {
-    constexpr size_t EB = IN64 ? 16u : 8u;
-    const char* __restrict__ row = reinterpret_cast<const char*>(A.in) + (size_t)(s2 * A.in_stride) * EB;
-    if constexpr (L16) {
-#pragma unroll
-      for (int j = 0; j < P / 2; ++j) {
-        const unsigned e = min(ee0 + 2u * NT * j, nin - 2u);
-        raw[j] = __builtin_nontemporal_load(reinterpret_cast<const raw_t*>(row + (size_t)e * 8u));
-      }
-    } else {
-#pragma unroll
-      for (int q = 0; q < P; ++q) {
-        const unsigned e = min(cc + NT * q, nin - 1u);
-        raw[q] = *reinterpret_cast<const raw_t*>(row + (size_t)e * EB);
-      }
-    }
-  };
-  unsigned best_key = 0, best_row = 0;
-  bool have = false;
-  auto rowid = [&](long long v) -> long long {
-    if constexpr (CAND) return (long long)(unsigned)__builtin_amdgcn_readfirstlane((int)cand[v]);
-    else return v;
-  };
+  if constexpr (CAND) n_rows = (long long)zf2p_cand_scan<NT>(A, lds_next, t);
+
   unsigned gb_seen = 0;
   auto next_live = [&](long long v) -> long long {
     if constexpr (CAND) {
@@ -167,29 +129,85 @@
     }
     return v;
   };
+  auto first_candidate = [&]() -> long long {
+    long long s0 = 0;
+    if (n_rows > 0) {
+      const float* cand_e = reinterpret_cast<const float*>(lds_next + ZF2P_CAND_EST);
+      const float top = __uint_as_float((unsigned)__builtin_amdgcn_readfirstlane((int)__float_as_uint(cand_e[0])));
+      const float emax2 = __uint_as_float((unsigned)__builtin_amdgcn_readfirstlane((int)lds_next[ZF2P_CAND_TOP]));
+      if (top < 0.81f * emax2) {
+        hooks.deferred();
+        if (t < XM_WAVE) {
+          const long long nx = next_live(0);
+          if (t == 0u) *lds_next = (unsigned)nx;
+        }
+        __syncthreads();
+        s0 = (long long)(unsigned)__builtin_amdgcn_readfirstlane((int)*lds_next);
+        __syncthreads();
+      }
+    }
+    return s0;
+  };
+  constexpr bool LATE = CAND && std::remove_reference<HOOKS>::type::kLateTables;
+  long long s_first = 0;
+  if constexpr (LATE) s_first = first_candidate();
+  const bool live = !CAND || s_first < n_rows;
+
+  HT tw;
+  tw.mid = HT::mid_in_lds() ? mid : A.tw;
+  if (live) {
+    tw.load(A.tw, (int)t);
+    for (unsigned i = t; i < (unsigned)HT::mid_lds_size(); i += NT) mid[i] = A.tw[i];
+  }
+  if constexpr (RAMP) {
+    double sn, cs;
+    sincos(A.ramp_db * (double)(2u * t), &sn, &cs);
+    tw.fold(mk<T>((T)cs, (T)sn));
+  }
+  Cx<T> rot = live ? A.aux[col] : mk<T>(T(0), T(0));
+  if constexpr (RAMP) rot = rot * mk<T>(A.ramp_e[0], A.ramp_e[1]);
+  const unsigned coff = col - (unsigned)A.pad_left;
+  T w[P];
+#pragma unroll
+  for (int q = 0; q < P; ++q) {
+    const bool ok = live && (coff + NT * q) < n_in;
+    w[q] = ok ? (A.window ? A.window[col + NT * q] * A.scale : A.scale) : T(0);
+  }
+  __syncthreads();
+
+  constexpr int NRAW = L16 ? P / 2 : P;
+  typedef unsigned raw_t __attribute__((ext_vector_type((L16 || IN64) ? 4 : 2)));
+  raw_t raw[NRAW];
+  const unsigned e0 = (t & ~(XM_WAVE - 1u)) + 2u * (lane & 31u) + NT * half - (unsigned)A.pad_left;
+  auto fetch = [&](long long s2, unsigned ee0, unsigned cc, unsigned nin) {
+    constexpr size_t EB = IN64 ? 16u : 8u;
+    const char* __restrict__ row = reinterpret_cast<const char*>(A.in) + (size_t)(s2 * A.in_stride) * EB;
+    if constexpr (L16) {
+#pragma unroll
+      for (int j = 0; j < P / 2; ++j) {
+        const unsigned e = min(ee0 + 2u * NT * j, nin - 2u);
+        raw[j] = __builtin_nontemporal_load(reinterpret_cast<const raw_t*>(row + (size_t)e * 8u));
+      }
+    } else {
+#pragma unroll
+      for (int q = 0; q < P; ++q) {
+        const unsigned e = min(cc + NT * q, nin - 1u);
+        raw[q] = *reinterpret_cast<const raw_t*>(row + (size_t)e * EB);
+      }
+    }
+  };
+  unsigned best_key = 0, best_row = 0;
+  bool have = false;
+  auto rowid = [&](long long v) -> long long {
+    if constexpr (CAND) return (long long)(unsigned)__builtin_amdgcn_readfirstlane((int)cand[v]);
+    else return v;
+  };
   const long long ch = (!CAND && A.queue_chunk > 0) ? A.queue_chunk : 1;
   const long long c_first = CAND ? 0 : blockIdx.x, c_step = CAND ? 1 : gridDim.x;
   long long c_cur = c_first, c_nxt = c_cur + c_step, c_nn = c_nxt + c_step;
   long long s = c_cur * ch;
   unsigned off = 0;
-  if constexpr (CAND) {
-    if (n_rows > 0) {
-      const float* cand_e = reinterpret_cast<const float*>(lds_next + ZF2P_CAND_EST);
-      const float top = __uint_as_float((unsigned)__builtin_amdgcn_readfirstlane((int)__float_as_uint(cand_e[0])));
-      const float emax2 = __uint_as_float((unsigned)__builtin_amdgcn_readfirstlane((int)lds_next[ZF2P_CAND_TOP]));
-      if (top < 0.81f * emax2) {
-#pragma unroll 1
-        for (int i = 0; i < 3; ++i) __builtin_amdgcn_s_sleep(127);
-        if (t < XM_WAVE) {
-          const long long nx = next_live(0);
-          if (t == 0u) *lds_next = (unsigned)nx;
-        }
-        __syncthreads();
-        s = (long long)(unsigned)__builtin_amdgcn_readfirstlane((int)*lds_next);
-        __syncthreads();
-      }
-    }
-  }
+  if constexpr (CAND) s = LATE ? s_first : first_candidate();
   if (s < n_rows) fetch(rowid(s), e0, coff, n_in);
   if constexpr (QUEUE) {
     if (t == 0) *lds_next = atomicAdd(A.queue, 1u) + gridDim.x;
@@ -344,6 +362,7 @@
     }
     s = s_nxt;
   }
+  hooks.after_rows();
   if constexpr (AMAX) {
     if (A.gkey && have && lane == 0u)
       atomicMax(A.gkey + (blockIdx.x % XM_KEY_SLOTS) * XM_KEY_STRIDE,
@@ -357,17 +376,18 @@
       __syncthreads();
     }
     unsigned last = 0;
-    if (t == 0) {
+    unsigned* fin = lead_next ? lead_next : lds_next;
+    if (t == 0 && lead) {
       const unsigned d = atomicAdd(A.queue + 1, 1u);
       last = d == gridDim.x - 1u;
       if (last) {
         __hip_atomic_store(A.queue, 0u, __ATOMIC_RELAXED, __HIP_MEMORY_SCOPE_AGENT);
         __hip_atomic_store(A.queue + 1, 0u, __ATOMIC_RELAXED, __HIP_MEMORY_SCOPE_AGENT);
       }
-      if constexpr (CAND) *lds_next = last;
+      if constexpr (CAND) *fin = last;
     }
     if constexpr (AMAX) {
-      if (decode && t < XM_WAVE) {
+      if (decode && lead && t < XM_WAVE) {
         last = (unsigned)__builtin_amdgcn_readfirstlane((int)last);
         if (last) {
           unsigned long long k = __hip_atomic_load(A.gkey + t * XM_KEY_STRIDE, __ATOMIC_RELAXED, __HIP_MEMORY_SCOPE_AGENT);
@@ -391,7 +411,7 @@
             if constexpr (CAND) {
               if (A.take_max2) A.take_max2[0] = __uint_as_float((unsigned)(k >> 32));
               A.take_flat[0] = (long long)row * (long long)N;
-              cand[0] = row;
+              fin[ZF2P_CAND_ROWS] = row;
             }
           }
         }
@@ -399,8 +419,8 @@
       if constexpr (CAND) {
         if (decode) {
           __syncthreads();
-          if (*lds_next != 0u && A.take_row) {
-            const size_t r = (size_t)cand[0] * (size_t)A.in_stride;
+          if (*fin != 0u && A.take_row && lead) {
+            const size_t r = (size_t)fin[ZF2P_CAND_ROWS] * (size_t)A.in_stride;
             for (unsigned j = t; j < n_in; j += NT) {
               if constexpr (IN64) {
                 A.take_row[j] = reinterpret_cast<const Cx<double>*>(A.in)[r + j];
@@ -415,3 +435,9 @@
     }
   }
 }
+
+template <class PL, int MODE, int OPT>
+__global__ __launch_bounds__(PL::NT, (zf2_waves<float, PL>())) void k_zf2p(PipeArgs<float> A) {
+  extern __shared__ __attribute__((aligned(16))) char xm_smem[];
+  zf2p_body<PL, MODE, OPT>(A, xm_smem, threadIdx.x, true, nullptr, Zf2pNap{});
+}
diff --git a/xmris_amd/device.py b/xmris_amd/device.py
--- a/xmris_amd/device.py
+++ b/xmris_amd/device.py
@@ -1824,6 +1824,32 @@
     return out_row
 
 
+def guess_stage_supported(x2, n_out: int, pad_left: int = 0, shift_out: bool = True, ortho: bool = True) -> bool:
+    if not getattr(x2, "is_cuda", False) or x2.dim() != 2 or not x2.is_contiguous():
+        return False
+    flags = (_lib.XM_FFT_ORTHO if ortho else 0) | (_lib.XM_FFT_SHIFT_OUT if shift_out else 0)
+    return bool(_lib.load().xm_guess_stage_supported(x2.data_ptr(), x2.shape[1], x2.shape[1], int(n_out), int(pad_left),
+                                                     flags, _dtype_code(x2)))
+
+
+def guess_stage(x2, n_out: int, window32, est, key, refine=None, shift_out: bool = True, ortho: bool = True):
+    _require_device(x2)
+    flags = (_lib.XM_FFT_ORTHO if ortho else 0) | (_lib.XM_FFT_SHIFT_OUT if shift_out else 0)
+    nb, n_in = x2.shape
+    if refine is None:
+        r = (None, 0, None, None, 0.75, None, None, None, None)
+    else:
+        rx, r_est, r_gkey, r_wkey, gmax, gflat, out_row, band = refine
+        _require_device(rx)
+        if rx.shape[1] != n_in or rx.dtype != x2.dtype or not rx.is_contiguous():
+            raise ValueError("guess_stage: the dataset to refine must have the rows' length, dtype and layout")
+        r = (rx.data_ptr(), rx.shape[0], r_est.data_ptr(), r_gkey.data_ptr(), float(band), r_wkey.data_ptr(),
+             gmax.data_ptr(), gflat.data_ptr(), out_row.data_ptr())
+    _lib.call("xm_guess_stage", x2.data_ptr(), n_in, window32.data_ptr(), nb, n_in, int(n_out), flags, est.data_ptr(),
+              key.data_ptr(), *r, _dtype_code(x2), _stream(x2))
+    return est
+
+
 def new_argmax_key(device):
     return _torch().zeros(131072 // 8, dtype=_torch().int64, device=device)
 
diff --git a/xmris_amd/pipeline.py b/xmris_amd/pipeline.py
--- a/xmris_amd/pipeline.py
+++ b/xmris_amd/pipeline.py
@@ -104,7 +104,7 @@
                 torch.empty((1, x2.shape[1]), dtype=torch.complex128, pin_memory=True))
 
     def __init__(self, x2, plan: "PipelinePlan", absmax2, argidx, index_from_slice: bool = False, key=None, slot=None,
-                 refine=None, blocking=None):
+                 refine=None, blocking=None, queued: bool = False):
         import torch
 
         n = plan.n_out
@@ -124,7 +124,9 @@
         self.h_row = slot[4] if (len(slot) > 4 and slice_on_host()) else None
         if self.h_row is not None:
             x1 = self.h_row
-        if refine is not None:
+        if queued:
+            pass
+        elif refine is not None:
             window32, est, gkey, wkey, band = refine
             dev.guess_refine(x2, n, window32, est, gkey, wkey, self.h_max, self.h_flat, x1, band=band)
         elif key is not None:
@@ -137,6 +139,12 @@
         self.event = torch.cuda.Event(blocking=aps.scarce_cpus() if blocking is None else blocking)
         self.event.record()
         self._done = False
+
+    @staticmethod
+    def refine_job(x2, slot, refine):
+        window32, est, gkey, wkey, band = refine
+        x1 = slot[4] if (len(slot) > 4 and slice_on_host()) else slot[3]
+        return (x2, est, gkey, wkey, slot[0], slot[1], x1, band)
 
     def wait(self):
         self.event.synchronize()
diff --git a/xmris_amd/stream.py b/xmris_amd/stream.py
--- a/xmris_amd/stream.py
+++ b/xmris_amd/stream.py
@@ -59,6 +59,7 @@
     use_service: bool
     use_keys: bool
     use_guess: bool
+    fused: bool
     l1_keys: bool
     band: float
     n_used: int
@@ -148,12 +149,14 @@
     use_keys = all(_geometry(plan, x)[0] for x in distinct)
     use_guess = (os.environ.get("XM_GUESS_L1") is None and plan.window is not None
                  and all(_geometry(plan, x)[1] for x in distinct))
+    fused = (use_guess and len({(tuple(x.shape), x.dtype) for x in distinct}) == 1
+             and all(dev.guess_stage_supported(x, plan.n_out, plan.pad_left) for x in distinct))
     return Schedule(
         workers=workers, team=cpu_budget.search_team(n_workers) if n_workers else cpu_budget.stream_threads(),
         fill_team=cpu_budget.burst_threads(), n_workers=n_workers, s_ahead=s_ahead, s_look=s_look, g_ahead=g_ahead,
-        ring=g_ahead + 2, cpu_fill=cpu_fill, use_dev=use_dev, dev_ahead=dev_ahead, est_ms=est_ms, fast_fill=fast_fill,
+        ring=g_ahead + (3 if fused else 2), cpu_fill=cpu_fill, use_dev=use_dev, dev_ahead=dev_ahead, est_ms=est_ms, fast_fill=fast_fill,
         ramped=overlap and not use_dev and not fast_fill,
-        use_service=polish == "exact", use_keys=use_keys, use_guess=use_guess,
+        use_service=polish == "exact", use_keys=use_keys, use_guess=use_guess, fused=fused,
         l1_keys=use_keys and not c128 and not use_guess,
         band=_guess_band(plan), n_used=_guess_n_used(plan), sub_step=_SUB_STEP, blocking=cpu_budget.scarce_cpus())
 
@@ -513,7 +516,8 @@
         self.results = [None] * self.n_sets
         self.iw = aps.index_width_of(plan.freq, peak_width)
         self.pending, self.dev_tickets, self.unverified = {}, {}, []
-        self.guessed = self.started = -1
+        self.guessed = self.started = self.selected = -1
+        self.g_ahead = s.g_ahead + (1 if s.fused else 0)
         slow = os.environ.get("XM_TEST_SLOW_SEARCH")
         self.slow_j, self.slow_s = (int(slow.split(",")[0]), 1e-3 * float(slow.split(",")[1])) if slow else (-1, 0.0)
         self.host = ServiceEngine(self) if s.use_service else ThreadEngine(self)
@@ -546,7 +550,10 @@
         if self.trace is not None:
             ev["pre0"], ev["pre1"] = torch.cuda.Event(enable_timing=True), torch.cuda.Event(enable_timing=True)
             ev["pre0"].record()
-        if s.use_guess:
+        if s.fused:
+            job = Selection.refine_job(self.inputs[j - 1], bufs.sel_slots[(j - 1) % s.ring], self.refine_args(j - 1)) if j else None
+            dev.guess_stage(x2, self.n, plan.extra["window32"], bufs.est[b], bufs.gkey[b], refine=job)
+        elif s.use_guess:
             dev.guess_rows(x2, self.n, plan.extra["window32"], bufs.est[b], bufs.gkey[b])
         else:
             dev.row_l1(x2, plan.window, plan.pad_left, out=bufs.norm[b], n_used=s.n_used, sub_step=s.sub_step,
@@ -554,15 +561,35 @@
         if self.trace is not None:
             ev["pre1"].record()
             ev["guess_kernel"] = dev.last_kernel()
-        self.sel[b] = Selection(x2, plan, bufs.norm[b], bufs.zero_idx, index_from_slice=True,
-                                key=bufs.gkey[b] if s.l1_keys else None, slot=bufs.sel_slots[b],
-                                refine=(plan.extra["window32"], bufs.est[b], bufs.gkey[b], bufs.wkey, s.band)
-                                if s.use_guess else None, blocking=s.blocking)
+        first = self.selected + 1
+        if s.fused:
+            if j:
+                self.select(j - 1, queued=True)
+            if j == self.n_sets - 1:
+                self.select(j)
+        else:
+            self.select(j)
         if self.trace is not None:
             ev["sel1"] = torch.cuda.Event(enable_timing=True)
             ev["sel1"].record()
-        if s.use_dev and self.exchange is None and j >= s.cpu_fill and not slice_on_host():
-            self.dev_tickets[j] = self.device.submit(j, None, -1, 0.0, 0, after=self.sel[b].event)
+        if s.use_dev and self.exchange is None and not slice_on_host():
+            for k in range(max(first, s.cpu_fill), self.selected + 1):
+                self.dev_tickets[k] = self.device.submit(k, None, -1, 0.0, 0, after=self.sel[k % s.ring].event)
+
+    def refine_args(self, j):
+        bufs, b = self.bufs, j % self.s.ring
+        return (self.plan.extra["window32"], bufs.est[b], bufs.gkey[b], bufs.wkey, self.s.band)
+
+    def select(self, j, queued=False):
+        s, bufs, b = self.s, self.bufs, j % self.s.ring
+        self.sel[b] = Selection(self.inputs[j], self.plan, bufs.norm[b], bufs.zero_idx, index_from_slice=True,
+                                key=bufs.gkey[b] if s.l1_keys else None, slot=bufs.sel_slots[b],
+                                refine=self.refine_args(j) if s.use_guess else None, blocking=s.blocking, queued=queued)
+        self.selected = j
+
+    def guess_through(self, j):
+        while self.selected < j:
+            self.guess_next()
 
     def start_search(self, j):
         s, ev, n = self.s, self.events[j], self.n
@@ -592,11 +619,12 @@
         s, last = self.s, self.n_sets - 1
         while self.guessed < min(last, 1):
             self.guess_next()
+        self.guess_through(0)
         self.started = 0
         self.start_search(0)
         first = self.pending[0]
         while first.engine is not None and not first.engine.done(0, first.ticket):
-            more_guesses = self.guessed < min(last, s.g_ahead)
+            more_guesses = self.guessed < min(last, self.g_ahead)
             if more_guesses:
                 self.guess_next()
             nxt = self.started + 1
@@ -604,7 +632,7 @@
                 if more_guesses:
                     continue
                 break
-            if nxt <= self.guessed and self.sel[nxt % s.ring].event.query():
+            if nxt <= self.selected and self.sel[nxt % s.ring].event.query():
                 self.started = nxt
                 self.start_search(nxt)
             elif s.blocking and not more_guesses:
@@ -616,11 +644,10 @@
             self.fill_one_rank()
         ramp = 2 + 3 * i if s.ramped else self.n_sets
         while self.started < min(last, i + s.s_look, ramp):
-            while self.guessed < min(last, self.started + 1):
-                self.guess_next()
+            self.guess_through(self.started + 1)
             self.started += 1
             self.start_search(self.started)
-        while self.guessed < min(last, i + s.g_ahead):
+        while self.guessed < min(last, i + self.g_ahead):
             self.guess_next()
 
     def collect(self, i) -> AutophaseResult:
```
